# arkworks-rs/groth16

Hardware: AMD Instinct MI355X
Metric: R1CS constraints/sec (create_proof, BLS12-381) (higher is better)
Workload: dtype u32-limb Montgomery integers (Fr 255-bit, Fq 381-bit); 1 GPU; SYN(k=22) synthetic R1CS, 4194302 constraints, FFT domain 2^22, bls12_381, full create_proof (7 NTTs + 4 G1 MSMs + 1 G2 MSM), valid proving key generated on the GPU from seeded toxic waste; curve=bls12_381, log2_domain=22, constraints=4194302, key=valid, witness=resident in HBM at entry (--full: value_incl_h2d holds the PCIe-inclusive rates), parallelism=single-gpu

## Files before the change

### groth16_amd/csrc/api.hip

```cpp
#include "api_types.hpp"
#include "key_load.hpp"
#include "prover.hpp"
#include "proof_glue.hpp"
#include "unit_api.hpp"

namespace {
template <class C>
struct Impl : KeyLoader<C>, Prover<C>, ProofGlue<C>, UnitApi<C> {
    typedef typename C::Fr Fr;
    typedef typename C::Fq Fq;
    typedef typename C::Fq2 Fq2;
};
}

#define G16_DISPATCH(curve, EXPR)                                             \
    do {                                                                      \
        try {                                                                 \
            if ((curve) == G16_BLS12_381) { typedef Impl<Bls12_381> I; return EXPR; } \
            if ((curve) == G16_BN254) { typedef Impl<Bn254> I; return EXPR; }  \
            return G16_ERR_BAD_ARG;                                           \
        } catch (const std::bad_alloc&) {                                     \
            return G16_ERR_OOM;                                               \
        } catch (...) {                                                       \
            return G16_ERR_INTERNAL;                                          \
// ... 59 lines not shown
              hipEventCreate(&c->ev_edge[0]) == hipSuccess && hipEventCreate(&c->ev_edge[1]) == hipSuccess &&
              hipEventCreate(&c->ev_edge[2]) == hipSuccess && hipEventCreate(&c->ev_edge[3]) == hipSuccess &&
              hipEventCreate(&c->ev_edge[4]) == hipSuccess && hipEventCreate(&c->ev_edge[5]) == hipSuccess &&
              hipEventCreate(&c->ev_edge[6]) == hipSuccess && hipEventCreate(&c->ev_edge[7]) == hipSuccess &&
              hipEventCreateWithFlags(&c->ev_heavy[0], hipEventDisableTiming) == hipSuccess &&
              hipEventCreateWithFlags(&c->ev_heavy[1], hipEventDisableTiming) == hipSuccess &&
              hipEventCreateWithFlags(&c->ev_heavy[2], hipEventDisableTiming) == hipSuccess &&
              hipEventCreateWithFlags(&c->ev_heavy[3], hipEventDisableTiming) == hipSuccess &&
              hipStreamCreateWithPriority(&c->red[0], hipStreamNonBlocking, prio_hi) == hipSuccess &&
              hipStreamCreateWithPriority(&c->red[1], hipStreamNonBlocking, prio_hi) == hipSuccess &&
              hipStreamCreateWithPriority(&c->red[2], hipStreamNonBlocking, prio_hi) == hipSuccess &&
              hipStreamCreateWithPriority(&c->red[3], hipStreamNonBlocking, prio_hi) == hipSuccess &&
              hipStreamCreateWithPriority(&c->red[4], hipStreamNonBlocking, prio_hi) == hipSuccess &&
              hipEventCreateWithFlags(&c->ev_wm, hipEventDisableTiming) == hipSuccess &&
              hipEventCreateWithFlags(&c->ev_z, hipEventDisableTiming) == hipSuccess &&
              hipEventCreateWithFlags(&c->ev_h, hipEventDisableTiming) == hipSuccess;
    for (int i = 0; ok && i < 5; ++i)
        ok = hipEventCreate(&c->ev_done[i]) == hipSuccess;
    for (int i = 0; ok && i < 8; ++i)
        ok = hipEventCreateWithFlags(&c->ev_up[i], hipEventDisableTiming) == hipSuccess;
    if (!ok) {
        g16::set_last_error("stream/event creation", hipGetLastError(), __FILE__, __LINE__);
        delete c;
        return G16_ERR_HIP;
    }
    *out = c;
    return G16_OK;
}

int g16_ctx_create_multi(int curve, const int* device_ids, int n_dev, g16_ctx** out) {
    if (!out || !device_ids || n_dev < 1 || n_dev > 64 || (curve != G16_BLS12_381 && curve != G16_BN254)) return G16_ERR_BAD_ARG;
    if (n_dev == 1) return g16_ctx_create(curve, device_ids[0], out);
    g16_ctx* c = new (std::nothrow) g16_ctx();
    if (!c) return G16_ERR_OOM;
    c->curve = curve;
    c->device = device_ids[0];
    c->stream = c->stream2 = c->stream3 = nullptr;
    memset(&c->tm, 0, sizeof(c->tm));
    for (int i = 0; i < n_dev; ++i) {
        g16_ctx* sub = nullptr;
        const int rc = g16_ctx_create(curve, device_ids[i], &sub);
        if (rc) {
            for (g16_ctx* s : c->subs) g16_ctx_destroy(s);
            delete c;
            return rc;
        }
        c->subs.push_back(sub);
    }
    const bool require_peer = getenv("G16_MULTI_REQUIRE_PEER") && atoi(getenv("G16_MULTI_REQUIRE_PEER")) != 0;
    const bool fake_refusal = getenv("G16_MULTI_FAKE_NO_PEER") && atoi(getenv("G16_MULTI_FAKE_NO_PEER")) != 0;
    c->peer.assign((size_t)n_dev * (size_t)n_dev, 1);
    auto fail = [&](int rc) {
        for (g16_ctx* sub : c->subs) g16_ctx_destroy(sub);
        delete c;
        return rc;
    };
    for (int a = 0; a < n_dev; ++a)
        for (int b = 0; b < n_dev; ++b) {
            if (a == b) continue;
            int can = device_ids[a] == device_ids[b] ? 1 : 0;
            if (!can && hipDeviceCanAccessPeer(&can, device_ids[a], device_ids[b]) != hipSuccess) { (void)hipGetLastError(); can = 0; }
            if (fake_refusal) can = 0;
            if (can && device_ids[a] != device_ids[b]) {
                if (hipSetDevice(device_ids[a]) != hipSuccess) return fail(G16_ERR_HIP);
                const hipError_t e = hipDeviceEnablePeerAccess(device_ids[b], 0);
                if (e != hipSuccess && e != hipErrorPeerAccessAlreadyEnabled) {
                    g16::set_last_error("hipDeviceEnablePeerAccess (the pair reports peer capability)", e, __FILE__, __LINE__);
                    return fail(G16_ERR_HIP);
                }
                (void)hipGetLastError();
            }
            c->peer[(size_t)a * n_dev + b] = (char)can;
            if (!can && require_peer) {
                char buf[160];
                snprintf(buf, sizeof(buf), "devices %d and %d of the context have no peer access (G16_MULTI_REQUIRE_PEER=1)", device_ids[a], device_ids[b]);
                g_last_error = buf;
                return fail(G16_ERR_NO_PEER_ACCESS);
            }
        }
    *out = c;
    return G16_OK;
}

int g16_ctx_peer_access(const g16_ctx* ctx, int i, int j) {
    if (!ctx) return -1;
    const int n = ctx->subs.empty() ? 1 : (int)ctx->subs.size();
    if (i < 0 || j < 0 || i >= n || j >= n) return -1;
    if (i == j || ctx->subs.empty()) return 1;
    return ctx->peer[(size_t)i * n + j] ? 1 : 0;
}

int g16_ctx_num_devices(const g16_ctx* ctx) { return ctx ? (ctx->subs.empty() ? 1 : (int)ctx->subs.size()) : 0; }

void g16_ctx_destroy(g16_ctx* ctx) {
    if (!ctx) return;
    if (!ctx->subs.empty()) {
        for (g16_ctx* sub : ctx->subs) g16_ctx_destroy(sub);
        delete ctx;
        return;
    }
    ctx->finprep.drop();
    (void)hipSetDevice(ctx->device);
    (void)hipStreamSynchronize(ctx->stream);
    (void)hipStreamSynchronize(ctx->stream2);
    (void)hipStreamSynchronize(ctx->stream3);
    (void)hipStreamSynchronize(ctx->stream_wm);
    (void)hipStreamSynchronize(ctx->stream_h2d);
    for (int i = 0; i < 5; ++i) (void)hipStreamSynchronize(ctx->red[i]);
    ctx->arena.release();
    ctx->t_wm.destroy(); ctx->t_prep_h.destroy(); ctx->t_prep_z.destroy(); ctx->t_ntt[0].destroy(); ctx->t_ntt[1].destroy();
    for (int i = 0; i < 5; ++i) {
        ctx->t_bucket[i].destroy();
        (void)hipEventDestroy(ctx->ev_done[i]);
    }
    (void)hipEventDestroy(ctx->ev_z); (void)hipEventDestroy(ctx->ev_h); (void)hipEventDestroy(ctx->ev_wm); (void)hipEventDestroy(ctx->ev_dwm);
    for (int i = 0; i < 4; ++i) (void)hipEventDestroy(ctx->ev_heavy[i]);
    for (int i = 0; i < 8; ++i) (void)hipEventDestroy(ctx->ev_edge[i]);
    for (int i = 0; i < 8; ++i) (void)hipEventDestroy(ctx->ev_up[i]);
    (void)hipStreamDestroy(ctx->stream_h2d);
    (void)hipStreamDestroy(ctx->stream_wm);
    if (ctx->pinned) (void)hipHostFree(ctx->pinned);
    (void)hipStreamDestroy(ctx->stream);
    (void)hipStreamDestroy(ctx->stream2);
    (void)hipStreamDestroy(ctx->stream3);
    for (int i = 0; i < 5; ++i) (void)hipStreamDestroy(ctx->red[i]);
    delete ctx;
}

void* g16_ctx_stream(g16_ctx* ctx) { return ctx ? (void*)(ctx->subs.empty() ? ctx->stream : ctx->subs[0]->stream) : nullptr; }
void* g16_ctx_wm_stream(g16_ctx* ctx) { return ctx ? (void*)(ctx->subs.empty() ? ctx->stream_wm : ctx->subs[0]->stream_wm) : nullptr; }

int g16_pk_load(g16_ctx* ctx, const g16_pk_view* view, g16_pk** out) {
    if (!ctx || !view || !out) return G16_ERR_BAD_ARG;
    if (!ctx->subs.empty()) {
        const int n = (int)ctx->subs.size();
        if (view->a.start || view->b_g1.start || view->b_g2.start || view->h.start || view->l.start) return G16_ERR_BAD_ARG;
        if (view->b_g1.count != view->a.count || view->b_g2.count != view->a.count || view->l.count > view->a.count) return G16_ERR_BAD_LENGTH;
        if (view->flags & G16_PK_DEVICE_PTRS)
            for (g16_ctx* sub : ctx->subs) if (sub->device != ctx->subs[0]->device) return G16_ERR_BAD_ARG;
        g16_pk* h = new (std::nothrow) g16_pk{ctx->curve, ctx, nullptr};
        if (!h) return G16_ERR_OOM;
        h->subs.assign((size_t)n, nullptr);
        const uint64_t m = view->a.count, w = view->l.count, hl = view->h.count, skip = m - w;
        const size_t g1b = (ctx->curve == G16_BLS12_381 ? 12 : 8), g2b = 2 * g1b;
        const bool dist_h = !(view->flags & G16_PK_DEVICE_PTRS) && view->h.points && dist_wm_admissible(n, hl + 1);
        if (dist_h) h->dist_n = hl + 1;
        bool bucket = false, bucket_forced = false;
        {
            const char* me = g_multi_force_base ? "base" : getenv("G16_MULTI_SHARD_MODE");
            if (me && strcmp(me, "bucket") == 0) bucket = bucket_forced = true;
            else if (!me || strcmp(me, "auto") == 0) {
                const double key_bytes = (double)(g1b * 8) * (double)(m * 2 + w + hl) + (double)(g2b * 8) * (double)m;
                const double rows = m >= ((uint64_t)1 << 20) ? 13.0 : 32.0;
                const double need = rows * key_bytes * 1.08 + 3.0 * key_bytes + 8.0 * 1073741824.0;
                bucket = rows * key_bytes <= 80.0 * 1073741824.0 && !(view->flags & G16_PK_DEVICE_PTRS);
                const char* pc = getenv("G16_MSM_PRECOMP");
                if ((pc && atoi(pc) == 0) || m <= 1 || hl == 0) bucket = false;
                for (g16_ctx* sub : ctx->subs) {
                    size_t fr = 0, tot = 0;
                    if (!bucket) break;
                    if (hipSetDevice(sub->device) != hipSuccess || hipMemGetInfo(&fr, &tot) != hipSuccess) { (void)hipGetLastError(); bucket = false; }
                    size_t copies = 0;
                    for (g16_ctx* o : ctx->subs) copies += o->device == sub->device ? 1 : 0;
                    if (need * (double)copies > (double)fr) bucket = false;
                }
            }
            if (bucket && (view->flags & G16_PK_DEVICE_PTRS)) { delete h; return G16_ERR_BAD_ARG; }
        }
        h->bucket_mode = bucket;
        std::vector<uint64_t> hgather;
        if (bucket && dist_h) {
            const uint64_t M = (hl + 1) / (uint64_t)n, blk = M / (uint64_t)n;
            hgather.reserve((size_t)(hl * g1b));
            for (uint64_t q = 0; q < (uint64_t)n; ++q)
                for (uint64_t k1 = 0; k1 < (uint64_t)n; ++k1)
                    for (uint64_t j = 0; j < blk; ++j) {
                        const uint64_t idx = q * blk + j + M * k1;
                        if (idx < hl) hgather.insert(hgather.end(), view->h.points + idx * g1b, view->h.points + (idx + 1) * g1b);
                    }
        }
        int rc = for_each_device(n, [&](int i) -> int {
            g16_pk_view v = *view;
            if (bucket) {
                if (dist_h) { v.h.points = hgather.data(); v.h.count = hgather.size() / g1b; v.h.start = 0; }
                return g16_pk_load_bucket_shard(ctx->subs[(size_t)i], &v, i, n, &h->subs[(size_t)i]);
            }
            const uint64_t a_lo = m * (uint64_t)i / n, a_hi = m * (uint64_t)(i + 1) / n;
            const uint64_t l_lo = std::min(w, a_lo > skip ? a_lo - skip : 0), l_hi = std::min(w, a_hi > skip ? a_hi - skip : 0);
            const uint64_t h_lo = hl * (uint64_t)i / n, h_hi = hl * (uint64_t)(i + 1) / n;
            std::vector<uint64_t> hblock;
            if (dist_h) {
                const uint64_t M = (hl + 1) / (uint64_t)n, blk = M / (uint64_t)n;
                hblock.reserve((size_t)(M * g1b));
                for (uint64_t k1 = 0; k1 < (uint64_t)n; ++k1)
                    for (uint64_t j = 0; j < blk; ++j) {
                        const uint64_t idx = (uint64_t)i * blk + j + M * k1;
                        if (idx < hl) hblock.insert(hblock.end(), view->h.points + idx * g1b, view->h.points + (idx + 1) * g1b);
                    }
            }
            auto cut = [](const g16_query& q, uint64_t lo, uint64_t hi, size_t limbs) {
                g16_query r;
                r.points = q.points ? q.points + lo * limbs : nullptr;
                r.count = hi - lo;
                r.start = lo;
                return r;
            };
            v.a = cut(view->a, a_lo, a_hi, g1b);
            v.b_g1 = cut(view->b_g1, a_lo, a_hi, g1b);
            v.b_g2 = cut(view->b_g2, a_lo, a_hi, g2b);
            v.l = cut(view->l, l_lo, l_hi, g1b);
            v.h = cut(view->h, h_lo, h_hi, g1b);
            if (dist_h) { v.h.points = hblock.data(); v.h.count = hblock.size() / g1b; v.h.start = 0; }
            return g16_pk_load(ctx->subs[(size_t)i], &v, &h->subs[(size_t)i]);
        }, serial_loads(ctx));
        if ((rc == G16_ERR_OOM || rc == G16_ERR_BAD_ARG) && bucket && !bucket_forced) {
            for (g16_pk*& sub : h->subs) { g16_pk_free(sub); sub = nullptr; }
            delete h;
            g_multi_force_base = true;
            const int rc2 = g16_pk_load(ctx, view, out);
            g_multi_force_base = false;
            return rc2;
        }
        if (rc) { g16_pk_free(h); return rc; }
        *out = h;
        return G16_OK;
    }
    G16_HIP_TRY(hipSetDevice(ctx->device));
    G16_DISPATCH(ctx->curve, I::pk_load(ctx, view, out));
}

int g16_pk_load_bucket_shard(g16_ctx* ctx, const g16_pk_view* view, int rank, int world, g16_pk** out) {
    if (!ctx || !view || !out || world < 1 || world > 64 || rank < 0 || rank >= world) return G16_ERR_BAD_ARG;
    if (!ctx->subs.empty()) return G16_ERR_BAD_ARG;
    if (world == 1) return g16_pk_load(ctx, view, out);
    G16_HIP_TRY(hipSetDevice(ctx->device));
    G16_DISPATCH(ctx->curve, I::pk_load(ctx, view, out, world, rank));
}

int g16_pk_rebind_bucket_shard(g16_pk* pk, int rank, int world) {
    if (!pk || world < 1 || world > 64 || rank < 0 || rank >= world || !pk->subs.empty() || !pk->dp) return G16_ERR_BAD_ARG;
    auto rebind = [&](auto* dp) -> int {
        if (dp->c_z == 0 || dp->a_start || dp->b_g1_start || dp->b_g2_start || dp->h_start || dp->l_start) return G16_ERR_BAD_ARG;
        dp->shard_n = world;
        dp->shard_r = rank;
        return G16_OK;
    };
    if (pk->ctx->finprep.key_id == pk->id) pk->ctx->finprep.drop();
    pk->ctx->drop_prepared_sort(pk->id);
    if (pk->curve == G16_BLS12_381) return rebind(static_cast<DevicePk<Bls12_381>*>(pk->dp));
    return rebind(static_cast<DevicePk<Bn254>*>(pk->dp));
}

int g16_pk_get_info(const g16_pk* pk, g16_pk_info* out) {
    if (!pk || !out) return G16_ERR_BAD_ARG;
    memset(out, 0, sizeof(*out));
    const g16_pk* one = pk->subs.empty() ? pk : pk->subs[0];
    if (!one || !one->dp) return G16_ERR_BAD_ARG;
    auto fill = [&](const auto* dp) {
        out->window_bits_z = dp->c_z;
        out->window_bits_h = dp->c_h;
        out->table_fallback = dp->table_fallback;
        out->bucket_shard_rank = dp->shard_r;
        out->bucket_shard_world = dp->shard_n;
        out->device_bytes = dp->table_bytes;
    };
    if (one->curve == G16_BLS12_381) fill(static_cast<const DevicePk<Bls12_381>*>(one->dp));
    else fill(static_cast<const DevicePk<Bn254>*>(one->dp));
    out->n_devices = pk->subs.empty() ? 1 : (int)pk->subs.size();
    return G16_OK;
}

void g16_pk_free(g16_pk* pk) {
    if (!pk) return;
    if (!pk->ctx->subs.empty()) {
        for (g16_pk* sub : pk->subs) g16_pk_free(sub);
        delete pk;
        return;
    }
    if (pk->ctx->finprep.key_id == pk->id) pk->ctx->finprep.drop();
    (void)hipSetDevice(pk->ctx->device);
    pk->ctx->drop_prepared_sort(pk->id);
    if (pk->curve == G16_BLS12_381) Impl<Bls12_381>::pk_free(static_cast<DevicePk<Bls12_381>*>(pk->dp));
    else Impl<Bn254>::pk_free(static_cast<DevicePk<Bn254>*>(pk->dp));
    delete pk;
}

int g16_circuit_load(g16_ctx* ctx, const g16_csr_view abc[3], uint64_t num_inputs, uint64_t num_constraints, uint64_t num_variables,
                     g16_circuit** out) {
    if (!ctx || !abc || !out) return G16_ERR_BAD_ARG;
    if (!ctx->subs.empty()) {
        const int n = (int)ctx->subs.size();
        g16_circuit* h = new (std::nothrow) g16_circuit{ctx->curve, ctx, nullptr, 0};
        if (!h) return G16_ERR_OOM;
        h->subs.assign((size_t)n, nullptr);
        const int rc = for_each_device(n, [&](int i) -> int {
            return g16_circuit_load(ctx->subs[(size_t)i], abc, num_inputs, num_constraints, num_variables, &h->subs[(size_t)i]);
        }, serial_loads(ctx));
        if (rc) { g16_circuit_free(h); return rc; }
        h->domain_size = h->subs[0]->domain_size;
        h->num_variables = num_variables;
        if (dist_wm_admissible(n, h->domain_size)) {
            h->dist.assign((size_t)n, DwmSlot());
            const uint64_t M = h->domain_size / (uint64_t)n;
            const int rc2 = for_each_device(n, [&](int i) -> int {
                DwmSlot& sl = h->dist[(size_t)i];
                G16_TRY(g16_dwm_create(ctx->subs[(size_t)i], h->subs[(size_t)i], i, n, &sl.dwm));
                for (int k = 0; k < 3; ++k) {
                    if (hipMalloc((void**)&sl.work[k], M * 32) != hipSuccess || hipMalloc((void**)&sl.recv[k], M * 32) != hipSuccess) return G16_ERR_OOM;
// ... 480 lines not shown
```

### groth16_amd/csrc/batch_affine.hpp

```cpp
#pragma once
#include "curve.hpp"
#include "fp30.hpp"

namespace g16 {

template <class P>
struct ModInv30 {
    static constexpr int NL = P::NL30;
    static constexpr int32_t M30 = (int32_t)((1u << 30) - 1u);
    struct S30 { int32_t v[NL]; };
    struct T2x2 { int32_t u, v, q, r; };

    G16_HD static int32_t divsteps30(int32_t zeta, uint32_t f0, uint32_t g0, T2x2& t) {
        uint32_t u = 1, v = 0, q = 0, r = 1, f = f0, g = g0;
        for (int i = 0; i < 30; ++i) {
            uint32_t m1 = (uint32_t)(zeta >> 31);
            const uint32_t m2 = 0u - (g & 1u);
            const uint32_t x = (f ^ m1) - m1, y = (u ^ m1) - m1, z = (v ^ m1) - m1;
            g += x & m2; q += y & m2; r += z & m2;
            m1 &= m2;
            zeta = (zeta ^ (int32_t)m1) - 1;
            f += g & m1; u += q & m1; v += r & m1;
            g >>= 1; u <<= 1; v <<= 1;
        }
        t.u = (int32_t)u; t.v = (int32_t)v; t.q = (int32_t)q; t.r = (int32_t)r;
        return zeta;
    }
    G16_HD static void update_fg(S30& f, S30& g, const T2x2& t) {
        const int64_t u = t.u, v = t.v, q = t.q, r = t.r;
        int64_t cf = u * f.v[0] + v * g.v[0], cg = q * f.v[0] + r * g.v[0];
        cf >>= 30; cg >>= 30;
        G16_UNROLL for (int i = 1; i < NL; ++i) {
            cf += u * f.v[i] + v * g.v[i];
            cg += q * f.v[i] + r * g.v[i];
            f.v[i - 1] = (int32_t)cf & M30; cf >>= 30;
            g.v[i - 1] = (int32_t)cg & M30; cg >>= 30;
        }
        f.v[NL - 1] = (int32_t)cf;
        g.v[NL - 1] = (int32_t)cg;
    }
    G16_HD static void update_de(S30& d, S30& e, const T2x2& t) {
        const int64_t u = t.u, v = t.v, q = t.q, r = t.r;
        const int32_t sd = d.v[NL - 1] >> 31, se = e.v[NL - 1] >> 31;
        int32_t md = (t.u & sd) + (t.v & se), me = (t.q & sd) + (t.r & se);
        int64_t cd = u * d.v[0] + v * e.v[0], ce = q * d.v[0] + r * e.v[0];
        md -= (int32_t)((P::PPINV30 * (uint32_t)cd + (uint32_t)md) & (uint32_t)M30);
        me -= (int32_t)((P::PPINV30 * (uint32_t)ce + (uint32_t)me) & (uint32_t)M30);
        cd += (int64_t)(int32_t)P::p30(0) * md;
        ce += (int64_t)(int32_t)P::p30(0) * me;
        cd >>= 30; ce >>= 30;
        G16_UNROLL for (int i = 1; i < NL; ++i) {
            cd += u * d.v[i] + v * e.v[i] + (int64_t)(int32_t)P::p30(i) * md;
            ce += q * d.v[i] + r * e.v[i] + (int64_t)(int32_t)P::p30(i) * me;
            d.v[i - 1] = (int32_t)cd & M30; cd >>= 30;
            e.v[i - 1] = (int32_t)ce & M30; ce >>= 30;
        }
        d.v[NL - 1] = (int32_t)cd;
        e.v[NL - 1] = (int32_t)ce;
    }
    G16_HD static void carry(S30& r) {
        G16_UNROLL for (int i = 0; i + 1 < NL; ++i) { r.v[i + 1] += r.v[i] >> 30; r.v[i] &= M30; }
    }
    G16_HD static void normalize(S30& r, int32_t sign) {
        const int32_t add1 = r.v[NL - 1] >> 31, neg = sign >> 31;
        G16_UNROLL for (int i = 0; i < NL; ++i) {
            int32_t x = r.v[i] + ((int32_t)P::p30(i) & add1);
            r.v[i] = (x ^ neg) - neg;
        }
        carry(r);
        const int32_t add2 = r.v[NL - 1] >> 31;
        G16_UNROLL for (int i = 0; i < NL; ++i) r.v[i] += (int32_t)P::p30(i) & add2;
        carry(r);
    }
    G16_HD static Fp30<P> inverse_plain(const Fp30<P>& x) {
        S30 d, e, f, g;
        G16_UNROLL for (int i = 0; i < NL; ++i) { d.v[i] = 0; e.v[i] = 0; f.v[i] = (int32_t)P::p30(i); g.v[i] = (int32_t)x.l[i]; }
        e.v[0] = 1;
        int32_t zeta = -1;
        for (int it = 0; it < 4 * NL; ++it) {
            int32_t nz = 0;
            G16_UNROLL for (int i = 0; i < NL; ++i) nz |= g.v[i];
            if (nz == 0) break;
            T2x2 t;
            zeta = divsteps30(zeta, (uint32_t)f.v[0], (uint32_t)g.v[0], t);
            update_de(d, e, t);
            update_fg(f, g, t);
        }
        normalize(d, f.v[NL - 1]);
        Fp30<P> r;
        G16_UNROLL for (int i = 0; i < NL; ++i) r.l[i] = (uint32_t)d.v[i];
        return r;
    }
    G16_HD static Fp30<P> inverse(const Fp30<P>& x) {
        Fp30<P> c;
        G16_UNROLL for (int i = 0; i < NL; ++i) c.l[i] = P::r3_30(i);
        return inverse_plain(x).mul(c);
    }
};

template <class P>
G16_HD Fp30<P> batch_inverse(const Fp30<P>& a) { return ModInv30<P>::inverse(a); }
template <class P>
G16_HD Fp30<P> pair_inverse(bool hi, const Fp30<P>& m, const Fp30<P>& o) {
    const Fp30<P> n = m.sqr().add(o.sqr());
    const Fp30<P> t = m.mul(ModInv30<P>::inverse(n));
    return hi ? Fp30<P>::zero().template sub<2>(t) : t;
}
template <class P>
G16_HD Fp2p30<P> batch_inverse(const Fp2p30<P>& a) { return {pair_inverse<P>(Fp2p30<P>::lane_hi(), a.c, Fp2p30<P>::swap(a.c))}; }

template <class F>
struct AffineBatch {
    enum { ADD = 0, DBL = 1, TAKE_P = 2, TAKE_Q = 3, ZERO = 4 };
    G16_HD static int classify(bool pz, bool qz, const F& px, const F& py, const F& qx, const F& qy, F& d) {
        d = F::one();
        if (pz || qz) return pz ? (qz ? (int)ZERO : (int)TAKE_Q) : (int)TAKE_P;
        if (qx.equals_canonical(px)) {
            if (py.add(qy).is_zero_exact()) return ZERO;
            d = py.dbl();
            return DBL;
        }
        d = qx.template sub<2>(px);
        return ADD;
    }
    G16_HD static void finish(int kind, const F& px, const F& py, const F& qx, const F& qy, const F& inv_d, F& rx, F& ry, bool& rz) {
        rz = false;
        if (kind >= TAKE_P) {
            if (kind == TAKE_P) { rx = px; ry = py; }
            else if (kind == TAKE_Q) { rx = qx; ry = qy; }
            else { rx = F::zero(); ry = F::zero(); rz = true; }
            return;
        }
        F num;
        if (kind == DBL) {
            const F x2 = px.sqr();
            num = x2.dbl().add(x2);
        } else {
            num = qy.template sub<2>(py);
        }
        const F lam = num.mul(inv_d);
        rx = lam.sqr().template sub<2>(px).template sub<2>(qx).canonical_lt8p();
        ry = lam.mul(px.template sub<2>(rx)).template sub<2>(py).canonical_lt8p();
    }
};

struct alignas(16) Word4 { uint32_t w[4]; };
static constexpr uint32_t SORT_HOLE = 0xffffffffu;

template <class F>
struct AffineLevelArgs {
    const Affine<typename F::Std>* in;
    Affine<typename F::Std>* out;
    const uint32_t* sorted;
    const uint32_t* total;
    Word4* prefix;
    int64_t shift;
    uint64_t base_count;
    uint32_t merged;
    uint32_t level;
    uint32_t K;
};

template <class F, bool LEVEL0>
struct AffineLevel {
    typedef Affine<typename F::Std> A;
    static constexpr int LPT = F::LANES_PER_TASK;
    static constexpr uint32_t T = 64 / LPT;
    static constexpr int QUADS = (F::PREFIX_LIMBS + 3) / 4;

    G16_HD static bool load_operand(const AffineLevelArgs<F>& a, uint64_t slot, F& x, F& y) {
        if constexpr (LEVEL0) {
            const uint32_t v = a.sorted[slot];
            if (v == SORT_HOLE) return false;
            const uint32_t pt = a.merged ? (v & 0x3ffffffu) : (v & 0x7fffffffu);
            const uint64_t row = a.merged ? (uint64_t)((v >> 26) & 31u) * a.base_count : 0;
            const int64_t idx = (int64_t)pt + a.shift;
            if (idx < 0 || (uint64_t)idx >= a.base_count) return false;
            if (!F::load_point(a.in, (int64_t)row + idx, x, y)) return false;
            if (v >> 31) y = y.neg_canonical();
            return true;
        } else {
            return F::load_point(a.in, (int64_t)slot, x, y);
        }
    }
    G16_HD static void store_prefix(const AffineLevelArgs<F>& a, uint32_t wave, uint32_t j, uint32_t lane, const F& v) {
        uint32_t w[4 * QUADS];
        G16_UNROLL for (int i = 0; i < 4 * QUADS; ++i) w[i] = 0;
        v.get_limbs(w);
        Word4* dst = a.prefix + ((uint64_t)wave * a.K + j) * (QUADS * 64) + lane;
        G16_UNROLL for (int c = 0; c < QUADS; ++c) {
            Word4 q;
            G16_UNROLL for (int i = 0; i < 4; ++i) q.w[i] = w[4 * c + i];
            dst[c * 64] = q;
        }
    }
    G16_HD static F load_prefix(const AffineLevelArgs<F>& a, uint32_t wave, uint32_t j, uint32_t lane) {
        uint32_t w[4 * QUADS];
        const Word4* src = a.prefix + ((uint64_t)wave * a.K + j) * (QUADS * 64) + lane;
        G16_UNROLL for (int c = 0; c < QUADS; ++c) {
            const Word4 q = src[c * 64];
            G16_UNROLL for (int i = 0; i < 4; ++i) w[4 * c + i] = q.w[i];
        }
        return F::from_limbs(w);
    }
    G16_HD static void run(const AffineLevelArgs<F>& a, uint32_t wave, uint32_t lane) {
        const uint64_t n_out = (uint64_t)(*a.total) >> (a.level + 1);
        const uint64_t first = (uint64_t)wave * a.K * T;
        if (first >= n_out) return;
        const uint64_t left = (n_out - first + T - 1) / T;
        const uint32_t steps = left < a.K ? (uint32_t)left : a.K;
        const uint32_t task = lane / LPT;
        F pre = F::one();
        for (uint32_t j = 0; j < steps; ++j) {
            const uint64_t q = first + (uint64_t)j * T + task;
            F px = F::zero(), py = F::zero(), qx = F::zero(), qy = F::zero(), d;
            bool pz = true, qz = true;
            if (q < n_out) {
                pz = !load_operand(a, 2 * q, px, py);
                qz = !load_operand(a, 2 * q + 1, qx, qy);
            }
            (void)AffineBatch<F>::classify(pz, qz, px, py, qx, qy, d);
            pre = pre.mul(d);
            store_prefix(a, wave, j, lane, pre);
        }
        F inv = batch_inverse(pre);
        for (uint32_t j = steps; j-- > 0;) {
            const uint64_t q = first + (uint64_t)j * T + task;
            F px = F::zero(), py = F::zero(), qx = F::zero(), qy = F::zero(), d;
            bool pz = true, qz = true;
            if (q < n_out) {
                pz = !load_operand(a, 2 * q, px, py);
                qz = !load_operand(a, 2 * q + 1, qx, qy);
            }
            const F prev = j ? load_prefix(a, wave, j - 1, lane) : F::one();
            const int kind = AffineBatch<F>::classify(pz, qz, px, py, qx, qy, d);
            const F inv_d = inv.mul(prev);
            inv = inv.mul(d);
            F rx, ry;
            bool rz;
            AffineBatch<F>::finish(kind, px, py, qx, qy, inv_d, rx, ry, rz);
            if (q < n_out) F::store_point(a.out, (int64_t)q, rx, ry, rz);
        }
    }
};

}
```

### groth16_amd/csrc/devtest.hip

```cpp
#include "internal.hpp"
#include "fp30.hpp"
#include <vector>

using namespace g16;

namespace g16 {
int ctx_devices(const g16_ctx* ctx, int* curve, std::vector<int>& devs, std::vector<hipStream_t>& streams);
}

namespace {

constexpr bool lab_slots(int form, int* nin, int* nout) {
    int i = 0, o = 1;
    switch (form) {
        case 0: i = 2; break;
        case 1: i = 1; break;
        case 2: i = 4; break;
        case 3: i = 8; break;
        case 4: case 6: case 8: i = 3; break;
        case 5: case 7: case 9: i = 5; break;
        case 10: i = 4; break;
        case 11: i = 3; break;
        case 20: case 21: case 22: case 23: case 24: case 25: i = 2; break;
        case 26: i = 1; break;
        case 27: i = 3; break;
        case 28: i = 2; o = 2; break;
        case 30: case 31: case 32: case 33: case 34: case 35: case 36: case 37: case 38: case 39: case 40: case 41: case 42: case 43: i = 1; break;
        case 50: i = 4; o = 2; break;
        case 51: i = 2; o = 2; break;
        case 60: i = 4; o = 2; break;
        case 61: i = 2; o = 2; break;
        case 62: i = 6; o = 2; break;
        case 63: case 64: case 65: i = 8; o = 2; break;
        case 70: i = 11; o = 5; break;
        case 71: case 72: i = 21; o = 9; break;
        default: return false;
    }
    *nin = i;
    *nout = o;
    return true;
}
constexpr int lab_nin(int form) { int i = 0, o = 0; lab_slots(form, &i, &o); return i; }
constexpr int lab_nout(int form) { int i = 0, o = 0; lab_slots(form, &i, &o); return o; }
constexpr bool lab_is_pair(int form) { return (form >= 60 && form < 70) || form == 72; }
template <class P>
constexpr bool lab_has(int form) {
    constexpr bool base = FipsAsm<P>::has_sub;
    if ((form >= 4 && form <= 11) || form >= 50) return base;
    if (form == 27) return !base;
    return true;
}

template <class P> G16_HD Fp30<P> ld(const uint32_t* s, int k) {
    Fp30<P> r;
    G16_UNROLL for (int i = 0; i < Fp30<P>::NL; ++i) r.l[i] = s[k * Fp30<P>::NL + i];
    return r;
}
template <class P> G16_HD void st(uint32_t* o, int k, const Fp30<P>& v) {
    G16_UNROLL for (int i = 0; i < Fp30<P>::NL; ++i) o[k * Fp30<P>::NL + i] = v.l[i];
}
template <class P> G16_HD void st_flag(uint32_t* o, int k, bool b) {
    G16_UNROLL for (int i = 0; i < Fp30<P>::NL; ++i) o[k * Fp30<P>::NL + i] = (i == 0 && b) ? 1u : 0u;
}
template <class P> G16_HD Fp<P> ld_words(const uint32_t* s, int k) {
    Fp<P> r;
    G16_UNROLL for (int i = 0; i < P::N; ++i) r.v[i] = s[k * Fp30<P>::NL + i];
    return r;
}
template <class P> G16_HD void st_words(uint32_t* o, int k, const Fp<P>& v) {
    G16_UNROLL for (int i = 0; i < Fp30<P>::NL; ++i) o[k * Fp30<P>::NL + i] = i < P::N ? v.v[i] : 0u;
}

template <class P, class F>
struct AccLab {
    typedef Fp30<P> B;
    static constexpr int C = sizeof(F) == sizeof(B) && F::LANES_PER_TASK == 1 ? 1 : 2;
    G16_HD static F ldf(const uint32_t* in, int slot, int hi) {
        if constexpr (F::LANES_PER_TASK == 2) return F{ld<P>(in, slot + hi)};
        else if constexpr (C == 2) return F{ld<P>(in, slot), ld<P>(in, slot + 1)};
        else return ld<P>(in, slot);
    }
    G16_HD static void stf(uint32_t* out, int slot, int hi, const F& v) {
        if constexpr (F::LANES_PER_TASK == 2) st_words<P>(out, slot + hi, v.c.to_packed());
        else if constexpr (C == 2) { st_words<P>(out, slot, v.c0.to_packed()); st_words<P>(out, slot + 1, v.c1.to_packed()); }
        else st_words<P>(out, slot, v.to_packed());
    }
    G16_HD static void run(const uint32_t* in, uint32_t* out, int hi) {
        const uint32_t* flags = in + 4 * C * B::NL;
        Acc30<F> a;
        a.x = ldf(in, 0, hi); a.y = ldf(in, C, hi); a.zz = ldf(in, 2 * C, hi); a.zzz = ldf(in, 3 * C, hi);
        a.inf = flags[0] != 0;
        const int n = flags[1] > 3u ? 3 : (int)flags[1];
        for (int j = 0; j < n; ++j) {
            if (flags[2 + j] != 0) continue;
            a.add_affine(ldf(in, 4 * C + 1 + 2 * j * C, hi), ldf(in, 4 * C + 1 + (2 * j + 1) * C, hi));
        }
        if (a.inf) a.x = a.y = a.zz = a.zzz = F::zero();
        stf(out, 0, hi, a.x); stf(out, C, hi, a.y); stf(out, 2 * C, hi, a.zz); stf(out, 3 * C, hi, a.zzz);
        if (F::LANES_PER_TASK == 1 || hi == 0) st_flag<P>(out, 4 * C, a.inf);
    }
};

template <class P, int FORM>
struct LabOp {
    typedef Fp30<P> B;
    G16_HD static void run(const uint32_t* in, uint32_t* out) {
        auto L = [&](int k) { return ld<P>(in, k); };
        if constexpr (FORM == 0) st<P>(out, 0, L(0).mul(L(1)));
        else if constexpr (FORM == 1) st<P>(out, 0, L(0).sqr());
        else if constexpr (FORM == 2) st<P>(out, 0, B::mul_add_fused(L(0), L(1), L(2), L(3)));
        else if constexpr (FORM == 3) st<P>(out, 0, B::template mul4_cols<uint64_t>(L(0), L(1), L(2), L(3), L(4), L(5), L(6), L(7)));
        else if constexpr (FORM == 4) st<P>(out, 0, L(0).template mul_sub_k<2>(L(1), L(2)));
        else if constexpr (FORM == 5) st<P>(out, 0, B::template mul2_sub_k<2>(L(0), L(1), L(2), L(3), L(4)));
        else if constexpr (FORM == 6) st<P>(out, 0, L(0).template mul_sub_k<4>(L(1), L(2)));
        else if constexpr (FORM == 7) st<P>(out, 0, B::template mul2_sub_k<4>(L(0), L(1), L(2), L(3), L(4)));
        else if constexpr (FORM == 8) st<P>(out, 0, L(0).template mul_sub_k<8>(L(1), L(2)));
        else if constexpr (FORM == 9) st<P>(out, 0, B::template mul2_sub_k<8>(L(0), L(1), L(2), L(3), L(4)));
        else if constexpr (FORM == 10) st<P>(out, 0, L(0).mul_sub_x3(L(1), L(2), L(3)));
        else if constexpr (FORM == 11) st<P>(out, 0, L(0).sqr_sub_x3(L(1), L(2)));
        else if constexpr (FORM == 20) st<P>(out, 0, L(0).template sub<2>(L(1)));
        else if constexpr (FORM == 21) st<P>(out, 0, L(0).template sub<4>(L(1)));
        else if constexpr (FORM == 22) st<P>(out, 0, L(0).template sub<6>(L(1)));
        else if constexpr (FORM == 23) st<P>(out, 0, L(0).template sub<8>(L(1)));
        else if constexpr (FORM == 24) st<P>(out, 0, L(0).template sub<16>(L(1)));
        else if constexpr (FORM == 25) st<P>(out, 0, L(0).add_dbl(L(1)));
        else if constexpr (FORM == 26) { B a = L(0); a.normalize(); st<P>(out, 0, a); }
        else if constexpr (FORM == 27) {
            const int k = (int)in[2 * B::NL];
            st<P>(out, 0, L(0).sub_pow2(L(1), k < 0 ? 0 : k > 11 ? 11 : k));
        }
        else if constexpr (FORM == 28) {
            const Fp<P> y = ld_words<P>(in, 0);
            const bool flip = in[B::NL] != 0;
            st<P>(out, 0, B::unpack_cond_neg(y, flip));
            st<P>(out, 1, B::cond_neg2(B::unpack(y.v), flip));
        }
        else if constexpr (FORM == 30) st<P>(out, 0, L(0).template cond_sub<2>());
        else if constexpr (FORM == 31) st<P>(out, 0, L(0).template cond_sub<4>());
        else if constexpr (FORM == 32) st<P>(out, 0, L(0).template cond_sub<8>());
        else if constexpr (FORM == 33) st<P>(out, 0, L(0).template cond_sub<16>());
        else if constexpr (FORM == 34) st<P>(out, 0, L(0).weak_reduce32());
        else if constexpr (FORM == 35) st<P>(out, 0, L(0).canonical_lt2p());
        else if constexpr (FORM == 36) st<P>(out, 0, L(0).canonical_lt8p());
        else if constexpr (FORM == 37) st<P>(out, 0, L(0).canonical_quick());
        else if constexpr (FORM == 38) st<P>(out, 0, L(0).neg_canonical());
        else if constexpr (FORM == 39) st_flag<P>(out, 0, L(0).maybe_zero());
        else if constexpr (FORM == 40) st_flag<P>(out, 0, L(0).is_zero_exact());
        else if constexpr (FORM == 41) st_words<P>(out, 0, L(0).to_std());
        else if constexpr (FORM == 42) st_words<P>(out, 0, B::std_to_r30(ld_words<P>(in, 0)));
        else if constexpr (FORM == 43) st_words<P>(out, 0, L(0).to_packed());
        else if constexpr (FORM == 50) {
            const Fp2x30<P> a{L(0), L(1)}, b{L(2), L(3)};
            const Fp2x30<P> r = a.mul(b);
            st<P>(out, 0, r.c0); st<P>(out, 1, r.c1);
        }
        else if constexpr (FORM == 51) {
            const Fp2x30<P> a{L(0), L(1)};
            const Fp2x30<P> r = a.sqr();
            st<P>(out, 0, r.c0); st<P>(out, 1, r.c1);
        }
        else if constexpr (FORM == 70) AccLab<P, Fp30<P>>::run(in, out, 0);
        else if constexpr (FORM == 71) AccLab<P, Fp2x30<P>>::run(in, out, 0);
    }
};

template <class P, int FORM>
struct LabPair {
    typedef Fp30<P> B;
    typedef Fp2p30<P> F;
#if defined(__HIP_DEVICE_COMPILE__)
    static __device__ __forceinline__ void run(const uint32_t* in, uint32_t* out) {
        const int hi = F::lane_hi() ? 1 : 0;
        if constexpr (FORM == 72) { AccLab<P, F>::run(in, out, hi); return; }
        auto L = [&](int k) { return F{ld<P>(in, 2 * k + hi)}; };
        F r = F::zero();
        if constexpr (FORM == 60) r = F::mul_v(F::lhs(L(0)), F::rhs(L(1)));
        else if constexpr (FORM == 61) r = F::sqr_v(F::lhs(L(0)));
        else if constexpr (FORM == 62) r = F::sqr_sub_x3_v(F::lhs(L(0)), L(1), L(2));
        else if constexpr (FORM == 63) r = F::mul_add_fused(L(0), L(1), L(2), L(3));
        else if constexpr (FORM == 64) r = F::mul_sub_fused(L(0), L(1), L(2), L(3));
        else if constexpr (FORM == 65) r = F::mul_add_fused_v(F::lhs(L(0)), F::rhs(L(1)), F::lhs(L(2)), F::rhs(L(3)));
        st<P>(out, hi, r.c);
    }
#endif
    static void run_host(const uint32_t* in, uint32_t* out) {
        for (int h = 0; h < 2; ++h) {
            const bool hi = h != 0;
            auto C = [&](int k, int c) { return ld<P>(in, 2 * k + c); };
            auto y2 = [&](int k) { return hi ? C(k, 0) : C(k, 1).neg16(); };
            B r = B::zero();
            if constexpr (FORM == 60) r = F::pair_mul_c(hi, C(0, 0), C(0, 1), C(1, h), C(1, 1 - h));
            else if constexpr (FORM == 61) r = F::pair_sqr_c(hi, C(0, 0), C(0, 1));
            else if constexpr (FORM == 62) r = F::pair_sqr_sub_x3(hi, C(0, 0), C(0, 1), C(1, h), C(2, h));
            else if constexpr (FORM == 63) r = F::pair_mul_add_c(hi, C(0, 0), C(0, 1), C(1, h), C(1, 1 - h), C(2, 0), C(2, 1), C(3, h), C(3, 1 - h));
            else if constexpr (FORM == 64) r = F::pair_mul_sub_c(hi, C(0, 0), C(0, 1), C(1, h), C(1, 1 - h), C(2, 0), C(2, 1), C(3, h), C(3, 1 - h));
            else if constexpr (FORM == 65) r = B::template mul4_cols<uint64_t>(C(0, 0), C(1, h), C(0, 1), y2(1), C(2, 0), C(3, h), C(2, 1), y2(3));
            st<P>(out, h, r);
        }
    }
};

constexpr int LAB_WG = 64;

template <class P, int FORM>
__global__ void __launch_bounds__(LAB_WG) devlab_op(const uint32_t* __restrict__ in, uint32_t* __restrict__ out, uint32_t n) {
    constexpr int NL = Fp30<P>::NL, NIN = lab_nin(FORM), NOUT = lab_nout(FORM);
    const uint32_t t = blockIdx.x * LAB_WG + threadIdx.x;
    if constexpr (lab_is_pair(FORM)) {
        if (t >= 2 * n) return;
        const size_t i = t >> 1;
#if defined(__HIP_DEVICE_COMPILE__)
        LabPair<P, FORM>::run(in + i * NIN * NL, out + i * NOUT * NL);
#endif
    } else {
        if (t >= n) return;
        LabOp<P, FORM>::run(in + (size_t)t * NIN * NL, out + (size_t)t * NOUT * NL);
    }
}

template <class P, int FORM>
int lab_device(hipStream_t st, const uint32_t* operands, uint64_t n, uint32_t* out) {
    constexpr int NL = Fp30<P>::NL, NIN = lab_nin(FORM), NOUT = lab_nout(FORM);
    const size_t in_bytes = (size_t)n * NIN * NL * 4, out_bytes = (size_t)n * NOUT * NL * 4;
    uint32_t *d_in = nullptr, *d_out = nullptr;
    G16_HIP_TRY(hipMalloc((void**)&d_in, in_bytes));
    if (hipMalloc((void**)&d_out, out_bytes) != hipSuccess) { (void)hipFree(d_in); return G16_ERR_OOM; }
    auto body = [&]() -> int {
        G16_HIP_TRY(hipMemcpyAsync(d_in, operands, in_bytes, hipMemcpyHostToDevice, st));
        G16_HIP_TRY(hipMemsetAsync(d_out, 0, out_bytes, st));
        const uint64_t lanes = lab_is_pair(FORM) ? 2 * n : n;
        devlab_op<P, FORM><<<dim3((unsigned)((lanes + LAB_WG - 1) / LAB_WG)), dim3(LAB_WG), 0, st>>>(d_in, d_out, (uint32_t)n);
        G16_LAUNCH_CHECK();
        G16_HIP_TRY(hipMemcpyAsync(out, d_out, out_bytes, hipMemcpyDeviceToHost, st));
        G16_HIP_TRY(hipStreamSynchronize(st));
        return G16_OK;
    };
    const int rc = body();
    (void)hipFree(d_in);
    (void)hipFree(d_out);
    return rc;
}

template <class P, int FORM>
int lab_host(const uint32_t* operands, uint64_t n, uint32_t* out) {
    constexpr int NL = Fp30<P>::NL, NIN = lab_nin(FORM), NOUT = lab_nout(FORM);
    for (uint64_t i = 0; i < n; ++i) {
        if constexpr (lab_is_pair(FORM)) LabPair<P, FORM>::run_host(operands + i * NIN * NL, out + i * NOUT * NL);
        else LabOp<P, FORM>::run(operands + i * NIN * NL, out + i * NOUT * NL);
    }
    return G16_OK;
}

#define LAB_FORMS(X)                                                                                                              \
    X(0) X(1) X(2) X(3) X(4) X(5) X(6) X(7) X(8) X(9) X(10) X(11) X(20) X(21) X(22) X(23) X(24) X(25) X(26) X(27) X(28) X(30) X(31) \
    X(32) X(33) X(34) X(35) X(36) X(37) X(38) X(39) X(40) X(41) X(42) X(43) X(50) X(51) X(60) X(61) X(62) X(63) X(64) X(65) X(70) X(71) X(72)

template <class P>
int lab_dispatch(bool device, hipStream_t st, int form, const uint32_t* operands, uint64_t n, uint32_t* out) {
    switch (form) {
#define X(F)                                                                                   \
    case F:                                                                                    \
        if constexpr (lab_has<P>(F)) {                                                         \
            if (device) return lab_device<P, F>(st, operands, n, out);                         \
            if constexpr (F == 72) return G16_ERR_BAD_ARG;                                     \
            else return lab_host<P, F>(operands, n, out);                                      \
        } else return G16_ERR_BAD_ARG;
        LAB_FORMS(X)
#undef X
        default: return G16_ERR_BAD_ARG;
    }
}

int lab_run(int curve, bool device, hipStream_t st, int field, int form, const uint32_t* operands, uint64_t n, uint32_t* out) {
    int nin = 0, nout = 0;
    if (!operands || !out || n == 0 || n > ((uint64_t)1 << 22) || (field != 0 && field != 1) || !lab_slots(form, &nin, &nout)) return G16_ERR_BAD_ARG;
    if (curve == G16_BLS12_381)
        return field ? lab_dispatch<Bls12_381FqP>(device, st, form, operands, n, out) : lab_dispatch<Bls12_381FrP>(device, st, form, operands, n, out);
    if (curve == G16_BN254)
        return field ? lab_dispatch<Bn254FqP>(device, st, form, operands, n, out) : lab_dispatch<Bn254FrP>(device, st, form, operands, n, out);
    return G16_ERR_BAD_ARG;
}

}

extern "C" int g16_dev_fp30_op(g16_ctx* ctx, int field, int form, const uint32_t* operands, uint64_t n, uint32_t* out) {
    int curve = 0;
    std::vector<int> devs;
    std::vector<hipStream_t> streams;
    G16_TRY(ctx_devices(ctx, &curve, devs, streams));
    G16_HIP_TRY(hipSetDevice(devs[0]));
    return lab_run(curve, true, streams[0], field, form, operands, n, out);
}

extern "C" int g16_host_fp30_op(int curve, int field, int form, const uint32_t* operands, uint64_t n, uint32_t* out) {
    return lab_run(curve, false, nullptr, field, form, operands, n, out);
}
```

### groth16_amd/csrc/fp30.hpp

```cpp
#pragma once
#include "field.hpp"
#include "fips_asm_gen.hpp"

#if defined(__HIP_DEVICE_COMPILE__) && !defined(G16_NO_FIPS_ASM)
#define G16_ASM_PRODUCTS 1
#endif

namespace g16 {

template <class P>
struct Fp30 {
    typedef P Params_t;
    static constexpr int NL = P::NL30;
    static constexpr int NW = P::N;
    static constexpr uint32_t MASK = (1u << 30) - 1u;
    uint32_t l[NL];

    G16_HD static Fp30 zero() {
        Fp30 r;
        G16_UNROLL for (int i = 0; i < NL; ++i) r.l[i] = 0;
        return r;
    }
    G16_HD static Fp30 one() {
        Fp30 r;
        G16_UNROLL for (int i = 0; i < NL; ++i) r.l[i] = P::one30(i);
        return r;
    }
    G16_HD static Fp30 unpack(const uint32_t* w) {
        Fp30 r;
        G16_UNROLL for (int i = 0; i < NL; ++i) {
            const int bit = 30 * i, wd = bit >> 5, sh = bit & 31;
            uint32_t v = w[wd] >> sh;
            if (sh > 2 && wd + 1 < NW) v |= w[wd + 1] << (32 - sh);
            r.l[i] = (i == NL - 1) ? v : (v & MASK);
        }
        return r;
    }
    G16_HD void pack(uint32_t* w) const {
        G16_UNROLL for (int k = 0; k < NW; ++k) w[k] = 0;
        G16_UNROLL for (int i = 0; i < NL; ++i) {
            const int bit = 30 * i, wd = bit >> 5, sh = bit & 31;
            w[wd] |= l[i] << sh;
            if (sh > 2 && wd + 1 < NW) w[wd + 1] |= l[i] >> (32 - sh);
        }
    }
    G16_HD void normalize() {
        G16_UNROLL for (int i = 0; i + 1 < NL; ++i) {
            l[i + 1] += l[i] >> 30;
            l[i] &= MASK;
        }
    }
    G16_HD Fp30 add(const Fp30& b) const {
        Fp30 r;
        G16_UNROLL for (int i = 0; i < NL; ++i) r.l[i] = l[i] + b.l[i];
        r.normalize();
        return r;
    }
    G16_HD Fp30 dbl() const { return add(*this); }
    template <int K>
    G16_HD Fp30 sub(const Fp30& b) const {
        static_assert(K == 2 || K == 4 || K == 6 || K == 8 || K == 16, "redundant K p tables exist for K = 2, 4, 6, 8, 16 only");
        Fp30 r;
        G16_UNROLL for (int i = 0; i < NL; ++i) {
            const uint32_t kp = K == 2 ? P::kp2(i) : K == 4 ? P::kp4(i) : K == 6 ? P::kp6(i) : K == 8 ? P::kp8(i) : P::kp16(i);
            r.l[i] = l[i] + kp - b.l[i];
        }
        r.normalize();
        return r;
    }
    G16_HD Fp30 add_dbl(const Fp30& b) const {
        Fp30 r;
        G16_UNROLL for (int i = 0; i < NL; ++i) r.l[i] = l[i] + (b.l[i] << 1);
        r.normalize();
        return r;
    }
    G16_HD Fp30 sub_pow2(const Fp30& b, int k) const {
        Fp30 r;
        G16_UNROLL for (int i = 0; i < NL; ++i) r.l[i] = l[i] + P::kp_pow2(k, i) - b.l[i];
        r.normalize();
        return r;
    }
    G16_HD Fp30 neg2() const { return zero().template sub<2>(*this); }
    typedef Fp<P> PackedC;
    G16_HD static constexpr uint32_t two_p32(int i) { return (P::mod(i) << 1) | (i ? P::mod(i - 1) >> 31 : 0u); }
    G16_HD static Fp30 unpack_cond_neg(const PackedC& y, bool flip) {
        uint32_t w[NW];
#if defined(__HIP_DEVICE_COMPILE__)
        unsigned borrow = 0;
        G16_UNROLL for (int i = 0; i < NW; ++i) {
            const uint32_t d = __builtin_subc(two_p32(i), y.v[i], borrow, &borrow);
            w[i] = flip ? d : y.v[i];
        }
#else
        uint32_t borrow = 0;
        G16_UNROLL for (int i = 0; i < NW; ++i) {
            const uint64_t t = (uint64_t)two_p32(i) - y.v[i] - borrow;
            borrow = (uint32_t)(t >> 63);
            w[i] = flip ? (uint32_t)t : y.v[i];
        }
#endif
        return unpack(w);
    }
    G16_HD static Fp30 cond_neg2(const Fp30& a, bool flip) { return flip ? a.neg2() : a; }
    G16_HD Fp30 neg16() const { return zero().template sub<16>(*this); }
    typedef Fp<P> Std;
    G16_HD static Fp30 from_packed(const Std& x) { return unpack(x.v); }

    G16_HD Fp30 mul(const Fp30& b) const { return mul_impl(b); }
    template <int NS>
    struct FipsPlan {
        unsigned char seg[2 * NL][NS + 1];
        unsigned char nseg[2 * NL];
        int extra;
        bool ok;
    };
    template <int NS>
    static constexpr FipsPlan<NS> fips_plan() {
        typedef unsigned __int128 W;
        FipsPlan<NS> pl{};
        const W LIM = (W)1 << 64, M = MASK, W32 = 0xffffffffu;
        W carry = 0;
        pl.ok = true;
        pl.extra = 0;
        for (int c = 0; c < 2 * NL - 1; ++c) {
            const int lo = c < NL ? 0 : c - NL + 1, hi = c < NL ? c : NL - 1;
            W psum = 0;
            for (int i = lo; i <= hi; ++i)
                if (i != c) psum += M * (W)P::p30(c - i);
            W B[NS + 1] = {};
            B[0] = carry + (c < NL ? M * (W)P::p30(0) : (W)0) + (W)(NS + 2) * W32;
            int cur = 0;
            for (int k = 0; k <= NS; ++k) {
                const W part = k < NS ? (W)(hi - lo + 1) * M * M : psum;
                if (B[cur] + part >= LIM) {
                    ++cur;
                    if (cur > NS || part >= LIM) { pl.ok = false; return pl; }
                }
                B[cur] += part;
                pl.seg[c][k] = (unsigned char)cur;
            }
            pl.nseg[c] = (unsigned char)(cur + 1);
            pl.extra += cur;
            carry = B[0] >> 30;
            for (int s = 1; s <= cur; ++s) carry += 4 * (B[s] >> 32);
        }
        return pl;
    }
    template <int NS>
    static constexpr bool fips_asm_plan_agrees() {
        if constexpr (!FipsAsm<P>::available) return true;
        else {
            static_assert(NS == 1 || NS == 2 || NS == 4, "assembly exists for one, two and four sweeps");
            const FipsPlan<NS> pl = fips_plan<NS>();
            if (!pl.ok || FipsAsm<P>::NL != NL) return false;
            for (int c = 0; c < 2 * NL - 1; ++c)
                for (int k = 0; k <= NS; ++k) {
                    const int want = NS == 1 ? FipsAsm<P>::plan1(c * 2 + k) : NS == 2 ? FipsAsm<P>::plan2(c * 3 + k) : FipsAsm<P>::plan4(c * 5 + k);
                    if (pl.seg[c][k] != want) return false;
                }
            return true;
        }
// ... 97 lines not shown
            Fp30 r;
            FipsAsm<P>::mul2(r.l, x1.l, y1.l, x2.l, y2.l);
            return r;
        }
#endif
        const Fp30* xs[2] = {&x1, &x2};
        const Fp30* ys[2] = {&y1, &y2};
        return fips<U, 2, false>(xs, ys);
    }
    template <class U>
    G16_HD static Fp30 mul4_cols(const Fp30& x1, const Fp30& y1, const Fp30& x2, const Fp30& y2, const Fp30& x3, const Fp30& y3,
                                 const Fp30& x4, const Fp30& y4) {
#ifdef G16_ASM_PRODUCTS
        if constexpr (sizeof(U) == 8 && FipsAsm<P>::available) {
            static_assert(fips_asm_plan_agrees<4>(), "gen_fips_asm.py and Fp30::fips_plan disagree on the column plan");
            Fp30 r;
            FipsAsm<P>::mul4(r.l, x1.l, y1.l, x2.l, y2.l, x3.l, y3.l, x4.l, y4.l);
            return r;
        }
#endif
        const Fp30* xs[4] = {&x1, &x2, &x3, &x4};
        const Fp30* ys[4] = {&y1, &y2, &y3, &y4};
        return fips<U, 4, false>(xs, ys);
    }
    template <class U>
    G16_HD static Fp30 mul_sub_cols(const Fp30& a, const Fp30& b, const Fp30& c, const Fp30& d) {
        return mul2_cols<U>(a, b, c, d.neg2());
    }
    template <int K>
    G16_HD Fp30 mul_sub_k(const Fp30& b, const Fp30& s) const {
        static_assert(K == 2 || K == 4 || K == 8, "fused subtraction: K = 2, 4, 8");
#ifdef G16_ASM_PRODUCTS
        if constexpr (FipsAsm<P>::has_sub) {
            static_assert(fips_asm_plan_agrees<1>(), "gen_fips_asm.py and Fp30::fips_plan disagree on the column plan");
            Fp30 r;
            if constexpr (K == 2) FipsAsm<P>::mul_s2(r.l, l, b.l, s.l);
            else if constexpr (K == 4) FipsAsm<P>::mul_s4(r.l, l, b.l, s.l);
            else FipsAsm<P>::mul_s8(r.l, l, b.l, s.l);
            return r;
        }
#endif
        return mul(b).template sub<K>(s);
    }
    template <int K>
    G16_HD static Fp30 mul2_sub_k(const Fp30& x1, const Fp30& y1, const Fp30& x2, const Fp30& y2, const Fp30& s) {
        static_assert(K == 2 || K == 4 || K == 8, "fused subtraction: K = 2, 4, 8");
#ifdef G16_ASM_PRODUCTS
        if constexpr (FipsAsm<P>::has_sub) {
            static_assert(fips_asm_plan_agrees<2>(), "gen_fips_asm.py and Fp30::fips_plan disagree on the column plan");
            Fp30 r;
            if constexpr (K == 2) FipsAsm<P>::mul2_s2(r.l, x1.l, y1.l, x2.l, y2.l, s.l);
            else if constexpr (K == 4) FipsAsm<P>::mul2_s4(r.l, x1.l, y1.l, x2.l, y2.l, s.l);
            else FipsAsm<P>::mul2_s8(r.l, x1.l, y1.l, x2.l, y2.l, s.l);
            return r;
        }
#endif
        return mul2_cols<uint64_t>(x1, y1, x2, y2).template sub<K>(s);
    }
    G16_HD Fp30 sqr_sub_x3(const Fp30& u, const Fp30& v) const {
#ifdef G16_ASM_PRODUCTS
        if constexpr (FipsAsm<P>::has_sub) {
            Fp30 r;
            FipsAsm<P>::sqr_x3(r.l, l, u.l, v.l);
            return r;
        }
#endif
        return sqr().template sub<6>(u.add_dbl(v));
    }
    G16_HD Fp30 mul_sub_x3(const Fp30& b, const Fp30& u, const Fp30& v) const {
#ifdef G16_ASM_PRODUCTS
        if constexpr (FipsAsm<P>::has_sub) {
            Fp30 r;
            FipsAsm<P>::mul_x3(r.l, l, b.l, u.l, v.l);
            return r;
        }
#endif
        return mul_impl(b).template sub<6>(u.add_dbl(v));
    }
    G16_HD Fp30 mul_impl(const Fp30& b) const { return mul_cols<uint64_t>(b); }
    G16_HD static Fp30 mul_sub(const Fp30& a, const Fp30& b, const Fp30& c, const Fp30& d) { return a.mul(b).template sub<2>(c.mul(d)); }
    typedef Fp30 Lhs;
    typedef Fp30 Rhs;
    G16_HD static const Fp30& lhs(const Fp30& a) { return a; }
    G16_HD static const Fp30& rhs(const Fp30& a) { return a; }
    G16_HD static Fp30 mul_v(const Fp30& a, const Fp30& b) { return a.mul(b); }
    G16_HD static Fp30 sqr_v(const Fp30& a) { return a.sqr(); }
    G16_HD static Fp30 sqr_sub_x3_v(const Fp30& a, const Fp30& u, const Fp30& v) { return a.sqr_sub_x3(u, v); }
    G16_HD static Fp30 mul_add_fused_v(const Fp30& a, const Fp30& b, const Fp30& c, const Fp30& d) { return mul2_cols<uint64_t>(a, b, c, d); }
    G16_HD static Fp30 mul_add_fused(const Fp30& a, const Fp30& b, const Fp30& c, const Fp30& d) { return mul2_cols<uint64_t>(a, b, c, d); }
    G16_HD static Fp30 mul_sub_fused(const Fp30& a, const Fp30& b, const Fp30& c, const Fp30& d) { return mul_sub_cols<uint64_t>(a, b, c, d); }
    G16_HD Fp30 sqr() const { return sqr_cols<uint64_t>(); }

    G16_HD bool maybe_zero() const { return ((l[0] * P::PPINV30) & MASK) < 16u; }
    G16_HD bool is_zero_exact() const {
        const uint32_t k = (l[0] * P::PPINV30) & MASK;
        if (k >= 16u) return false;
        Fp30 kp;
        uint64_t c = 0;
        G16_UNROLL for (int i = 0; i < NL; ++i) {
            const uint64_t v = (uint64_t)k * P::p30(i) + c;
            kp.l[i] = (i == NL - 1) ? (uint32_t)v : ((uint32_t)v & MASK);
            c = v >> 30;
        }
        uint32_t diff = 0;
        G16_UNROLL for (int i = 0; i < NL; ++i) diff |= kp.l[i] ^ l[i];
        return diff == 0;
    }
    template <int K>
    G16_HD Fp30 cond_sub() const {
        static_assert(K == 2 || K == 4 || K == 8 || K == 16, "k p constants exist for k = 2, 4, 8, 16 only");
        Fp30 d;
        int32_t br = 0;
        G16_UNROLL for (int i = 0; i < NL; ++i) {
            const uint32_t c = K == 2 ? P::np2(i) : K == 4 ? P::np4(i) : K == 8 ? P::np8(i) : P::np16(i);
            const int32_t v = (int32_t)l[i] - (int32_t)c + br;
            if (i == NL - 1) { d.l[i] = (uint32_t)v; br = v >> 31; }
            else { d.l[i] = (uint32_t)v & MASK; br = v >> 30; }
        }
        Fp30 r;
        const bool lt = br < 0;
        G16_UNROLL for (int i = 0; i < NL; ++i) r.l[i] = lt ? l[i] : d.l[i];
        return r;
    }
    G16_HD Fp30 weak_reduce32() const { return cond_sub<16>().template cond_sub<8>().template cond_sub<4>().template cond_sub<2>(); }
    G16_HD bool raw_zero() const {
        uint32_t a = 0;
        G16_UNROLL for (int i = 0; i < NL; ++i) a |= l[i];
        return a == 0;
    }
    typedef Fp30 Raw;
    static constexpr int KM = 2, K2M = 4, KX = 8, KY = 4;
#ifndef G16_ACC_MIN_WAVES
#define G16_ACC_MIN_WAVES 2
#endif
    static constexpr int ACC_MIN_WAVES = G16_ACC_MIN_WAVES;
    static constexpr bool ACC_PREFETCH = true;
    static constexpr int LANES_PER_TASK = 1;
    template <class A>
    G16_HD static bool load_point(const A* bases, int64_t idx, Fp30& px, Fp30& py) {
        const A p = bases[idx];
        if (p.is_identity()) return false;
        px = from_packed(p.x);
        py = from_packed(p.y);
        return true;
    }
    template <class A>
    G16_HD static bool load_point_py(const A* bases, int64_t idx, Fp30& px, PackedC& yw) {
        const A p = bases[idx];
        if (p.is_identity()) return false;
        px = from_packed(p.x);
        yw = p.y;
        return true;
    }


    G16_HD Fp30 canonical_lt2p() const {
        Fp30 d;
        int32_t br = 0;
        G16_UNROLL for (int i = 0; i < NL; ++i) {
            const int32_t v = (int32_t)l[i] - (int32_t)P::p30(i) + br;
            if (i == NL - 1) { d.l[i] = (uint32_t)v; br = v >> 31; }
            else { d.l[i] = (uint32_t)v & MASK; br = v >> 30; }
        }
        Fp30 r;
        const bool lt = br < 0;
        G16_UNROLL for (int i = 0; i < NL; ++i) r.l[i] = lt ? l[i] : d.l[i];
        return r;
    }

    G16_HD Fp30 canonical_lt8p() const { return cond_sub<4>().template cond_sub<2>().canonical_lt2p(); }
    G16_HD Fp30 canonical_quick() const {
        constexpr uint32_t D = P::p30(NL - 1) + 1u;
        static_assert(D > (1u << 13), "the top limb of p carries at least 14 bits for every supported field");
        constexpr uint64_t MAGIC = ((uint64_t)1 << 40) / D;
        const uint32_t q = (uint32_t)(((uint64_t)l[NL - 1] * MAGIC) >> 40);
        Fp30 r;
        int64_t carry = 0;
        G16_UNROLL for (int i = 0; i < NL; ++i) {
            const int64_t t = (int64_t)l[i] - (int64_t)((uint64_t)q * P::p30(i)) + carry;
            r.l[i] = (i == NL - 1) ? (uint32_t)t : ((uint32_t)t & MASK);
            carry = t >> 30;
        }
        return r.canonical_lt8p();
    }
    G16_HD Fp30 neg_canonical() const {
        Fp30 d;
        int32_t br = 0;
        G16_UNROLL for (int i = 0; i < NL; ++i) {
            const int32_t v = (int32_t)P::p30(i) - (int32_t)l[i] + br;
            if (i == NL - 1) d.l[i] = (uint32_t)v;
            else { d.l[i] = (uint32_t)v & MASK; br = v >> 30; }
        }
        return d;
    }
    G16_HD bool same_limbs(const Fp30& o) const {
        uint32_t a = 0;
        G16_UNROLL for (int i = 0; i < NL; ++i) a |= l[i] ^ o.l[i];
        return a == 0;
    }
    static constexpr int PREFIX_LIMBS = NL;
    G16_HD void get_limbs(uint32_t* w) const { G16_UNROLL for (int i = 0; i < NL; ++i) w[i] = l[i]; }
    G16_HD static Fp30 from_limbs(const uint32_t* w) { Fp30 r; G16_UNROLL for (int i = 0; i < NL; ++i) r.l[i] = w[i]; return r; }
    G16_HD bool equals_canonical(const Fp30& o) const { return same_limbs(o); }
    template <class A>
    G16_HD static void store_point(A* dst, int64_t idx, const Fp30& x, const Fp30& y, bool identity) {
        A p;
        if (identity) { p = A::identity(); }
        else { x.pack(p.x.v); y.pack(p.y.v); }
        dst[idx] = p;
    }

    G16_HD Std to_packed() const {
        Std r;
        mul_impl(one()).canonical_lt2p().pack(r.v);
        return r;
    }
    G16_HD static Fp<P> std_to_r30(const Fp<P>& x) {
        Fp<P> c;
        G16_UNROLL for (int i = 0; i < P::N; ++i) c.v[i] = P::r30_plain(i);
        return x * c;
    }
    G16_HD Fp<P> to_std() const {
        Fp30 c;
        G16_UNROLL for (int i = 0; i < NL; ++i) c.l[i] = P::rstd30(i);
        const Fp30 t = mul(c).canonical_lt2p();
        Fp<P> r;
        t.pack(r.v);
        return r;
    }
};

template <class P>
struct Fp2x30 {
    typedef Fp30<P> B;
    typedef Fp2<P> Std;
    B c0, c1;
    G16_HD static Fp2x30 zero() { return {B::zero(), B::zero()}; }
    G16_HD static Fp2x30 one() { return {B::one(), B::zero()}; }
    G16_HD static Fp2x30 from_packed(const Std& x) { return {B::unpack(x.c0.v), B::unpack(x.c1.v)}; }
    G16_HD Fp2x30 add(const Fp2x30& o) const { return {c0.add(o.c0), c1.add(o.c1)}; }
    G16_HD Fp2x30 dbl() const { return {c0.dbl(), c1.dbl()}; }
    G16_HD Fp2x30 add_dbl(const Fp2x30& o) const { return {c0.add_dbl(o.c0), c1.add_dbl(o.c1)}; }
    template <int K>
    G16_HD Fp2x30 sub(const Fp2x30& o) const { return {c0.template sub<K>(o.c0), c1.template sub<K>(o.c1)}; }
    G16_HD Fp2x30 neg2() const { return {c0.neg2(), c1.neg2()}; }
    G16_HD static Fp2x30 cond_neg2(const Fp2x30& a, bool flip) { return flip ? a.neg2() : a; }
    G16_HD Fp2x30 mul_impl(const Fp2x30& o) const {
        Fp2x30 r;
        const B nb1 = o.c1.neg16();
        r.c0 = B::template mul2_cols<uint64_t>(c0, o.c0, c1, nb1);
        r.c1 = B::template mul2_cols<uint64_t>(c0, o.c1, c1, o.c0);
        return r;
    }
    G16_HD Fp2x30 sqr_impl() const {
        return {c0.add(c1).mul_impl(c0.template sub<16>(c1)), c0.dbl().mul_impl(c1)};
    }
    G16_HD_NOINLINE static Fp2x30 mul_outlined(const Fp2x30& a, const Fp2x30& b) { return a.mul_impl(b); }
    G16_HD_NOINLINE static Fp2x30 sqr_outlined(const Fp2x30& a) { return a.sqr_impl(); }
    G16_HD Fp2x30 mul(const Fp2x30& o) const { return mul_outlined(*this, o); }
    G16_HD Fp2x30 sqr() const { return sqr_outlined(*this); }
    template <int K>
    G16_HD Fp2x30 mul_sub_k(const Fp2x30& o, const Fp2x30& s) const { return mul(o).template sub<K>(s); }
    G16_HD Fp2x30 sqr_sub_x3(const Fp2x30& u, const Fp2x30& v) const { return sqr().template sub<KM + K2M>(u.add_dbl(v)); }
    G16_HD bool maybe_zero() const { return c0.maybe_zero() && c1.maybe_zero(); }
    G16_HD bool is_zero_exact() const { return c0.is_zero_exact() && c1.is_zero_exact(); }
    G16_HD Std to_std() const { return {c0.to_std(), c1.to_std()}; }
    G16_HD Std to_packed() const { return {c0.to_packed(), c1.to_packed()}; }
    static constexpr int KM = 2, K2M = 4, KX = 8, KY = 4;
    G16_HD static Fp2x30 mul_sub(const Fp2x30& a, const Fp2x30& b, const Fp2x30& c, const Fp2x30& d) { return a.mul(b).template sub<KM>(c.mul(d)); }
    G16_HD static Fp2x30 mul_sub_fused(const Fp2x30& a, const Fp2x30& b, const Fp2x30& c, const Fp2x30& d) { return mul_sub(a, b, c, d); }
    G16_HD static Fp2x30 mul_add_fused(const Fp2x30& a, const Fp2x30& b, const Fp2x30& c, const Fp2x30& d) { return a.mul(b).add(c.mul(d)); }
    typedef Fp2x30 Lhs;
    typedef Fp2x30 Rhs;
    G16_HD static const Fp2x30& lhs(const Fp2x30& a) { return a; }
    G16_HD static const Fp2x30& rhs(const Fp2x30& a) { return a; }
    G16_HD static Fp2x30 mul_v(const Fp2x30& a, const Fp2x30& b) { return a.mul(b); }
    G16_HD static Fp2x30 sqr_v(const Fp2x30& a) { return a.sqr(); }
    G16_HD static Fp2x30 sqr_sub_x3_v(const Fp2x30& a, const Fp2x30& u, const Fp2x30& v) { return a.sqr_sub_x3(u, v); }
    G16_HD static Fp2x30 mul_add_fused_v(const Fp2x30& a, const Fp2x30& b, const Fp2x30& c, const Fp2x30& d) { return mul_add_fused(a, b, c, d); }
    G16_HD bool raw_zero() const { return c0.raw_zero() && c1.raw_zero(); }
    typedef Fp2x30 Raw;
    static constexpr int PREFIX_LIMBS = 2 * B::NL;
    static constexpr int LANES_PER_TASK = 1;
};

template <class P>
struct Fp2p30 {
    typedef Fp30<P> B;
    typedef Fp2<P> Std;
    B c;

    G16_HD static bool lane_hi() {
#if defined(__HIP_DEVICE_COMPILE__)
        return (threadIdx.x & 1u) != 0;
#else
        return false;
#endif
    }
    G16_HD static uint32_t swap32(uint32_t v) {
#if defined(__HIP_DEVICE_COMPILE__)
        return (uint32_t)__builtin_amdgcn_mov_dpp((int)v, 0xB1 , 0xF, 0xF, true);
#else
        return v;
#endif
    }
    G16_HD static B swap(const B& x) {
        B r;
        G16_UNROLL for (int i = 0; i < B::NL; ++i) r.l[i] = swap32(x.l[i]);
        return r;
    }
    G16_HD static B sel(bool c, const B& a, const B& b) {
        B r;
        G16_UNROLL for (int i = 0; i < B::NL; ++i) r.l[i] = c ? a.l[i] : b.l[i];
        return r;
    }
    G16_HD static uint32_t bcast32(uint32_t v, bool odd) {
#if defined(__HIP_DEVICE_COMPILE__)
        return odd ? (uint32_t)__builtin_amdgcn_mov_dpp((int)v, 0xF5 , 0xF, 0xF, true)
                   : (uint32_t)__builtin_amdgcn_mov_dpp((int)v, 0xA0 , 0xF, 0xF, true);
#else
        return v;
#endif
    }
    G16_HD static B comp0(const B& x) { B r; G16_UNROLL for (int i = 0; i < B::NL; ++i) r.l[i] = bcast32(x.l[i], false); return r; }
    G16_HD static B comp1(const B& x) { B r; G16_UNROLL for (int i = 0; i < B::NL; ++i) r.l[i] = bcast32(x.l[i], true); return r; }
    G16_HD static B pair_mul_c(bool hi, const B& a0, const B& a1, const B& mb, const B& ob) {
        const B y2 = sel(hi, ob, ob.neg16());
        return pair_cols<uint64_t>(a0, mb, a1, y2);
    }
    G16_HD static B pair_mul(bool hi, const B& ma, const B& oa, const B& mb, const B& ob) {
        return pair_mul_c(hi, sel(hi, oa, ma), sel(hi, ma, oa), mb, ob);
    }
    template <class U>
    G16_HD static B pair_cols(const B& x1, const B& y1, const B& x2, const B& y2) {
        return B::template mul2_cols<U>(x1, y1, x2, y2);
    }
    G16_HD static void pair_sqr_operands(bool hi, const B& a0, const B& a1, B& x, B& y) {
        x = a0.add(sel(hi, a0, a1));
        y = sel(hi, a1, a0.template sub<16>(a1));
    }
    G16_HD static B pair_sqr_c(bool hi, const B& a0, const B& a1) {
        B x, y;
        pair_sqr_operands(hi, a0, a1, x, y);
        return x.mul_impl(y);
    }
    G16_HD static B pair_sqr(bool hi, const B& m, const B& o) { return pair_sqr_c(hi, sel(hi, o, m), sel(hi, m, o)); }
    G16_HD static B pair_mul_sub_c(bool hi, const B& a0, const B& a1, const B& mb, const B& ob, const B& c0, const B& c1, const B& md,
                                   const B& od) {
        const B y2 = sel(hi, ob, ob.neg16());
        const B z1 = md.neg2();
        const B z2 = sel(hi, od.neg2(), od);
        return B::template mul4_cols<uint64_t>(a0, mb, a1, y2, c0, z1, c1, z2);
    }
    G16_HD static B pair_mul_sub(bool hi, const B& ma, const B& oa, const B& mb, const B& ob, const B& mc, const B& oc, const B& md,
                                 const B& od) {
        return pair_mul_sub_c(hi, sel(hi, oa, ma), sel(hi, ma, oa), mb, ob, sel(hi, oc, mc), sel(hi, mc, oc), md, od);
    }
    G16_HD static B pair_mul_add_c(bool hi, const B& a0, const B& a1, const B& mb, const B& ob, const B& c0, const B& c1, const B& md,
                                   const B& od) {
        const B y2 = sel(hi, ob, ob.neg16());
        const B z2 = sel(hi, od, od.neg2());
        return B::template mul4_cols<uint64_t>(a0, mb, a1, y2, c0, md, c1, z2);
    }
    G16_HD static Fp2p30 mul_add_fused(const Fp2p30& a, const Fp2p30& b, const Fp2p30& c, const Fp2p30& d) {
        return {pair_mul_add_c(lane_hi(), comp0(a.c), comp1(a.c), b.c, swap(b.c), comp0(c.c), comp1(c.c), d.c, swap(d.c))};
    }
    struct Lhs { B a0, a1; };
    struct Rhs { B m, y2; };
    G16_HD static Lhs lhs(const Fp2p30& a) { return {comp0(a.c), comp1(a.c)}; }
    G16_HD static Rhs rhs(const Fp2p30& b) { return {b.c, swap(sel(lane_hi(), b.c.neg16(), b.c))}; }
    G16_HD static Fp2p30 mul_v(const Lhs& a, const Rhs& b) { return {pair_cols<uint64_t>(a.a0, b.m, a.a1, b.y2)}; }
    G16_HD static Fp2p30 sqr_v(const Lhs& a) { return {pair_sqr_c(lane_hi(), a.a0, a.a1)}; }
    G16_HD static Fp2p30 sqr_sub_x3_v(const Lhs& a, const Fp2p30& u, const Fp2p30& v) { return {pair_sqr_sub_x3(lane_hi(), a.a0, a.a1, u.c, v.c)}; }
    G16_HD static Fp2p30 mul_add_fused_v(const Lhs& a, const Rhs& b, const Lhs& c, const Rhs& d) {
        return {B::template mul4_cols<uint64_t>(a.a0, b.m, a.a1, b.y2, c.a0, d.m, c.a1, d.y2)};
    }
    G16_HD static Fp2p30 mul_sub(const Fp2p30& a, const Fp2p30& b, const Fp2p30& c, const Fp2p30& d) { return a.mul(b).template sub<2>(c.mul(d)); }
    G16_HD static Fp2p30 mul_sub_fused(const Fp2p30& a, const Fp2p30& b, const Fp2p30& c, const Fp2p30& d) {
        return {pair_mul_sub_c(lane_hi(), comp0(a.c), comp1(a.c), b.c, swap(b.c), comp0(c.c), comp1(c.c), d.c, swap(d.c))};
    }
    G16_HD static Fp2p30 zero() { return {B::zero()}; }
    G16_HD static Fp2p30 one() { return {lane_hi() ? B::zero() : B::one()}; }
    G16_HD Fp2p30 add(const Fp2p30& o) const { return {c.add(o.c)}; }
    G16_HD Fp2p30 dbl() const { return {c.dbl()}; }
    G16_HD Fp2p30 add_dbl(const Fp2p30& o) const { return {c.add_dbl(o.c)}; }
    template <int K>
    G16_HD Fp2p30 sub(const Fp2p30& o) const { return {c.template sub<K>(o.c)}; }
    G16_HD Fp2p30 neg2() const { return {c.neg2()}; }
    G16_HD static Fp2p30 cond_neg2(const Fp2p30& a, bool flip) { return flip ? a.neg2() : a; }
    G16_HD Fp2p30 mul(const Fp2p30& o) const { return {pair_mul_c(lane_hi(), comp0(c), comp1(c), o.c, swap(o.c))}; }
    template <int K>
    G16_HD static B pair_mul_sub_k(bool hi, const B& a0, const B& a1, const B& mb, const B& ob, const B& sub) {
        const B y2 = sel(hi, ob, ob.neg16());
        return B::template mul2_sub_k<K>(a0, mb, a1, y2, sub);
    }
    template <int K>
    G16_HD Fp2p30 mul_sub_k(const Fp2p30& o, const Fp2p30& s) const { return {pair_mul_sub_k<K>(lane_hi(), comp0(c), comp1(c), o.c, swap(o.c), s.c)}; }
    G16_HD static B pair_sqr_sub_x3(bool hi, const B& a0, const B& a1, const B& u, const B& v) {
        B x, y;
        pair_sqr_operands(hi, a0, a1, x, y);
        return x.mul_sub_x3(y, u, v);
    }
    G16_HD Fp2p30 sqr_sub_x3(const Fp2p30& u, const Fp2p30& v) const { return {pair_sqr_sub_x3(lane_hi(), comp0(c), comp1(c), u.c, v.c)}; }
    G16_HD Fp2p30 sqr() const { return {pair_sqr_c(lane_hi(), comp0(c), comp1(c))}; }
    G16_HD static bool both(bool v) { return v && (swap32(v ? 1u : 0u) != 0u); }
    G16_HD bool maybe_zero() const { return both(c.maybe_zero()); }
    G16_HD bool is_zero_exact() const { return both(c.is_zero_exact()); }
    static constexpr int KM = 2, K2M = 4, KX = 8, KY = 4;
    G16_HD Fp2p30 canonical_lt8p() const { return {c.canonical_lt8p()}; }
    G16_HD Fp2p30 neg_canonical() const { return {c.neg_canonical()}; }
    G16_HD bool equals_canonical(const Fp2p30& o) const { return both(c.same_limbs(o.c)); }
    static constexpr int PREFIX_LIMBS = B::NL;
    G16_HD void get_limbs(uint32_t* w) const { c.get_limbs(w); }
    G16_HD static Fp2p30 from_limbs(const uint32_t* w) { return {B::from_limbs(w)}; }
    template <class A>
    G16_HD static void store_point(A* dst, int64_t idx, const Fp2p30& x, const Fp2p30& y, bool identity) {
        Fp<P>* w = reinterpret_cast<Fp<P>*>(dst + idx);
        const int k = lane_hi() ? 1 : 0;
        Fp<P> xw = Fp<P>::zero(), yw = Fp<P>::zero();
        if (!identity) { x.c.pack(xw.v); y.c.pack(yw.v); }
        w[k] = xw;
        w[2 + k] = yw;
    }
    typedef Fp2x30<P> Raw;
#ifndef G16_PAIR_MIN_WAVES
#define G16_PAIR_MIN_WAVES 2
#endif
    static constexpr int ACC_MIN_WAVES = G16_PAIR_MIN_WAVES;
    static constexpr bool ACC_PREFETCH = false;
    static constexpr int LANES_PER_TASK = 2;
    template <class A>
    G16_HD static bool load_point(const A* bases, int64_t idx, Fp2p30& px, Fp2p30& py) {
        const Fp<P>* w = reinterpret_cast<const Fp<P>*>(bases + idx);
        const int k = lane_hi() ? 1 : 0;
        const Fp<P> xw = w[k], yw = w[2 + k];
        const bool zero_half = xw.is_zero() && yw.is_zero();
        if (both(zero_half)) return false;
        px.c = B::unpack(xw.v);
        py.c = B::unpack(yw.v);
        return true;
    }
    typedef Fp<P> PackedC;
    template <class A>
    G16_HD static bool load_point_py(const A* bases, int64_t idx, Fp2p30& px, PackedC& yout) {
        const Fp<P>* w = reinterpret_cast<const Fp<P>*>(bases + idx);
        const int k = lane_hi() ? 1 : 0;
        const Fp<P> xw = w[k], yw = w[2 + k];
        const bool zero_half = xw.is_zero() && yw.is_zero();
        if (both(zero_half)) return false;
        px.c = B::unpack(xw.v);
        yout = yw;
        return true;
    }
    G16_HD static Fp2p30 unpack_cond_neg(const PackedC& y, bool flip) { return {B::unpack_cond_neg(y, flip)}; }
};

template <class R>
struct alignas(16) AccRaw {
    R x, y, zz, zzz;
};

template <class F>
struct Acc30 {
    typedef typename F::Std StdF;
    F x, y, zz, zzz;
    bool inf;

    G16_HD static Acc30 identity() {
        Acc30 a;
        a.x = a.y = a.zz = a.zzz = F::zero();
        a.inf = true;
        return a;
    }
    G16_HD void set_double(const F& px, const F& py) {
        const F U = py.dbl();
        if (U.is_zero_exact()) { inf = true; return; }
        const F V = U.sqr();
        const F W = U.mul(V);
        const F S = px.mul(V);
        const F X2 = px.sqr();
        const F M = X2.dbl().add(X2);
        const F X3 = M.sqr().template sub<F::K2M>(S.dbl());
        const F Y3 = F::mul_sub(M, S.template sub<F::KX>(X3), py, W);
        x = X3; y = Y3; zz = V; zzz = W;
        inf = false;
    }
    G16_HD void add_affine(const F& px, const F& py) {
        if (inf) {
            x = px; y = py; zz = F::one(); zzz = F::one();
            inf = false;
            return;
        }
        const F U2 = px.mul(zz);
        const F S2 = py.mul(zzz);
        const F Pd = U2.template sub<F::KX>(x);
        const F R = S2.template sub<F::KY>(y);
        if (Pd.maybe_zero()) {
            if (Pd.is_zero_exact()) {
                if (R.is_zero_exact()) set_double(px, py);
                else inf = true;
                return;
            }
        }
        const F PP = Pd.sqr();
        const F PPP = Pd.mul(PP);
        const F Q = x.mul(PP);
        const F X3 = R.sqr().template sub<F::KM>(PPP).template sub<F::K2M>(Q.dbl());
        const F Y3 = F::mul_sub(R, Q.template sub<F::KX>(X3), y, PPP);
        x = X3;
        y = Y3;
        zz = zz.mul(PP);
        zzz = zzz.mul(PPP);
    }
    G16_HD void dbl() {
        if (inf) return;
        const F U = y.dbl();
        if (U.is_zero_exact()) { inf = true; return; }
        const F V = U.sqr();
        const F W = U.mul(V);
        const F S = x.mul(V);
        const F X2 = x.sqr();
        const F M = X2.dbl().add(X2);
        const F X3 = M.sqr().template sub<F::K2M>(S.dbl());
        const F Y3 = F::mul_sub(M, S.template sub<F::KX>(X3), y, W);
        x = X3; y = Y3;
        zz = V.mul(zz);
        zzz = W.mul(zzz);
    }
    G16_HD void add(const Acc30& o) {
        if (o.inf) return;
        if (inf) { *this = o; return; }
        const F U1 = x.mul(o.zz);
        const F U2 = o.x.mul(zz);
        const F S1 = y.mul(o.zzz);
        const F S2 = o.y.mul(zzz);
        const F Pd = U2.template sub<F::KM>(U1);
        const F R = S2.template sub<F::KM>(S1);
        if (Pd.maybe_zero()) {
            if (Pd.is_zero_exact()) {
                if (R.is_zero_exact()) dbl();
                else inf = true;
                return;
            }
        }
        const F PP = Pd.sqr();
        const F PPP = Pd.mul(PP);
        const F Q = U1.mul(PP);
        const F X3 = R.sqr().template sub<F::KM>(PPP).template sub<F::K2M>(Q.dbl());
        const F Y3 = F::mul_sub(R, Q.template sub<F::KX>(X3), S1, PPP);
        x = X3;
        y = Y3;
        zz = zz.mul(o.zz).mul(PP);
        zzz = zzz.mul(o.zzz).mul(PPP);
    }
    G16_HD Acc30 mul_small(uint32_t k) const {
        Acc30 acc = identity();
        for (int i = 31; i >= 0; --i) {
            acc.dbl();
            if ((k >> i) & 1) acc.add(*this);
        }
        return acc;
    }
    G16_HD void store_raw(AccRaw<typename F::Raw>* dst) const {
        typedef typename F::Raw R;
        if constexpr (F::LANES_PER_TASK == 1) {
            static_assert(sizeof(F) == sizeof(R), "one-lane fields share the raw layout");
            F* w = reinterpret_cast<F*>(dst);
            w[0] = x; w[1] = y; w[2] = inf ? F::zero() : zz; w[3] = zzz;
        } else {
            typedef typename F::B B30;
            B30* w = reinterpret_cast<B30*>(dst);
            const int k = F::lane_hi() ? 1 : 0;
            w[0 + k] = x.c; w[2 + k] = y.c; w[4 + k] = inf ? B30::zero() : zz.c; w[6 + k] = zzz.c;
        }
    }
    G16_HD static Acc30 load_raw(const AccRaw<typename F::Raw>& p) {
        Acc30 a;
        if constexpr (F::LANES_PER_TASK == 1) {
            const F* w = reinterpret_cast<const F*>(&p);
            a.x = w[0]; a.y = w[1]; a.zz = w[2]; a.zzz = w[3];
            a.inf = a.zz.raw_zero();
        } else {
            typedef typename F::B B30;
            const B30* w = reinterpret_cast<const B30*>(&p);
            const int k = F::lane_hi() ? 1 : 0;
            a.x.c = w[0 + k]; a.y.c = w[2 + k]; a.zz.c = w[4 + k]; a.zzz.c = w[6 + k];
            a.inf = F::both(a.zz.c.raw_zero());
        }
        return a;
    }
    G16_HD void store_std(XYZZ<StdF>* dst) const {
        if constexpr (F::LANES_PER_TASK == 1) {
            *dst = to_std();
        } else {
            typedef typename F::B B30;
            typedef typename B30::Std W;
            W* w = reinterpret_cast<W*>(dst);
            const int k = F::lane_hi() ? 1 : 0;
            const W z = W::zero();
            w[0 + k] = inf ? z : x.c.to_std();
            w[2 + k] = inf ? z : y.c.to_std();
            w[4 + k] = inf ? z : zz.c.to_std();
            w[6 + k] = inf ? z : zzz.c.to_std();
        }
    }
    G16_HD void store_packed(XYZZ<StdF>* dst) const {
        if constexpr (F::LANES_PER_TASK == 1) {
// ... 164 lines not shown
```

### groth16_amd/csrc/internal.hpp

```cpp
#pragma once
#include <hip/hip_runtime.h>
#include <atomic>
#include <cstdint>
#include <cstdio>
#include <cstring>
#include <string>
#include <vector>
#include "../../include/g16_mi355x.h"
#include "curve.hpp"

namespace g16 {

void set_last_error(const char* what, hipError_t e, const char* file, int line);

#define G16_HIP_TRY(expr)                                                     \
    do {                                                                      \
        hipError_t e__ = (expr);                                              \
        if (e__ != hipSuccess) {                                              \
            ::g16::set_last_error(#expr, e__, __FILE__, __LINE__);            \
            return e__ == hipErrorOutOfMemory ? G16_ERR_OOM : G16_ERR_HIP;    \
        }                                                                     \
    } while (0)

#define G16_TRY(expr)                  \
// ... 30 lines not shown
    int start(hipStream_t s) {
        if (!a) { G16_HIP_TRY(hipEventCreate(&a)); G16_HIP_TRY(hipEventCreate(&b)); }
        used = true;
        G16_HIP_TRY(hipEventRecord(a, s));
        return G16_OK;
    }
    int stop(hipStream_t s) { G16_HIP_TRY(hipEventRecord(b, s)); return G16_OK; }
    double ms() {
        if (!used) return 0.0;
        float t = 0.f;
        if (hipEventElapsedTime(&t, a, b) != hipSuccess) return 0.0;
        return (double)t;
    }
    void destroy() { if (a) { (void)hipEventDestroy(a); (void)hipEventDestroy(b); a = b = nullptr; } }
};

template <class C>
struct Domain {
    typedef typename C::Fr Fr;
    int log_n = 0;
    size_t n = 0;
    Fr* tw_fwd = nullptr;
    Fr* tw_inv = nullptr;
    Fr* s1_br = nullptr;
    Fr* s2 = nullptr;
    Fr* g_pow = nullptr;
    Fr n_inv, zinv;
};
template <class C> int domain_create(int log_n, hipStream_t st, Domain<C>** out);
template <class C> void domain_destroy(Domain<C>* d);
template <class C> int domain_ensure_gpow(Domain<C>* d, hipStream_t st);

template <class C> int ntt_dif(const Domain<C>* d, typename C::Fr* data, bool inverse, hipStream_t st);
template <class C> int ntt_dif_quotient(const Domain<C>* d, typename C::Fr* a, const typename C::Fr* b, const typename C::Fr* c,
                                        const typename C::Fr& zinv, bool inverse, hipStream_t st);
template <class C> int ntt_dit(const Domain<C>* d, typename C::Fr* data, bool inverse, const typename C::Fr* prescale, hipStream_t st);
template <class C> int ntt_dif_dit(const Domain<C>* d, typename C::Fr* data, bool dif_inverse, const typename C::Fr* prescale, hipStream_t st);
template <class C> int ntt_dif_batch(const Domain<C>* d, typename C::Fr* const* data, int nbatch, bool inverse, hipStream_t st);
template <class C> int ntt_dit_batch(const Domain<C>* d, typename C::Fr* const* data, int nbatch, bool inverse, const typename C::Fr* prescale,
                                     hipStream_t st);
template <class C> int ntt_dif_dit_batch(const Domain<C>* d, typename C::Fr* const* data, int nbatch, bool dif_inverse,
                                         const typename C::Fr* prescale, hipStream_t st);
template <class C> int bitrev_scale(const Domain<C>* d, typename C::Fr* out, const typename C::Fr* in, const typename C::Fr* table,
                                    const typename C::Fr* cst, hipStream_t st);
template <class C> int scale_by_table(typename C::Fr* data, const typename C::Fr* table, size_t n, hipStream_t st);
template <class C> int gen_power_table(typename C::Fr* out, size_t n, const typename C::Fr& base, const typename C::Fr& scale, bool r30_form,
                                       hipStream_t st);

template <class C>
struct DeviceCircuit {
    typedef typename C::Fr Fr;
    uint64_t num_inputs = 0, num_constraints = 0, num_variables = 0;
    uint64_t* row_ptr[3] = {nullptr, nullptr, nullptr};
    uint32_t* col[3] = {nullptr, nullptr, nullptr};
    Fr* val[3] = {nullptr, nullptr, nullptr};
    uint64_t nnz[3] = {0, 0, 0};
    Domain<C>* dom = nullptr;
    static constexpr int Z_CHUNKS = 8;
    uint64_t need_col[Z_CHUNKS] = {};
};
struct ZUpload {
    const void* host = nullptr;
    hipStream_t copy_stream = nullptr;
    hipEvent_t landed[8] = {};
    int pieces = 0;
};
template <class C> int mark_unit_coefficients(DeviceCircuit<C>* ck, hipStream_t st);
template <class C> int witness_map_device(const DeviceCircuit<C>* ck, const typename C::Fr* d_z, typename C::Fr* d_h, Arena& arena,
                                          hipStream_t st, EventTimer* ntt_timers = nullptr, ZUpload* up = nullptr);

template <class C>
struct DistWm {
    typedef typename C::Fr Fr;
    int rank = 0, world = 1, log_world = 0;
    size_t M = 0, blk = 0;
    Domain<C>* dom_m = nullptr;
    Fr* tw1 = nullptr;
    Fr* sc_mid = nullptr;
    Fr* tw2 = nullptr;
    Fr* sc_out = nullptr;
    Fr wn_fwd[8], wn_inv[8];
    Fr zinv;
};
template <class C> int dwm_create(const DeviceCircuit<C>* ck, int rank, int world, hipStream_t st, DistWm<C>** out);
template <class C> void dwm_destroy(DistWm<C>* d);
template <class C> int dwm_stage(const DeviceCircuit<C>* ck, const DistWm<C>* dw, int stage, const typename C::Fr* d_z,
                                 typename C::Fr* const work[3], typename C::Fr* const recv[3], typename C::Fr* h_local, hipStream_t st);

struct MsmPlan {
    int c = 0;
    int W = 0;
    int groups = 0;
    bool merged = false;
    uint32_t B = 0;
    uint32_t Lmax = 0;
    int affine_levels = 0;
    uint32_t chunk = 0;
    uint32_t K[10];
    int shard_n = 1, shard_r = 0;
    uint32_t buckets() const { return B * (uint32_t)groups; }
    uint32_t G = 8;
    uint32_t chunk_buckets() const { return B >= G ? G : B; }
    uint32_t chunks() const { return B / chunk_buckets(); }
    int chunk_bits() const { int k = 0; while ((1u << k) < chunks()) ++k; return k; }
    int planes() const { return 2 + chunk_bits(); }
    int outputs() const { return groups * planes(); }
};
static constexpr int MSM_MAX_OUTPUTS = 256;
static constexpr int MSM_MERGED_MIN_C = 9, MSM_MERGED_MAX_C = 20;
static constexpr uint64_t MSM_MERGED_MAX_N = (uint64_t)1 << 26;
int make_msm_plan(uint64_t n, int scalar_bits, const uint32_t* modulus_words, int mod_nwords, int merged_c, MsmPlan* plan, int shard_n = 1,
                  int shard_r = 0);
int msm_window_override();
int merged_window_bits(uint64_t n, int scalar_bits, const uint32_t* modulus_words, int mod_nwords);
int msm_plan_windows(int c, int scalar_bits, const uint32_t* modulus_words, int mod_nwords);

struct ScalarSort {
    MsmPlan plan;
    uint64_t n = 0;
    uint32_t* sorted = nullptr;
    uint32_t* offsets = nullptr;
    uint32_t* task_off = nullptr;
    uint32_t* heavy = nullptr;
    uint32_t max_tasks = 0;
    uint32_t max_segments = 0;
    uint64_t max_sorted = 0;
};
template <class C> int sort_scalars(const typename C::Fr* d_scalars, uint64_t n, int merged_c, Arena& arena, hipStream_t st, ScalarSort* out,
                                    int shard_n = 1, int shard_r = 0);

template <class F>
struct MsmBuffers {
    void* partials = nullptr;
    void* chunk_out = nullptr;
    XYZZ<F>* window_sums = nullptr;
};
template <class F> int msm_bucket_pass(const Affine<F>* d_bases, int64_t shift, uint64_t base_count, const ScalarSort& ss, Arena& arena,
                                       hipStream_t st, MsmBuffers<F>* out, EventTimer* bucket_timer);
template <class F>
struct PassJob {
    const Affine<F>* bases;
    int64_t shift;
    uint64_t base_count;
    const ScalarSort* ss;
    MsmBuffers<F>* out;
};
template <class F> int msm_bucket_pass_batch(const PassJob<F>* jobs, int n, Arena& arena, hipStream_t st, EventTimer* bucket_timer);
template <class F> int msm_reduce(const MsmBuffers<F>& buf, const ScalarSort& ss, hipStream_t st);
template <class F> int msm_reduce_batch(const MsmBuffers<F>* const* bufs, const ScalarSort* const* sorts, int n, hipStream_t st, bool heavy_done);
template <class F> int msm_heavy_reduce(const MsmBuffers<F>& buf, const ScalarSort& ss, hipStream_t st);
template <class F> int msm_heavy_reduce_batch(const MsmBuffers<F>* const* bufs, const ScalarSort* const* sorts, int n, hipStream_t st);
template <class F> int convert_bases(Affine<F>* d_bases, uint64_t n, hipStream_t st);
template <class F> XYZZ<F> fold_windows(const XYZZ<F>* window_sums, const MsmPlan& plan);
template <class F> int build_window_tables(const Affine<F>* d_src, uint64_t n, int c, int W, Affine<F>* d_table, hipStream_t st, void* park = nullptr);
template <class F> size_t window_table_park_bytes(uint64_t n, int W);

template <class C>
int generate_parameters_device(hipStream_t st, Arena& arena, const g16_csr_view abc[3], uint64_t ni, uint64_t nc, uint64_t nv,
                               const g16_toxic_waste* tw, const uint64_t* g1_gen, const uint64_t* g2_gen, const g16_params_view* out);
template <class C>
int qap_evaluations_host(const g16_csr_view abc[3], uint64_t ni, uint64_t nc, uint64_t nv, const uint64_t* t, uint64_t* a_out, uint64_t* b_out,
                         uint64_t* c_out, uint64_t* zt_out);

int serialize_points(int curve, int g2, int compressed, const uint64_t* points, uint64_t n, uint8_t* out);
int deserialize_points(int curve, int g2, int compressed, const uint8_t* in, uint64_t n, int validate, uint64_t* points_out);
uint64_t serialized_point_size(int curve, int g2, int compressed);

int mad_rate_device(hipStream_t st, double* mad_per_s);
template <class C> int synth_bases_device(int g2, uint64_t seed, uint64_t first, uint64_t n, void* out_dev, hipStream_t st);

}
```

### groth16_amd/csrc/key_load.hpp

```cpp
#pragma once
#include "api_types.hpp"

namespace {

template <class C>
struct KeyLoader {
    typedef typename C::Fr Fr;
    typedef typename C::Fq Fq;
    typedef typename C::Fq2 Fq2;
    typedef typename C::G1A G1A;
    typedef typename C::G2A G2A;
    typedef typename C::G1X G1X;
    typedef typename C::G2X G2X;
    static constexpr int L = Fq::N / 2;

    struct LoadScratch {
        void* park = nullptr;
        size_t park_bytes = 0;
        struct Staged { void* p; hipEvent_t built; };
        std::vector<Staged> staged;
        void reap(bool wait) {
            size_t keep = 0;
            for (Staged& st : staged) {
                if (wait ? ((void)hipEventSynchronize(st.built), true) : hipEventQuery(st.built) == hipSuccess) {
                    (void)hipFree(st.p);
                    (void)hipEventDestroy(st.built);
                } else {
                    staged[keep++] = st;
                }
            }
            staged.resize(keep);
        }
        void release() {
            reap(true);
            (void)hipFree(park);
            park = nullptr;
            park_bytes = 0;
        }
        int alloc(void** out, size_t bytes) {
            if (hipMalloc(out, bytes) == hipSuccess) return G16_OK;
            (void)hipGetLastError();
            if (staged.empty()) return G16_ERR_OOM;
            reap(true);
            return hipMalloc(out, bytes) == hipSuccess ? G16_OK : G16_ERR_OOM;
        }
    };

    template <class F>
    static int load_query(g16_ctx* ctx, const g16_query& q, bool dev_ptrs, int c, Affine<F>** out, LoadScratch& ls) {
        typedef Affine<F> P;
        *out = nullptr;
        if (q.count == 0) return G16_OK;
        if (!q.points) return G16_ERR_BAD_ARG;
        if (c == 0) {
            if (hipMalloc((void**)out, q.count * sizeof(P)) != hipSuccess) return G16_ERR_OOM;
            G16_HIP_TRY(hipMemcpyAsync(*out, q.points, q.count * sizeof(P), dev_ptrs ? hipMemcpyDeviceToDevice : hipMemcpyHostToDevice,
                                       ctx->stream));
            return convert_bases<F>(*out, q.count, ctx->stream);
        }
        uint32_t modw[Fr::N];
        for (int i = 0; i < Fr::N; ++i) modw[i] = Fr::Params::mod(i);
        const int W = msm_plan_windows(c, Fr::Params::BITS, modw, Fr::N);
        if (W <= 0) return G16_ERR_INTERNAL;
        const char* cap = getenv("G16_PK_TABLE_BUDGET_MB");
        if (cap && (double)q.count * sizeof(P) * W > atof(cap) * 1048576.0) return G16_ERR_OOM;
        if (ls.alloc((void**)out, q.count * sizeof(P) * (size_t)W) != G16_OK) return G16_ERR_OOM;
        const P* src = reinterpret_cast<const P*>(q.points);
        P* staged = nullptr;
        if (!dev_ptrs) {
            if (ls.alloc((void**)&staged, q.count * sizeof(P)) != G16_OK) return G16_ERR_OOM;
            G16_HIP_TRY(hipMemcpyAsync(staged, q.points, q.count * sizeof(P), hipMemcpyHostToDevice, ctx->stream));
            src = staged;
        }
        const size_t need = window_table_park_bytes<F>(q.count, W);
        if (need > ls.park_bytes) {
            if (ls.park) {
                G16_HIP_TRY(hipStreamSynchronize(ctx->stream));
                (void)hipFree(ls.park);
                ls.park = nullptr;
                ls.park_bytes = 0;
            }
            if (ls.alloc(&ls.park, need) != G16_OK) { if (staged) (void)hipFree(staged); return G16_ERR_OOM; }
            ls.park_bytes = need;
        }
        const int rc = build_window_tables<F>(src, q.count, c, W, *out, ctx->stream, ls.park);
        if (staged) {
            hipEvent_t ev = nullptr;
            if (hipEventCreateWithFlags(&ev, hipEventDisableTiming) != hipSuccess || hipEventRecord(ev, ctx->stream) != hipSuccess) {
                (void)hipStreamSynchronize(ctx->stream);
                (void)hipFree(staged);
                if (ev) (void)hipEventDestroy(ev);
            } else {
                ls.staged.push_back({staged, ev});
            }
        }
        return rc;
    }

    static void pk_free(DevicePk<C>* p) {
        if (!p) return;
        (void)hipFree(p->a); (void)hipFree(p->b_g1); (void)hipFree(p->b_g2); (void)hipFree(p->h); (void)hipFree(p->l);
        delete p;
    }

    static int pk_load(g16_ctx* ctx, const g16_pk_view* v, g16_pk** out, int shard_n = 1, int shard_r = 0) {
        if (!v->alpha_g1 || !v->beta_g1 || !v->delta_g1 || !v->beta_g2 || !v->delta_g2 || !v->a_query0 || !v->b_g1_query0 ||
            !v->b_g2_query0)
            return G16_ERR_BAD_ARG;
        DevicePk<C>* p = new (std::nothrow) DevicePk<C>();
        if (!p) return G16_ERR_OOM;
        p->glue->alpha_g1 = load_pod<G1A>(v->alpha_g1);
        p->glue->beta_g1 = load_pod<G1A>(v->beta_g1);
        p->glue->delta_g1 = load_pod<G1A>(v->delta_g1);
        p->glue->beta_g2 = load_pod<G2A>(v->beta_g2);
        p->glue->delta_g2 = load_pod<G2A>(v->delta_g2);
        p->glue->a_query0 = load_pod<G1A>(v->a_query0);
        p->glue->b_g1_query0 = load_pod<G1A>(v->b_g1_query0);
        p->glue->b_g2_query0 = load_pod<G2A>(v->b_g2_query0);
        const bool dev = (v->flags & G16_PK_DEVICE_PTRS) != 0;
        int rc = G16_OK;
        uint32_t modw[Fr::N];
        for (int i = 0; i < Fr::N; ++i) modw[i] = Fr::Params::mod(i);
        const uint64_t nz = std::max(std::max(v->a.count, v->b_g1.count), std::max(v->b_g2.count, v->l.count));
        if (std::max(nz, (uint64_t)v->h.count) >= ((uint64_t)1 << 27)) {
            delete p;
            g_last_error = "a proving-key shard holds 2^27 or more points of one query: shard it over more ranks";
            return G16_ERR_BAD_LENGTH;
        }
        p->c_z = merged_window_bits(nz, Fr::Params::BITS, modw, Fr::N);
        p->c_h = merged_window_bits(v->h.count, Fr::Params::BITS, modw, Fr::N);
        if (v->h.count == 0) p->c_h = p->c_z;
        if (nz == 0) p->c_z = p->c_h;
        if (p->c_z == 0 || p->c_h == 0) {
            const char* e = getenv("G16_MSM_PRECOMP");
            p->table_fallback = (nz || v->h.count) ? ((e && atoi(e) == 0) ? 1 : 2) : 0;
            p->c_z = p->c_h = 0;
        }
        p->shard_n = shard_n;
        p->shard_r = shard_r;
        if (shard_n > 1) {
            if (v->a.start || v->b_g1.start || v->b_g2.start || v->h.start || v->l.start) {
                delete p;
                g_last_error = "a bucket-space shard is loaded from the WHOLE key (every query.start == 0): the ranks divide the buckets, not the bases";
                return G16_ERR_BAD_ARG;
            }
            if (p->c_z == 0) {
                delete p;
                g_last_error = "a bucket-space shard needs the key's window tables (merged windows): G16_MSM_PRECOMP=0 or an over-long query rules them out";
                return G16_ERR_BAD_ARG;
            }
        }
        LoadScratch ls;
        for (int attempt = 0; attempt < 2; ++attempt) {
            const int cz = p->c_z, ch = p->c_h;
            if ((rc = load_query<Fq2>(ctx, v->b_g2, dev, cz, &p->b_g2, ls)) || (rc = load_query<Fq>(ctx, v->a, dev, cz, &p->a, ls)) ||
                (rc = load_query<Fq>(ctx, v->b_g1, dev, cz, &p->b_g1, ls)) || (rc = load_query<Fq>(ctx, v->l, dev, cz, &p->l, ls)) ||
                (rc = load_query<Fq>(ctx, v->h, dev, ch, &p->h, ls))) {
                (void)hipStreamSynchronize(ctx->stream);
                ls.release();
                (void)hipFree(p->a); (void)hipFree(p->b_g1); (void)hipFree(p->b_g2); (void)hipFree(p->h); (void)hipFree(p->l);
                p->a = p->b_g1 = p->h = p->l = nullptr;
                p->b_g2 = nullptr;
                if (rc == G16_ERR_OOM && cz != 0 && shard_n <= 1) {
                    (void)hipGetLastError();
                    p->c_z = p->c_h = 0;
                    p->table_fallback = 3;
                    continue;
                }
                if (rc == G16_ERR_OOM && shard_n > 1)
                    g_last_error = "the whole key's window tables do not fit on this GPU: a bucket-space shard cannot be held (use base-range shards)";
                pk_free(p);
                return rc;
            }
            break;
        }
        p->a_start = v->a.start; p->a_count = v->a.count;
        p->b_g1_start = v->b_g1.start; p->b_g1_count = v->b_g1.count;
        p->b_g2_start = v->b_g2.start; p->b_g2_count = v->b_g2.count;
        p->h_start = v->h.start; p->h_count = v->h.count;
        p->l_start = v->l.start; p->l_count = v->l.count;
        {
            const uint64_t rows_z = p->c_z ? (uint64_t)msm_plan_windows(p->c_z, Fr::Params::BITS, modw, Fr::N) : 1;
            const uint64_t rows_h = p->c_h ? (uint64_t)msm_plan_windows(p->c_h, Fr::Params::BITS, modw, Fr::N) : 1;
            p->table_bytes = rows_z * ((v->a.count + v->b_g1.count + v->l.count) * sizeof(G1A) + v->b_g2.count * sizeof(G2A)) +
                             rows_h * v->h.count * sizeof(G1A);
        }
        const bool load_ok = hipStreamSynchronize(ctx->stream) == hipSuccess;
        ls.release();
        if (!load_ok) { pk_free(p); return G16_ERR_HIP; }
        g16_pk* h = new (std::nothrow) g16_pk{C::CURVE_ID, ctx, p};
        if (!h) { pk_free(p); return G16_ERR_OOM; }
        *out = h;
        return G16_OK;
    }

    static void circuit_free(DeviceCircuit<C>* dc) {
        if (!dc) return;
        for (int m = 0; m < 3; ++m) { (void)hipFree(dc->row_ptr[m]); (void)hipFree(dc->col[m]); (void)hipFree(dc->val[m]); }
        domain_destroy<C>(dc->dom);
        delete dc;
    }

    static int circuit_load(g16_ctx* ctx, const g16_csr_view abc[3], uint64_t num_inputs, uint64_t num_constraints, uint64_t num_variables,
                            g16_circuit** out) {
        if (num_inputs == 0 || num_variables < num_inputs) return G16_ERR_BAD_LENGTH;
        const uint64_t need = num_constraints + num_inputs;
        int log_n = 0;
        while (((uint64_t)1 << log_n) < need) {
            ++log_n;
            if (log_n > 40) return G16_ERR_DEGREE_TOO_LARGE;
        }
        if (log_n > C::TWO_ADICITY) return G16_ERR_DEGREE_TOO_LARGE;
        if (log_n > 30) return G16_ERR_DEGREE_TOO_LARGE;
        DeviceCircuit<C>* dc = new (std::nothrow) DeviceCircuit<C>();
        if (!dc) return G16_ERR_OOM;
        dc->num_inputs = num_inputs;
        dc->num_constraints = num_constraints;
        dc->num_variables = num_variables;
        auto fail = [&](int code) { circuit_free(dc); return code; };
        for (int m = 0; m < 3; ++m) {
            if (!abc[m].row_ptr) return fail(G16_ERR_BAD_ARG);
            if (abc[m].row_ptr[0] != 0) return fail(G16_ERR_BAD_LENGTH);
            for (uint64_t i = 0; i < num_constraints; ++i)
                if (abc[m].row_ptr[i] > abc[m].row_ptr[i + 1]) return fail(G16_ERR_BAD_LENGTH);
            const uint64_t nnz = abc[m].row_ptr[num_constraints];
            dc->nnz[m] = nnz;
            if (nnz && (!abc[m].col || !abc[m].val)) return fail(G16_ERR_BAD_ARG);
            for (uint64_t k = 0; k < nnz; ++k)
                if (abc[m].col[k] >= num_variables) return fail(G16_ERR_BAD_LENGTH);
            if (hipMalloc((void**)&dc->row_ptr[m], (num_constraints + 1) * sizeof(uint64_t)) != hipSuccess) return fail(G16_ERR_OOM);
            if (hipMalloc((void**)&dc->col[m], (nnz ? nnz : 1) * sizeof(uint32_t)) != hipSuccess) return fail(G16_ERR_OOM);
            if (hipMalloc((void**)&dc->val[m], (nnz ? nnz : 1) * sizeof(Fr)) != hipSuccess) return fail(G16_ERR_OOM);
            if (hipMemcpyAsync(dc->row_ptr[m], abc[m].row_ptr, (num_constraints + 1) * sizeof(uint64_t), hipMemcpyHostToDevice, ctx->stream) !=
                hipSuccess)
                return fail(G16_ERR_HIP);
            if (nnz) {
                if (hipMemcpyAsync(dc->col[m], abc[m].col, nnz * sizeof(uint32_t), hipMemcpyHostToDevice, ctx->stream) != hipSuccess)
                    return fail(G16_ERR_HIP);
                if (hipMemcpyAsync(dc->val[m], abc[m].val, nnz * sizeof(Fr), hipMemcpyHostToDevice, ctx->stream) != hipSuccess)
                    return fail(G16_ERR_HIP);
            }
        }
        {
            constexpr int ZC = DeviceCircuit<C>::Z_CHUNKS;
            const uint64_t n_dom = (uint64_t)1 << log_n;
            uint64_t run = 0;
            for (int k = 0; k < ZC; ++k) {
                const uint64_t r_lo = n_dom * (uint64_t)k / ZC, r_hi = n_dom * (uint64_t)(k + 1) / ZC;
                for (int m = 0; m < 3; ++m) {
                    const uint64_t a = std::min(r_lo, num_constraints), b = std::min(r_hi, num_constraints);
                    for (uint64_t e = abc[m].row_ptr[a]; e < abc[m].row_ptr[b]; ++e) run = std::max<uint64_t>(run, abc[m].col[e]);
                }
                if (r_hi > num_constraints && num_inputs) run = std::max(run, std::min(r_hi - num_constraints, num_inputs) - 1);
                dc->need_col[k] = run;
            }
        }
        int rc = mark_unit_coefficients<C>(dc, ctx->stream);
        if (rc) return fail(rc);
        rc = domain_create<C>(log_n, ctx->stream, &dc->dom);
        if (rc) return fail(rc);
        if (hipStreamSynchronize(ctx->stream) != hipSuccess) return fail(G16_ERR_HIP);
        g16_circuit* h = new (std::nothrow) g16_circuit{C::CURVE_ID, ctx, dc, (uint64_t)1 << log_n};
        if (!h) return fail(G16_ERR_OOM);
        *out = h;
        return G16_OK;
    }

};

}
```

### groth16_amd/csrc/msm.hip

```cpp
#include "internal.hpp"
#include "msm_common.hpp"
#include "fp30.hpp"
#include "batch_affine.hpp"
#include "window_tables.hpp"
#include <algorithm>
#include <cstdlib>

namespace g16 {

static constexpr int SORT_THREADS = 1024;
static constexpr int ACC_THREADS = 64;
static constexpr int RED_THREADS = 64;
static constexpr int WIN_THREADS = 256;
#ifndef G16_REDUCE_G
#define G16_REDUCE_G 8
#endif
static constexpr uint32_t REDUCE_G = G16_REDUCE_G;

struct PlanDev {
    int c, W;
    uint32_t B;
    uint32_t K[10];
    uint32_t shard_n, shard_r, shard_magic;
};

__device__ __forceinline__ bool shard_local_key(const PlanDev& plan, uint32_t* key) {
    if (plan.shard_n <= 1) return true;
    const uint32_t q = __umulhi(*key, plan.shard_magic);
    if (*key - q * plan.shard_n != plan.shard_r) return false;
    *key = q;
    return true;
}

template <class Fr>
__global__ __launch_bounds__(256) void digits_kernel(const Fr* __restrict__ scalars, uint64_t n, PlanDev plan,
                                                     uint16_t* __restrict__ planes) {
    __shared__ uint32_t sw[MSM_SWORDS][256];
    const uint64_t i = (uint64_t)blockIdx.x * 256 + threadIdx.x;
    if (i >= n) return;
    uint32_t s[Fr::N];
    scalars[i].to_canonical(s);
    uint64_t carry = 0;
    G16_UNROLL for (int k = 0; k < 10; ++k) {
        carry += (uint64_t)(k < Fr::N ? s[k] : 0u) + plan.K[k];
        sw[k][threadIdx.x] = (uint32_t)carry;
        carry >>= 32;
    }
    sw[10][threadIdx.x] = 0;
    for (int w = 0; w < plan.W; ++w) {
        const int bit = w * plan.c, word = bit >> 5, sh = bit & 31;
        const uint64_t two = (uint64_t)sw[word][threadIdx.x] | ((uint64_t)sw[word + 1][threadIdx.x] << 32);
        planes[(uint64_t)w * n + i] = (uint16_t)((uint32_t)(two >> sh) & ((1u << plan.c) - 1u));
    }
}

static __global__ __launch_bounds__(SORT_THREADS) void bucket_count_kernel(const uint16_t* __restrict__ planes, uint64_t n, uint32_t chunk,
                                                                    int c, uint32_t B, uint32_t* __restrict__ counts) {
    extern __shared__ __attribute__((aligned(16))) unsigned char smem[];
    uint32_t* hist = reinterpret_cast<uint32_t*>(smem);
    const int w = blockIdx.y;
    for (uint32_t b = threadIdx.x; b < B; b += SORT_THREADS) hist[b] = 0;
    __syncthreads();
    const uint64_t lo = (uint64_t)blockIdx.x * chunk, hi = min(n, lo + chunk);
    const uint16_t* plane = planes + (uint64_t)w * n;
    for (uint64_t p = lo + threadIdx.x; p < hi; p += SORT_THREADS) {
        uint32_t bucket, neg;
        if (digit_to_bucket(plane[p], c, &bucket, &neg)) atomicAdd(&hist[bucket], 1u);
    }
    __syncthreads();
    uint32_t* out = counts + (uint64_t)w * B;
    for (uint32_t b = threadIdx.x; b < B; b += SORT_THREADS) {
        const uint32_t v = hist[b];
        if (v) atomicAdd(&out[b], v);
    }
}

static constexpr int CLASS_THREADS = 256;
static constexpr int MAX_CLASSES = 64;
static constexpr uint32_t SORT_CLASS_LOG = 13;
static constexpr int SORT_M_THREADS = 256;

template <class Fr>
__device__ __forceinline__ void biased_scalar(const Fr& sc, const PlanDev& plan, uint32_t (*sw)[CLASS_THREADS]) {
    uint32_t s[Fr::N];
    sc.to_canonical(s);
    uint64_t carry = 0;
    G16_UNROLL for (int k = 0; k < 10; ++k) {
        carry += (uint64_t)(k < Fr::N ? s[k] : 0u) + plan.K[k];
        sw[k][threadIdx.x] = (uint32_t)carry;
        carry >>= 32;
    }
    sw[10][threadIdx.x] = 0;
}
__device__ __forceinline__ uint32_t window_of(const uint32_t (*sw)[CLASS_THREADS], int w, int c) {
    const int bit = w * c, word = bit >> 5, sh = bit & 31;
    const uint64_t two = (uint64_t)sw[word][threadIdx.x] | ((uint64_t)sw[word + 1][threadIdx.x] << 32);
    return (uint32_t)(two >> sh) & ((1u << c) - 1u);
}

template <class Fr>
__global__ __launch_bounds__(CLASS_THREADS) void class_count_kernel(const Fr* __restrict__ scalars, uint64_t n, PlanDev plan, uint32_t blog,
                                                                    uint32_t Q, uint32_t* __restrict__ block_counts) {
    __shared__ uint32_t sw[MSM_SWORDS][CLASS_THREADS];
    __shared__ uint32_t cnt[MAX_CLASSES];
    if (threadIdx.x < MAX_CLASSES) cnt[threadIdx.x] = 0;
    __syncthreads();
    const uint64_t i = (uint64_t)blockIdx.x * CLASS_THREADS + threadIdx.x;
    if (i < n) {
        biased_scalar(scalars[i], plan, sw);
        for (int w = 0; w < plan.W; ++w) {
            uint32_t key, neg;
            if (digit_to_bucket(window_of(sw, w, plan.c), plan.c, &key, &neg) && shard_local_key(plan, &key)) atomicAdd(&cnt[key >> blog], 1u);
        }
    }
    __syncthreads();
    if (threadIdx.x < Q) block_counts[(uint64_t)threadIdx.x * gridDim.x + blockIdx.x] = cnt[threadIdx.x];
}

template <class Fr>
__global__ __launch_bounds__(CLASS_THREADS) void class_partition_kernel(const Fr* __restrict__ scalars, uint64_t n, PlanDev plan, uint32_t blog,
                                                                        uint32_t Q, const uint32_t* __restrict__ block_off,
                                                                        uint16_t* __restrict__ ent_key, uint32_t* __restrict__ ent_tag) {
    __shared__ uint32_t sw[MSM_SWORDS][CLASS_THREADS];
    __shared__ uint32_t cur[MAX_CLASSES];
    if (threadIdx.x < Q) cur[threadIdx.x] = block_off[(uint64_t)threadIdx.x * gridDim.x + blockIdx.x];
    __syncthreads();
    const uint64_t i = (uint64_t)blockIdx.x * CLASS_THREADS + threadIdx.x;
    if (i >= n) return;
    biased_scalar(scalars[i], plan, sw);
    for (int w = 0; w < plan.W; ++w) {
        uint32_t key, neg;
        if (digit_to_bucket(window_of(sw, w, plan.c), plan.c, &key, &neg) && shard_local_key(plan, &key)) {
            const uint32_t pos = atomicAdd(&cur[key >> blog], 1u);
            ent_key[pos] = (uint16_t)((key & ((1u << blog) - 1u)) | (neg << 15));
            ent_tag[pos] = (uint32_t)i | ((uint32_t)w << 26);
        }
    }
}

static __global__ __launch_bounds__(SORT_M_THREADS) void bucket_count_merged_kernel(const uint16_t* __restrict__ ent_key,
                                                                           const uint32_t* __restrict__ class_off, uint32_t nb, uint32_t B,
                                                                           uint32_t* __restrict__ wg_counts) {
    extern __shared__ __attribute__((aligned(16))) unsigned char smem[];
    uint32_t* hist = reinterpret_cast<uint32_t*>(smem);
    const uint32_t q = blockIdx.y;
    const uint32_t lo = class_off[(uint64_t)q * nb], hi = class_off[(uint64_t)(q + 1) * nb];
    for (uint32_t b = threadIdx.x; b < B; b += SORT_M_THREADS) hist[b] = 0;
    __syncthreads();
    for (uint64_t p = (uint64_t)lo + blockIdx.x * SORT_M_THREADS + threadIdx.x; p < hi; p += (uint64_t)gridDim.x * SORT_M_THREADS)
        atomicAdd(&hist[ent_key[p] & 0x7fffu], 1u);
    __syncthreads();
    uint32_t* out = wg_counts + ((uint64_t)q * gridDim.x + blockIdx.x) * B;
    for (uint32_t b = threadIdx.x; b < B; b += SORT_M_THREADS) out[b] = hist[b];
}

static __global__ __launch_bounds__(256) void bucket_wg_scan_kernel(uint32_t* __restrict__ wg_counts, uint32_t G, uint32_t B, uint32_t M,
                                                                    uint32_t* __restrict__ counts) {
    const uint32_t i = blockIdx.x * 256 + threadIdx.x;
    if (i >= M) return;
// ... 65 lines not shown
                                                                          uint32_t* __restrict__ prefix) {
    __shared__ uint32_t sa[SCAN_THREADS];
    uint32_t carry = 0;
    for (uint32_t base = 0; base < nblocks; base += SCAN_THREADS) {
        const uint32_t i = base + threadIdx.x;
        const uint32_t a = i < nblocks ? block_sums[i] : 0u;
        uint32_t tot;
        const uint32_t ea = block_exclusive(a, sa, &tot);
        if (i < nblocks) block_sums[i] = carry + ea;
        carry += tot;
    }
    if (threadIdx.x == 0) prefix[M] = carry;
}

static __global__ __launch_bounds__(SCAN_THREADS) void scan_write_kernel(const uint32_t* __restrict__ vals, uint32_t M, uint32_t pad,
                                                                  const uint32_t* __restrict__ block_base, uint32_t* __restrict__ prefix) {
    __shared__ uint32_t sa[SCAN_THREADS];
    const uint32_t base = blockIdx.x * SCAN_TILE + threadIdx.x * SCAN_PER_THREAD;
    uint32_t cv[SCAN_PER_THREAD], sum = 0, tot;
    G16_UNROLL for (int j = 0; j < SCAN_PER_THREAD; ++j) { cv[j] = (base + j < M) ? ((vals[base + j] + pad) & ~pad) : 0u; sum += cv[j]; }
    uint32_t a = block_base[blockIdx.x] + block_exclusive(sum, sa, &tot);
    G16_UNROLL for (int j = 0; j < SCAN_PER_THREAD; ++j) {
        if (base + j < M) { prefix[base + j] = a; a += cv[j]; }
    }
}

static __global__ void bucket_slots_kernel(const uint32_t* __restrict__ offsets, uint32_t M, uint32_t off_shift, uint32_t lseg,
                                    uint32_t* __restrict__ nparts, uint32_t* __restrict__ heavy ) {
    const uint32_t b = blockIdx.x * blockDim.x + threadIdx.x;
    if (b >= M) return;
    const uint32_t lo = offsets[b] >> off_shift, hi = offsets[b + 1] >> off_shift;
    const uint32_t np = hi > lo ? ((hi - 1) / lseg - lo / lseg + 1u) : 0u;
    nparts[b] = np;
    if (np > HEAVY_PARTS) heavy[1 + atomicAdd(&heavy[0], 1u)] = b;
}

static __global__ __launch_bounds__(SORT_THREADS) void bucket_scatter_kernel(const uint16_t* __restrict__ planes, uint64_t n, uint32_t chunk,
                                                                      int c, uint32_t B, const uint32_t* __restrict__ offsets,
                                                                      uint32_t* __restrict__ cursor, uint32_t* __restrict__ sorted) {
    extern __shared__ __attribute__((aligned(16))) unsigned char smem[];
    uint32_t* hist = reinterpret_cast<uint32_t*>(smem);
    const int w = blockIdx.y;
    for (uint32_t b = threadIdx.x; b < B; b += SORT_THREADS) hist[b] = 0;
    __syncthreads();
    const uint64_t lo = (uint64_t)blockIdx.x * chunk, hi = min(n, lo + chunk);
    const uint16_t* plane = planes + (uint64_t)w * n;
    for (uint64_t p = lo + threadIdx.x; p < hi; p += SORT_THREADS) {
        uint32_t bucket, neg;
        if (digit_to_bucket(plane[p], c, &bucket, &neg)) atomicAdd(&hist[bucket], 1u);
    }
    __syncthreads();
    const uint64_t wb = (uint64_t)w * B;
    for (uint32_t b = threadIdx.x; b < B; b += SORT_THREADS) {
        const uint32_t v = hist[b];
        if (v) hist[b] = offsets[wb + b] + atomicAdd(&cursor[wb + b], v);
    }
    __syncthreads();
    for (uint64_t p = lo + threadIdx.x; p < hi; p += SORT_THREADS) {
        uint32_t bucket, neg;
        if (digit_to_bucket(plane[p], c, &bucket, &neg)) {
            const uint32_t pos = atomicAdd(&hist[bucket], 1u);
            sorted[pos] = (uint32_t)p | (neg << 31);
        }
    }
}

template <class F30>
struct LdsAccStore {
    static constexpr int NL = F30::PREFIX_LIMBS;
    static constexpr int QUADS = NL / 4, TAIL = NL % 4;
    static constexpr int WORDS_PER_VALUE = NL * ACC_THREADS;
    uint32_t* quad;
    uint32_t* tail;
    __device__ __forceinline__ F30 ld(int v) const {
        asm volatile("" ::: "memory");
        uint32_t w[NL];
        const uint32_t* q = quad + v * WORDS_PER_VALUE;
        G16_UNROLL for (int g = 0; g < QUADS; ++g) {
            const uint4 t = *reinterpret_cast<const uint4*>(q + g * 4 * ACC_THREADS);
            w[4 * g] = t.x; w[4 * g + 1] = t.y; w[4 * g + 2] = t.z; w[4 * g + 3] = t.w;
        }
        const uint32_t* r = tail + v * WORDS_PER_VALUE;
        G16_UNROLL for (int i = 0; i < TAIL; ++i) w[4 * QUADS + i] = r[i * ACC_THREADS];
        return F30::from_limbs(w);
    }
    __device__ __forceinline__ void st(int v, const F30& a) const {
        uint32_t w[NL];
        a.get_limbs(w);
        uint32_t* q = quad + v * WORDS_PER_VALUE;
        G16_UNROLL for (int g = 0; g < QUADS; ++g)
            *reinterpret_cast<uint4*>(q + g * 4 * ACC_THREADS) = make_uint4(w[4 * g], w[4 * g + 1], w[4 * g + 2], w[4 * g + 3]);
        uint32_t* r = tail + v * WORDS_PER_VALUE;
        G16_UNROLL for (int i = 0; i < TAIL; ++i) r[i * ACC_THREADS] = w[4 * QUADS + i];
        asm volatile("" ::: "memory");
    }
};

template <class F30>
struct RawAccStore {
    AccRaw<typename F30::Raw>* p;
    __device__ __forceinline__ F30 ld(int k) const {
        asm volatile("" ::: "memory");
        if constexpr (F30::LANES_PER_TASK == 1) {
            static_assert(sizeof(F30) == sizeof(typename F30::Raw), "one-lane fields share the raw layout");
            return reinterpret_cast<const F30*>(p)[k];
        } else {
            typedef typename F30::B B30;
            return F30{reinterpret_cast<const B30*>(p)[2 * k + (F30::lane_hi() ? 1 : 0)]};
        }
    }
    __device__ __forceinline__ void st(int k, const F30& a) const {
        if constexpr (F30::LANES_PER_TASK == 1) {
            reinterpret_cast<F30*>(p)[k] = a;
        } else {
            typedef typename F30::B B30;
            reinterpret_cast<B30*>(p)[2 * k + (F30::lane_hi() ? 1 : 0)] = a.c;
        }
        asm volatile("" ::: "memory");
    }
    __device__ __forceinline__ bool inf() const {
        const F30 zz = ld(2);
        if constexpr (F30::LANES_PER_TASK == 1) return zz.raw_zero();
        else return F30::both(zz.c.raw_zero());
    }
    __device__ __forceinline__ void set_inf() const { st(2, F30::zero()); }
};
template <class F30>
struct RegAccStore {
    F30 v[4];
    __device__ __forceinline__ F30 ld(int k) const { return v[k]; }
    __device__ __forceinline__ void st(int k, const F30& a) { v[k] = a; }
};
template <class F30, class St>
__device__ __forceinline__ Acc30<F30> gather_acc(const St& st, bool inf) {
    Acc30<F30> a;
    a.inf = inf;
    if (inf) { a.x = a.y = a.zz = a.zzz = F30::zero(); return a; }
    a.x = st.ld(0); a.y = st.ld(1); a.zz = st.ld(2); a.zzz = st.ld(3);
    return a;
}

static constexpr int PASS_BATCH = 4;
template <class F30>
struct PassBatch {
    const Affine<typename F30::Std>* bases[PASS_BATCH];
    int64_t shift[PASS_BATCH];
    uint64_t base_count[PASS_BATCH];
    const uint32_t* sorted[PASS_BATCH];
    const uint32_t* offsets[PASS_BATCH];
    const uint32_t* slot_off[PASS_BATCH];
    AccRaw<typename F30::Raw>* partials[PASS_BATCH];
};

template <class F30, bool DIRECT>
__global__ __launch_bounds__(ACC_THREADS, F30::ACC_MIN_WAVES) void bucket_accumulate30_kernel(
    PassBatch<F30> batch, uint32_t M, uint32_t off_shift, uint32_t lseg, uint32_t merged) {
    const Affine<typename F30::Std>* __restrict__ bases = batch.bases[blockIdx.y];
    const int64_t shift = batch.shift[blockIdx.y];
    const uint64_t base_count = batch.base_count[blockIdx.y];
    const uint32_t* __restrict__ sorted = batch.sorted[blockIdx.y];
    const uint32_t* __restrict__ offsets = batch.offsets[blockIdx.y];
    const uint32_t* __restrict__ slot_off = batch.slot_off[blockIdx.y];
    AccRaw<typename F30::Raw>* __restrict__ partials = batch.partials[blockIdx.y];
    const uint32_t t = (blockIdx.x * ACC_THREADS + threadIdx.x) / F30::LANES_PER_TASK;
    const uint32_t S = offsets[M] >> off_shift;
    const uint64_t start64 = (uint64_t)t * lseg;
    if (start64 >= S) return;
    const uint32_t start = (uint32_t)start64;
    const uint32_t end = (uint32_t)min((uint64_t)S, start64 + lseg);
    uint32_t lo = 0, hi = M;
    while (hi - lo > 1) {
        const uint32_t mid = (lo + hi) >> 1;
        if ((offsets[mid] >> off_shift) <= start) lo = mid; else hi = mid;
    }
    uint32_t b = lo, b_first = offsets[b] >> off_shift, b_end = offsets[b + 1] >> off_shift;
    __shared__ __attribute__((aligned(16))) uint32_t acc_lds[4 * F30::PREFIX_LIMBS * ACC_THREADS];
    AccParked<F30, LdsAccStore<F30>> acc;
    acc.s.quad = acc_lds + 4 * threadIdx.x;
    acc.s.tail = acc_lds + 4 * LdsAccStore<F30>::QUADS * ACC_THREADS + threadIdx.x;
    acc.inf = true;
    auto flush = [&](AccRaw<typename F30::Raw>* dst) { acc.gather().store_raw(dst); acc.inf = true; };
    uint32_t v_next = 0;
    typedef typename F30::PackedC YNext;
    F30 px_next = F30::zero();
    YNext py_next = YNext::zero();
    bool ok_next = false;
    auto decode = [&](uint32_t v, int64_t* at) -> bool {
        const uint32_t pt = merged ? (v & 0x3ffffffu) : (v & 0x7fffffffu);
        const uint64_t row = merged ? (uint64_t)((v >> 26) & 31u) * base_count : 0;
        const int64_t idx = (int64_t)pt + shift;
        *at = (int64_t)row + idx;
        return idx >= 0 && (uint64_t)idx < base_count;
    };
    auto fetch = [&](uint32_t v) {
        v_next = DIRECT ? 0u : v;
        int64_t at = (int64_t)v;
        ok_next = DIRECT ? true : decode(v, &at);
        if (ok_next) ok_next = F30::load_point_py(bases, at, px_next, py_next);
    };
    fetch(DIRECT ? start : sorted[start]);
    uint32_t v_fetch = DIRECT ? start + 1 : (start + 1 < end ? sorted[start + 1] : 0u);
    for (uint32_t e = start; e < end; ++e) {
        if (e == b_end) {
            flush(&partials[slot_off[b] + (t - b_first / lseg)]);
            do { ++b; b_end = offsets[b + 1] >> off_shift; } while (b_end <= e);
            b_first = offsets[b] >> off_shift;
        }
        const uint32_t v = v_next;
        const F30 px = px_next;
        YNext py = py_next;
        const bool ok = ok_next;
        auto advance = [&]() {
            if (e + 1 < end) fetch(v_fetch);
            if constexpr (DIRECT) v_fetch = e + 2;
            else v_fetch = e + 2 < end ? sorted[e + 2] : 0u;
        };
        if constexpr (F30::ACC_PREFETCH) advance();
        if (ok) acc.add_affine_packed(px, py, (v >> 31) != 0);
        if constexpr (!F30::ACC_PREFETCH) advance();
    }
    flush(&partials[slot_off[b] + (t - b_first / lseg)]);
}

static constexpr int AFF_THREADS = 128;
template <class F30, bool LEVEL0>
__global__ __launch_bounds__(AFF_THREADS, 2) void affine_level_kernel(AffineLevelArgs<F30> args) {
    const uint32_t wave = (blockIdx.x * AFF_THREADS + threadIdx.x) >> 6;
    AffineLevel<F30, LEVEL0>::run(args, wave, threadIdx.x & 63u);
}

template <class P> G16_HD Fp<P> to_r30(const Fp<P>& x) { return Fp30<P>::std_to_r30(x); }
template <class P> G16_HD Fp2<P> to_r30(const Fp2<P>& x) { return {Fp30<P>::std_to_r30(x.c0), Fp30<P>::std_to_r30(x.c1)}; }

template <class F>
__global__ void convert_bases30_kernel(Affine<F>* __restrict__ pts, uint64_t n) {
    const uint64_t i = (uint64_t)blockIdx.x * blockDim.x + threadIdx.x;
    if (i >= n) return;
    Affine<F> a = pts[i];
    a.x = to_r30(a.x);
    a.y = to_r30(a.y);
    pts[i] = a;
}

template <class F> struct Lazy30;
template <class P> struct Lazy30<Fp<P>> { typedef Fp30<P> type; };
template <class P> struct Lazy30<Fp2<P>> { typedef Fp2p30<P> type; };

static constexpr int HEAVY_THREADS = 128;
#ifndef G16_FIRST_STAGE_WAVES
#define G16_FIRST_STAGE_WAVES 2
#endif
static constexpr int HEAVY_BLOCKS = 512;

static constexpr int REDUCE_BATCH = 4;
template <class Raw, class X>
struct ReduceBatch {
    Raw* partials[REDUCE_BATCH];
    const uint32_t* slot_off[REDUCE_BATCH];
    const uint32_t* heavy[REDUCE_BATCH];
    Raw* chunk_out[REDUCE_BATCH];
    X* window_sums[REDUCE_BATCH];
};

template <class F30>
__global__ __launch_bounds__(HEAVY_THREADS, F30::LANES_PER_TASK == 1 ? G16_FIRST_STAGE_WAVES : 2) void heavy_reduce_kernel(ReduceBatch<AccRaw<typename F30::Raw>, XYZZ<typename F30::Std>> batch) {
    extern __shared__ __attribute__((aligned(16))) unsigned char smem[];
    AccRaw<typename F30::Raw>* sh = reinterpret_cast<AccRaw<typename F30::Raw>*>(smem);
    constexpr uint32_t LPT = F30::LANES_PER_TASK, TASKS = HEAVY_THREADS / LPT;
    AccRaw<typename F30::Raw>* __restrict__ partials = batch.partials[blockIdx.y];
    const uint32_t* __restrict__ slot_off = batch.slot_off[blockIdx.y];
    const uint32_t* __restrict__ heavy = batch.heavy[blockIdx.y];
    const uint32_t nheavy = heavy[0], task = threadIdx.x / LPT;
    for (uint32_t i = blockIdx.x; i < nheavy; i += gridDim.x) {
        const uint32_t b = heavy[1 + i];
        const uint32_t t0 = slot_off[b], t1 = slot_off[b + 1];
        __syncthreads();
        const RawAccStore<F30> mine{&sh[task]};
        bool inf = true;
        for (uint32_t q = t0 + task; q < t1; q += TASKS) {
            const RawAccStore<F30> src{&partials[q]};
            acc_add_streamed<F30>(mine, inf, src, src.inf());
        }
        if (inf) mine.set_inf();
        __syncthreads();
        for (uint32_t d = TASKS / 2; d > 0; d >>= 1) {
            if (task < d) {
                const RawAccStore<F30> other{&sh[task + d]};
                bool mi = mine.inf();
                const bool was = mi;
                acc_add_streamed<F30>(mine, mi, other, other.inf());
                if (mi && !was) mine.set_inf();
            }
            __syncthreads();
        }
        if (task == 0) Acc30<F30>::load_raw(sh[0]).store_raw(&partials[t0]);
    }
}

template <class F30>
__global__ __launch_bounds__(RED_THREADS, F30::LANES_PER_TASK == 1 ? G16_FIRST_STAGE_WAVES : 2) void bucket_combine_kernel(ReduceBatch<AccRaw<typename F30::Raw>, XYZZ<typename F30::Std>> batch, uint32_t M) {
    AccRaw<typename F30::Raw>* __restrict__ partials = batch.partials[blockIdx.y];
    const uint32_t* __restrict__ slot_off = batch.slot_off[blockIdx.y];
    const uint32_t b = (blockIdx.x * RED_THREADS + threadIdx.x) / F30::LANES_PER_TASK;
    if (b >= M) return;
    const uint32_t t0 = slot_off[b], np = slot_off[b + 1] - t0;
    if (np < 2 || np > HEAVY_PARTS) return;
    const RawAccStore<F30> mine{&partials[t0]};
    bool inf = mine.inf();
    const bool was = inf;
    for (uint32_t q = 1; q < np; ++q) {
        const RawAccStore<F30> src{&partials[t0 + q]};
        acc_add_streamed<F30>(mine, inf, src, src.inf());
    }
    if (inf && !was) mine.set_inf();
}

template <class F30>
__global__ __launch_bounds__(RED_THREADS, 2) void bucket_reduce_kernel(ReduceBatch<AccRaw<typename F30::Raw>, XYZZ<typename F30::Std>> batch, uint32_t B, int W,
                                                                    uint32_t G) {
    const AccRaw<typename F30::Raw>* __restrict__ partials = batch.partials[blockIdx.y];
    const uint32_t* __restrict__ slot_off = batch.slot_off[blockIdx.y];
    const uint32_t cpw = B / G;
    AccRaw<typename F30::Raw>* __restrict__ chunk_out = batch.chunk_out[blockIdx.y];
    AccRaw<typename F30::Raw>* __restrict__ chunk_sum = chunk_out + (size_t)cpw * W;
    const uint32_t t = (blockIdx.x * RED_THREADS + threadIdx.x) / F30::LANES_PER_TASK;
    if (t >= cpw * (uint32_t)W) return;
    const uint32_t w = t / cpw, ch = t % cpw, b_lo = ch * G;
    constexpr bool PAIR = F30::LANES_PER_TASK == 2;
    constexpr int SLOTS = PAIR ? 8 : 4;
    __shared__ __attribute__((aligned(16))) uint32_t red_lds[SLOTS * F30::PREFIX_LIMBS * RED_THREADS];
    static_assert(RED_THREADS == ACC_THREADS, "LdsAccStore is laid out for ACC_THREADS lanes");
    LdsAccStore<F30> tot_s;
    tot_s.quad = red_lds + 4 * threadIdx.x;
    tot_s.tail = red_lds + 4 * LdsAccStore<F30>::QUADS * RED_THREADS + threadIdx.x;
    typename std::conditional<PAIR, LdsAccStore<F30>, RegAccStore<F30>>::type run_s;
    if constexpr (PAIR) {
        run_s.quad = tot_s.quad + 4 * LdsAccStore<F30>::WORDS_PER_VALUE;
        run_s.tail = tot_s.tail + 4 * LdsAccStore<F30>::WORDS_PER_VALUE;
    }
    bool run_inf = true, tot_inf = true;
    for (uint32_t bb = G; bb-- > 0;) {
        const uint32_t gb = w * B + b_lo + bb;
        const uint32_t t0 = slot_off[gb];
        if (slot_off[gb + 1] != t0) {
            const RawAccStore<F30> src{const_cast<AccRaw<typename F30::Raw>*>(&partials[t0])};
            acc_add_streamed<F30>(run_s, run_inf, src, src.inf());
        }
        acc_add_streamed<F30>(tot_s, tot_inf, run_s, run_inf);
    }
    gather_acc<F30>(run_s, run_inf).store_raw(&chunk_sum[t]);
    gather_acc<F30>(tot_s, tot_inf).store_raw(&chunk_out[t]);
}

template <class F30>
__global__ __launch_bounds__(WIN_THREADS, 2) void window_reduce_kernel(ReduceBatch<AccRaw<typename F30::Raw>, XYZZ<typename F30::Std>> batch, uint32_t cpw) {
    extern __shared__ __attribute__((aligned(16))) unsigned char smem[];
    AccRaw<typename F30::Raw>* sh = reinterpret_cast<AccRaw<typename F30::Raw>*>(smem);
    constexpr uint32_t LPT = F30::LANES_PER_TASK, TASKS = WIN_THREADS / LPT;
    const uint32_t w = blockIdx.x, p = blockIdx.y, task = threadIdx.x / LPT;
    const AccRaw<typename F30::Raw>* __restrict__ chunk_out = batch.chunk_out[blockIdx.z];
    const AccRaw<typename F30::Raw>* __restrict__ chunk_sum = chunk_out + (size_t)cpw * gridDim.x;
    XYZZ<typename F30::Std>* __restrict__ window_sums = batch.window_sums[blockIdx.z];
    const AccRaw<typename F30::Raw>* src = (p == 0 ? chunk_out : chunk_sum) + (uint64_t)w * cpw;
    const uint32_t mask = p >= 2 ? 1u << (p - 2) : 0u;
    const RawAccStore<F30> mine{&sh[task]};
    bool inf = true;
    for (uint32_t j = task; j < cpw; j += TASKS)
        if (!mask || (j & mask)) {
            const RawAccStore<F30> s_j{const_cast<AccRaw<typename F30::Raw>*>(&src[j])};
            acc_add_streamed<F30>(mine, inf, s_j, s_j.inf());
        }
// ... 212 lines not shown
    G16_HIP_TRY(hipMemsetAsync(counts, 0, ((size_t)2 * M + 1) * sizeof(uint32_t), st));
    PlanDev pd;
    pd.c = plan.c; pd.W = plan.W; pd.B = plan.B;
    for (int k = 0; k < 10; ++k) pd.K[k] = plan.K[k];
    pd.shard_n = (uint32_t)plan.shard_n;
    pd.shard_r = (uint32_t)plan.shard_r;
    pd.shard_magic = plan.shard_n > 1 ? (uint32_t)((((uint64_t)1 << 32) + (uint64_t)plan.shard_n - 1) / (uint64_t)plan.shard_n) : 0u;
    const size_t lds = (size_t)Bs * sizeof(uint32_t);
    static PerDeviceOnce attr_once;
    std::atomic<bool>& attr_set = attr_once.flag();
    if (!attr_set) {
        G16_HIP_TRY(hipFuncSetAttribute(reinterpret_cast<const void*>(&bucket_count_kernel), hipFuncAttributeMaxDynamicSharedMemorySize,
                                        128 * 1024));
        G16_HIP_TRY(hipFuncSetAttribute(reinterpret_cast<const void*>(&bucket_scatter_kernel), hipFuncAttributeMaxDynamicSharedMemorySize,
                                        128 * 1024));
        G16_HIP_TRY(hipFuncSetAttribute(reinterpret_cast<const void*>(&bucket_count_merged_kernel),
                                        hipFuncAttributeMaxDynamicSharedMemorySize, 128 * 1024));
        G16_HIP_TRY(hipFuncSetAttribute(reinterpret_cast<const void*>(&bucket_scatter_merged_kernel),
                                        hipFuncAttributeMaxDynamicSharedMemorySize, 128 * 1024));
        attr_set = true;
    }
    const unsigned nchunks = (unsigned)((n + plan.chunk - 1) / plan.chunk);
    const uint32_t blog = plan.merged ? slog : (uint32_t)ilog2(plan.B);
    const uint32_t max_scan = std::max(M, plan.merged ? Q * nb : 0u);
    G16_TRY(arena.alloc_n((size_t)(max_scan + SCAN_TILE - 1) / SCAN_TILE, &block_sums));
    auto prefix_scan = [&](const uint32_t* vals, uint32_t* prefix, uint32_t count, uint32_t padmask = 0) -> int {
        const uint32_t nblocks = (count + SCAN_TILE - 1) / SCAN_TILE;
        hipLaunchKernelGGL(scan_block_sums_kernel, dim3(nblocks), dim3(SCAN_THREADS), 0, st, vals, count, padmask, block_sums);
        G16_LAUNCH_CHECK();
        hipLaunchKernelGGL(scan_block_offsets_kernel, dim3(1), dim3(SCAN_THREADS), 0, st, block_sums, nblocks, count, prefix);
        G16_LAUNCH_CHECK();
        hipLaunchKernelGGL(scan_write_kernel, dim3(nblocks), dim3(SCAN_THREADS), 0, st, vals, count, padmask, block_sums, prefix);
        G16_LAUNCH_CHECK();
        return G16_OK;
    };
    unsigned gx = std::max(1u, std::min(std::min(4096u / Q, 256u), (unsigned)((nw + SORT_M_THREADS - 1) / SORT_M_THREADS)));
    if (const char* e = getenv("G16_SORT_GX")) {
        const int v = atoi(e);
        if (v >= 1 && v <= 4096) gx = (unsigned)v;
    }
    uint32_t* wg_counts = nullptr;
    if (plan.merged) G16_TRY(arena.alloc_n((size_t)Q * gx * Bs, &wg_counts));
    if (n) {
        if (plan.merged) {
            hipLaunchKernelGGL((class_count_kernel<Fr>), dim3(nb), dim3(CLASS_THREADS), 0, st, d_scalars, n, pd, blog, Q, class_cnt);
            G16_LAUNCH_CHECK();
            G16_TRY(prefix_scan(class_cnt, class_off, Q * nb));
            hipLaunchKernelGGL((class_partition_kernel<Fr>), dim3(nb), dim3(CLASS_THREADS), 0, st, d_scalars, n, pd, blog, Q, class_off, planes,
                               ent_tag);
            G16_LAUNCH_CHECK();
            hipLaunchKernelGGL(bucket_count_merged_kernel, dim3(gx, Q), dim3(SORT_M_THREADS), lds, st, planes, class_off, nb, Bs, wg_counts);
            G16_LAUNCH_CHECK();
            hipLaunchKernelGGL(bucket_wg_scan_kernel, dim3((M + 255) / 256), dim3(256), 0, st, wg_counts, gx, Bs, M, counts);
        } else {
            hipLaunchKernelGGL((digits_kernel<Fr>), dim3((unsigned)((n + 255) / 256)), dim3(256), 0, st, d_scalars, n, pd, planes);
            G16_LAUNCH_CHECK();
            hipLaunchKernelGGL(bucket_count_kernel, dim3(nchunks, plan.W), dim3(SORT_THREADS), lds, st, planes, n, plan.chunk, plan.c, plan.B,
                               counts);
        }
        G16_LAUNCH_CHECK();
    }
    G16_TRY(prefix_scan(counts, out->offsets, M, pad));
    hipLaunchKernelGGL(bucket_slots_kernel, dim3((M + 255) / 256), dim3(256), 0, st, out->offsets, M, (uint32_t)R, plan.Lmax, nparts,
                       out->heavy);
    G16_LAUNCH_CHECK();
    G16_TRY(prefix_scan(nparts, out->task_off, M));
    if (n) {
        if (plan.merged)
            hipLaunchKernelGGL(bucket_scatter_merged_kernel, dim3(gx, Q), dim3(SORT_M_THREADS), lds, st, planes, ent_tag, class_off, nb, Bs,
                               out->offsets, wg_counts, out->sorted);
        else
            hipLaunchKernelGGL(bucket_scatter_kernel, dim3(nchunks, plan.W), dim3(SORT_THREADS), lds, st, planes, n, plan.chunk, plan.c, plan.B,
                               out->offsets, cursor, out->sorted);
        G16_LAUNCH_CHECK();
    }
    return G16_OK;
}

template <class F>
static int alloc_msm_buffers(const ScalarSort& ss, Arena& arena, MsmBuffers<F>* out) {
    typedef AccRaw<typename Lazy30<F>::type::Raw> Raw;
    const MsmPlan& plan = ss.plan;
    const uint32_t cpw = plan.B / plan.chunk_buckets();
    Raw *partials = nullptr, *chunk_out = nullptr;
    G16_TRY(arena.alloc_n((size_t)ss.max_tasks ? ss.max_tasks : 1, &partials));
    G16_TRY(arena.alloc_n((size_t)cpw * plan.groups * 2, &chunk_out));
    G16_TRY(arena.alloc_n((size_t)plan.outputs(), &out->window_sums));
    out->partials = partials;
    out->chunk_out = chunk_out;
    return G16_OK;
}

template <class F>
int msm_bucket_pass(const Affine<F>* d_bases, int64_t shift, uint64_t base_count, const ScalarSort& ss, Arena& arena, hipStream_t st,
                    MsmBuffers<F>* out, EventTimer* bucket_timer) {
    typedef typename Lazy30<F>::type F30;
    typedef AccRaw<typename Lazy30<F>::type::Raw> Raw;
    const MsmPlan& plan = ss.plan;
    const uint32_t M = plan.buckets();
    const int R = plan.affine_levels;
    if (!R || !ss.max_sorted) {
        const PassJob<F> job{d_bases, shift, base_count, &ss, out};
        return msm_bucket_pass_batch<F>(&job, 1, arena, st, bucket_timer);
    }
    G16_TRY(alloc_msm_buffers<F>(ss, arena, out));
    Raw* partials = static_cast<Raw*>(out->partials);
    Affine<F>* lists[2] = {nullptr, nullptr};
    Word4* prefix = nullptr;
    constexpr uint32_t T = 64 / F30::LANES_PER_TASK;
    constexpr int QUADS = AffineLevel<F30, true>::QUADS;
    auto level_K = [&](int r) -> uint32_t {
        const uint64_t pairs = ss.max_sorted >> (r + 1);
        uint32_t K = 64;
        while (K > 8 && pairs / ((uint64_t)K * T) < 2048) K >>= 1;
        return K;
    };
    auto level_waves = [&](int r) -> uint64_t { return ((ss.max_sorted >> (r + 1)) + (uint64_t)level_K(r) * T - 1) / ((uint64_t)level_K(r) * T); };
    {
        G16_TRY(arena.alloc_n((size_t)(ss.max_sorted >> 1) + 1, &lists[0]));
        if (R > 1) G16_TRY(arena.alloc_n((size_t)(ss.max_sorted >> 2) + 1, &lists[1]));
        size_t recs = 0;
        for (int r = 0; r < R; ++r) recs = std::max(recs, (size_t)(level_waves(r) * level_K(r)) * QUADS * 64);
        G16_TRY(arena.alloc_n(recs ? recs : 1, &prefix));
    }
    if (bucket_timer) G16_TRY(bucket_timer->start(st));
    {
        AffineLevelArgs<F30> a;
        a.sorted = ss.sorted;
        a.total = ss.offsets + M;
        a.prefix = prefix;
        a.shift = shift;
        a.base_count = base_count;
        a.merged = plan.merged ? 1u : 0u;
        for (int r = 0; r < R; ++r) {
            a.in = r == 0 ? d_bases : lists[(r - 1) & 1];
            a.out = lists[r & 1];
            a.level = (uint32_t)r;
            a.K = level_K(r);
            const uint64_t waves = level_waves(r);
            const unsigned blocks = (unsigned)((waves * 64 + AFF_THREADS - 1) / AFF_THREADS);
            if (r == 0) hipLaunchKernelGGL((affine_level_kernel<F30, true>), dim3(blocks), dim3(AFF_THREADS), 0, st, a);
            else hipLaunchKernelGGL((affine_level_kernel<F30, false>), dim3(blocks), dim3(AFF_THREADS), 0, st, a);
            G16_LAUNCH_CHECK();
        }
    }
    if (ss.max_segments) {
        const uint64_t lanes = (uint64_t)ss.max_segments * F30::LANES_PER_TASK;
        const dim3 grid((unsigned)((lanes + ACC_THREADS - 1) / ACC_THREADS));
        PassBatch<F30> b;
        for (int i = 0; i < PASS_BATCH; ++i) {
            b.bases[i] = lists[(R - 1) & 1]; b.shift[i] = 0; b.base_count[i] = 0; b.sorted[i] = nullptr;
            b.offsets[i] = ss.offsets; b.slot_off[i] = ss.task_off; b.partials[i] = partials;
        }
        hipLaunchKernelGGL((bucket_accumulate30_kernel<F30, true>), grid, dim3(ACC_THREADS), 0, st, b, M, (uint32_t)R, plan.Lmax, 0u);
        G16_LAUNCH_CHECK();
    }
    if (bucket_timer) G16_TRY(bucket_timer->stop(st));
    return G16_OK;
}

template <class F30>
static unsigned pass_lds_pad() {
    static const int want = [] { const char* e = getenv("G16_PASS_WG_PER_CU"); return e ? atoi(e) : 0; }();
    if (want <= 0) return 0;
    const unsigned own = 4u * F30::PREFIX_LIMBS * ACC_THREADS * 4u;
    const unsigned per = (160u * 1024u / (unsigned)want) & ~255u;
    return per > own ? per - own : 0;
}

template <class F>
int msm_bucket_pass_batch(const PassJob<F>* jobs, int n, Arena& arena, hipStream_t st, EventTimer* bucket_timer) {
    typedef typename Lazy30<F>::type F30;
    typedef AccRaw<typename Lazy30<F>::type::Raw> Raw;
    if (n < 1 || n > PASS_BATCH) return G16_ERR_INTERNAL;
    const MsmPlan& plan = jobs[0].ss->plan;
    for (int i = 0; i < n; ++i) {
        const MsmPlan& q = jobs[i].ss->plan;
        if (q.B != plan.B || q.groups != plan.groups || q.Lmax != plan.Lmax || q.merged != plan.merged) return G16_ERR_INTERNAL;
        if (q.affine_levels && jobs[i].ss->max_sorted) return G16_ERR_INTERNAL;
    }
    PassBatch<F30> b;
    uint32_t max_segments = 0;
    for (int i = 0; i < n; ++i) G16_TRY(alloc_msm_buffers<F>(*jobs[i].ss, arena, jobs[i].out));
    for (int i = 0; i < PASS_BATCH; ++i) {
        const PassJob<F>& j = jobs[i < n ? i : 0];
        b.bases[i] = j.bases; b.shift[i] = j.shift; b.base_count[i] = j.base_count; b.sorted[i] = j.ss->sorted;
        b.offsets[i] = j.ss->offsets; b.slot_off[i] = j.ss->task_off; b.partials[i] = static_cast<Raw*>(j.out->partials);
        if (i < n) max_segments = std::max(max_segments, j.ss->max_segments);
    }
    if (bucket_timer) G16_TRY(bucket_timer->start(st));
    if (max_segments) {
        const uint64_t lanes = (uint64_t)max_segments * F30::LANES_PER_TASK;
        const dim3 grid((unsigned)((lanes + ACC_THREADS - 1) / ACC_THREADS), (unsigned)n);
        hipLaunchKernelGGL((bucket_accumulate30_kernel<F30, false>), grid, dim3(ACC_THREADS), pass_lds_pad<F30>(), st, b, plan.buckets(), 0u,
                           plan.Lmax, plan.merged ? 1u : 0u);
        G16_LAUNCH_CHECK();
    }
    if (bucket_timer) G16_TRY(bucket_timer->stop(st));
    return G16_OK;
}

template <class F>
static int reduce_setup(size_t* lds_heavy, size_t* lds_win) {
    typedef typename Lazy30<F>::type F30;
    typedef AccRaw<typename F30::Raw> Raw;
    static PerDeviceOnce attr_once;
    std::atomic<bool>& attr_set = attr_once.flag();
    *lds_heavy = sizeof(Raw) * HEAVY_THREADS / F30::LANES_PER_TASK;
    *lds_win = sizeof(Raw) * WIN_THREADS / F30::LANES_PER_TASK;
    if (!attr_set) {
        G16_HIP_TRY(hipFuncSetAttribute(reinterpret_cast<const void*>(&heavy_reduce_kernel<F30>), hipFuncAttributeMaxDynamicSharedMemorySize,
                                        (int)*lds_heavy));
        G16_HIP_TRY(hipFuncSetAttribute(reinterpret_cast<const void*>(&window_reduce_kernel<F30>), hipFuncAttributeMaxDynamicSharedMemorySize,
                                        (int)*lds_win));
        attr_set = true;
    }
    return G16_OK;
}

template <class F>
static ReduceBatch<AccRaw<typename Lazy30<F>::type::Raw>, XYZZ<F>> make_reduce_batch(const MsmBuffers<F>* const* bufs, const ScalarSort* const* sorts, int n) {
    typedef AccRaw<typename Lazy30<F>::type::Raw> Raw;
    ReduceBatch<Raw, XYZZ<F>> batch;
    for (int i = 0; i < REDUCE_BATCH; ++i) {
        const int k = i < n ? i : 0;
        batch.partials[i] = static_cast<Raw*>(bufs[k]->partials);
        batch.slot_off[i] = sorts[k]->task_off;
        batch.heavy[i] = sorts[k]->heavy;
        batch.chunk_out[i] = static_cast<Raw*>(bufs[k]->chunk_out);
        batch.window_sums[i] = bufs[k]->window_sums;
    }
    return batch;
}

template <class F>
int msm_heavy_reduce_batch(const MsmBuffers<F>* const* bufs, const ScalarSort* const* sorts, int n, hipStream_t st) {
    typedef typename Lazy30<F>::type F30;
    if (n < 1 || n > REDUCE_BATCH) return G16_ERR_INTERNAL;
    const MsmPlan& plan = sorts[0]->plan;
    for (int i = 1; i < n; ++i)
        if (sorts[i]->plan.B != plan.B || sorts[i]->plan.groups != plan.groups) return G16_ERR_INTERNAL;
    size_t lds_heavy, lds_win;
    G16_TRY(reduce_setup<F>(&lds_heavy, &lds_win));
    const auto batch = make_reduce_batch<F>(bufs, sorts, n);
    hipLaunchKernelGGL((heavy_reduce_kernel<F30>), dim3(HEAVY_BLOCKS, n), dim3(HEAVY_THREADS), lds_heavy, st, batch);
    G16_LAUNCH_CHECK();
    const uint32_t M = plan.buckets();
    hipLaunchKernelGGL((bucket_combine_kernel<F30>), dim3((M * F30::LANES_PER_TASK + RED_THREADS - 1) / RED_THREADS, n), dim3(RED_THREADS), 0, st, batch, M);
    G16_LAUNCH_CHECK();
    return G16_OK;
}

template <class F>
int msm_heavy_reduce(const MsmBuffers<F>& buf, const ScalarSort& ss, hipStream_t st) {
    const MsmBuffers<F>* b = &buf;
    const ScalarSort* s = &ss;
    return msm_heavy_reduce_batch<F>(&b, &s, 1, st);
}

template <class F>
int msm_reduce_batch(const MsmBuffers<F>* const* bufs, const ScalarSort* const* sorts, int n, hipStream_t st, bool heavy_done) {
    typedef typename Lazy30<F>::type F30;
    if (n < 1 || n > REDUCE_BATCH) return G16_ERR_INTERNAL;
    const MsmPlan& plan = sorts[0]->plan;
    for (int i = 1; i < n; ++i)
        if (sorts[i]->plan.B != plan.B || sorts[i]->plan.groups != plan.groups) return G16_ERR_INTERNAL;
    const uint32_t G = plan.chunk_buckets();
    const uint32_t cpw = plan.B / G;
    size_t lds_heavy, lds_win;
    G16_TRY(reduce_setup<F>(&lds_heavy, &lds_win));
    const auto batch = make_reduce_batch<F>(bufs, sorts, n);
    if (!heavy_done) G16_TRY((msm_heavy_reduce_batch<F>(bufs, sorts, n, st)));
    hipLaunchKernelGGL((bucket_reduce_kernel<F30>), dim3((cpw * plan.groups * F30::LANES_PER_TASK + RED_THREADS - 1) / RED_THREADS, n), dim3(RED_THREADS), 0,
                       st, batch, plan.B, plan.groups, G);
    G16_LAUNCH_CHECK();
    hipLaunchKernelGGL((window_reduce_kernel<F30>), dim3(plan.groups, plan.planes(), n), dim3(WIN_THREADS), lds_win, st, batch, cpw);
    G16_LAUNCH_CHECK();
    return G16_OK;
}

template <class F>
int msm_reduce(const MsmBuffers<F>& buf, const ScalarSort& ss, hipStream_t st) {
    const MsmBuffers<F>* b = &buf;
    const ScalarSort* s = &ss;
    return msm_reduce_batch<F>(&b, &s, 1, st, false);
}

template <class F>
int convert_bases(Affine<F>* d_bases, uint64_t n, hipStream_t st) {
    if (n == 0) return G16_OK;
    hipLaunchKernelGGL((convert_bases30_kernel<F>), dim3((unsigned)((n + 255) / 256)), dim3(256), 0, st, d_bases, n);
    G16_LAUNCH_CHECK();
    return G16_OK;
}

template <class F>
XYZZ<F> fold_windows(const XYZZ<F>* ws, const MsmPlan& plan) {
    const int NP = plan.planes(), bits = plan.chunk_bits();
    auto group_T = [&](int g) -> XYZZ<F> {
        const XYZZ<F>* P = ws + (size_t)g * NP;
        XYZZ<F> hi = XYZZ<F>::identity();
        for (int k = bits - 1; k >= 0; --k) { hi = hi.dbl(); hi.add(P[2 + k]); }
        for (uint32_t b = plan.chunk_buckets(); b > 1; b >>= 1) hi = hi.dbl();
        hi.add(P[0]);
        return hi;
    };
    XYZZ<F> total = XYZZ<F>::identity();
    if (plan.merged) {
        const int Q = plan.groups;
        if (Q > 1) {
            XYZZ<F> run = XYZZ<F>::identity();
            for (int q = Q - 1; q >= 1; --q) { run.add(ws[(size_t)q * NP + 1]); total.add(run); }
            for (uint32_t b = plan.B; b > 1; b >>= 1) total = total.dbl();
        }
        for (int q = 0; q < Q; ++q) total.add(group_T(q));
        if (plan.shard_n > 1) {
            XYZZ<F> plain = XYZZ<F>::identity();
            for (int q = 0; q < Q; ++q) plain.add(ws[(size_t)q * NP + 1]);
            const uint32_t kn = (uint32_t)plan.shard_n, km = (uint32_t)(plan.shard_n - 1 - plan.shard_r);
            total = total.mul_bits(&kn, 7);
            if (km) total.add(plain.mul_bits(&km, 7).neg());
        }
        return total;
    }
    for (int w = plan.W - 1; w >= 0; --w) {
        for (int k = 0; k < plan.c; ++k) total = total.dbl();
        total.add(group_T(w));
    }
    return total;
}

static constexpr int TABLE_MAX_W = 32;
static constexpr int TABLE_THREADS = 128;
static constexpr uint64_t TABLE_CHUNK = (uint64_t)1 << 18;
template <class F30>
__global__ __launch_bounds__(TABLE_THREADS, 2) void build_window_tables_kernel(const Affine<typename F30::Std>* __restrict__ src, uint64_t first,
                                                                              uint64_t count, uint64_t n, int c, int W,
                                                                              Affine<typename F30::Std>* __restrict__ table, uint32_t* __restrict__ park) {
    typedef TableDeviceIO<F30> IO;
    typedef typename IO::W32 W32;
    const uint64_t lane = (uint64_t)blockIdx.x * TABLE_THREADS + threadIdx.x;
    const uint64_t t = lane / F30::LANES_PER_TASK;
    if (t >= count) return;
    const uint64_t i = first + t;
    IO io{reinterpret_cast<const W32*>(src + i), reinterpret_cast<W32*>(table + i), n * 2 * IO::TL::PARTS, park + lane, count * F30::LANES_PER_TASK};
    window_table_task<F30>(io, c, W);
}

template <class F>
size_t window_table_park_bytes(uint64_t n, int W) {
    typedef typename Lazy30<F>::type F30;
    const uint64_t chunk = std::min(n ? n : 1, TABLE_CHUNK);
    return (size_t)4 * (W > 1 ? W - 1 : 1) * TableLane<F30>::B::NL * chunk * F30::LANES_PER_TASK * sizeof(uint32_t);
}

template <class F>
int build_window_tables(const Affine<F>* d_src, uint64_t n, int c, int W, Affine<F>* d_table, hipStream_t st, void* park_buf) {
    typedef typename Lazy30<F>::type F30;
    static_assert(sizeof(Affine<F>) == 2 * TableLane<F30>::PARTS * sizeof(typename TableLane<F30>::B::Std), "affine point = x parts | y parts");
    if (n == 0) return G16_OK;
    if (W > TABLE_MAX_W) return G16_ERR_INTERNAL;
    const uint64_t chunk = std::min(n, TABLE_CHUNK);
    uint32_t* park = static_cast<uint32_t*>(park_buf);
    if (!park && hipMalloc((void**)&park, window_table_park_bytes<F>(n, W)) != hipSuccess) { (void)hipGetLastError(); return G16_ERR_OOM; }
    int rc = G16_OK;
    for (uint64_t first = 0; first < n && rc == G16_OK; first += chunk) {
        const uint64_t count = std::min(chunk, n - first);
        const uint64_t lanes = count * F30::LANES_PER_TASK;
        hipLaunchKernelGGL((build_window_tables_kernel<F30>), dim3((unsigned)((lanes + TABLE_THREADS - 1) / TABLE_THREADS)), dim3(TABLE_THREADS), 0, st,
                           d_src, first, count, n, c, W, d_table, park);
        if (hipGetLastError() != hipSuccess) rc = G16_ERR_HIP;
    }
    if (!park_buf) {
        if (hipStreamSynchronize(st) != hipSuccess && rc == G16_OK) rc = G16_ERR_HIP;
        (void)hipFree(park);
    }
    return rc;
}

#define G16_INSTANTIATE_MSM(C)                                                                                               \
    template int convert_bases<typename C::Fq>(Affine<typename C::Fq>*, uint64_t, hipStream_t);                             \
    template int convert_bases<typename C::Fq2>(Affine<typename C::Fq2>*, uint64_t, hipStream_t);                           \
    template int sort_scalars<C>(const typename C::Fr*, uint64_t, int, Arena&, hipStream_t, ScalarSort*, int, int);                   \
    template int build_window_tables<typename C::Fq>(const Affine<typename C::Fq>*, uint64_t, int, int, Affine<typename C::Fq>*, hipStream_t, void*);    \
    template int build_window_tables<typename C::Fq2>(const Affine<typename C::Fq2>*, uint64_t, int, int, Affine<typename C::Fq2>*, hipStream_t, void*); \
    template size_t window_table_park_bytes<typename C::Fq>(uint64_t, int);                                                 \
    template size_t window_table_park_bytes<typename C::Fq2>(uint64_t, int);                                                \
    template int msm_bucket_pass<typename C::Fq>(const Affine<typename C::Fq>*, int64_t, uint64_t, const ScalarSort&, Arena&, \
                                                 hipStream_t, MsmBuffers<typename C::Fq>*, EventTimer*);                      \
    template int msm_bucket_pass<typename C::Fq2>(const Affine<typename C::Fq2>*, int64_t, uint64_t, const ScalarSort&,     \
                                                  Arena&, hipStream_t, MsmBuffers<typename C::Fq2>*, EventTimer*);            \
    template int msm_bucket_pass_batch<typename C::Fq>(const PassJob<typename C::Fq>*, int, Arena&, hipStream_t, EventTimer*);   \
    template int msm_bucket_pass_batch<typename C::Fq2>(const PassJob<typename C::Fq2>*, int, Arena&, hipStream_t, EventTimer*); \
    template int msm_reduce<typename C::Fq>(const MsmBuffers<typename C::Fq>&, const ScalarSort&, hipStream_t);             \
    template int msm_reduce_batch<typename C::Fq>(const MsmBuffers<typename C::Fq>* const*, const ScalarSort* const*, int, hipStream_t, bool); \
    template int msm_heavy_reduce<typename C::Fq>(const MsmBuffers<typename C::Fq>&, const ScalarSort&, hipStream_t);     \
    template int msm_heavy_reduce_batch<typename C::Fq>(const MsmBuffers<typename C::Fq>* const*, const ScalarSort* const*, int, hipStream_t); \
    template int msm_reduce<typename C::Fq2>(const MsmBuffers<typename C::Fq2>&, const ScalarSort&, hipStream_t);           \
    template XYZZ<typename C::Fq> fold_windows<typename C::Fq>(const XYZZ<typename C::Fq>*, const MsmPlan&);               \
    template XYZZ<typename C::Fq2> fold_windows<typename C::Fq2>(const XYZZ<typename C::Fq2>*, const MsmPlan&);

#if G16_MSM_PART == 0
G16_INSTANTIATE_MSM(Bls12_381)
#else
G16_INSTANTIATE_MSM(Bn254)
#endif

}
```

### groth16_amd/csrc/unit_api.hpp

```cpp
#pragma once
#include "api_types.hpp"
#include "prover.hpp"

namespace {

template <class C>
struct UnitApi {
    typedef typename C::Fr Fr;
    typedef typename C::Fq Fq;
    typedef typename C::Fq2 Fq2;
    typedef typename C::G1A G1A;
    typedef typename C::G2A G2A;
    typedef typename C::G1X G1X;
    typedef typename C::G2X G2X;
    static constexpr int L = Fq::N / 2;
    static int witness_map_api(g16_ctx* ctx, const g16_circuit* ckh, const uint64_t* z, uint64_t n_assign, int on_device, uint64_t* h_out) {
        const DeviceCircuit<C>* ck = static_cast<const DeviceCircuit<C>*>(ckh->dc);
        if (n_assign != ck->num_variables) return G16_ERR_BAD_LENGTH;
        DrainOnError drain(ctx);
        ctx->reset_arena();
        const Fr* d_z = nullptr;
        G16_TRY(Prover<C>::stage_assignment(ctx, z, n_assign, on_device, &d_z));
        Fr* d_h = nullptr;
        G16_TRY(ctx->arena.alloc_n(ck->dom->n, &d_h));
        G16_TRY((witness_map_device<C>(ck, d_z, d_h, ctx->arena, ctx->stream)));
        G16_HIP_TRY(hipMemcpyAsync(h_out, d_h, ck->dom->n * sizeof(Fr), hipMemcpyDeviceToHost, ctx->stream));
        G16_HIP_TRY(hipStreamSynchronize(ctx->stream));
        drain.dismiss();
        return G16_OK;
    }

    static int dwm_stage_api(g16_ctx* ctx, const g16_circuit* ckh, const void* dwp, int stage, const uint64_t* z, uint64_t n_assign, int on_device,
                             uint64_t* const work[3], uint64_t* const recv[3], uint64_t* h_local, bool async) {
        const DeviceCircuit<C>* ck = static_cast<const DeviceCircuit<C>*>(ckh->dc);
        const DistWm<C>* dw = static_cast<const DistWm<C>*>(dwp);
        DrainOnError drain(ctx);
        const Fr* d_z = nullptr;
        if (stage == 0) {
            if (!z || n_assign != ck->num_variables) return G16_ERR_BAD_LENGTH;
            if (async) {
                if (!on_device) return G16_ERR_BAD_ARG;
                d_z = reinterpret_cast<const Fr*>(z);
            } else {
                ctx->reset_arena();
                G16_TRY(Prover<C>::stage_assignment(ctx, z, n_assign, on_device, &d_z));
            }
        }
        Fr* w[3] = {reinterpret_cast<Fr*>(work[0]), reinterpret_cast<Fr*>(work[1]), reinterpret_cast<Fr*>(work[2])};
        Fr* rv[3] = {reinterpret_cast<Fr*>(recv[0]), reinterpret_cast<Fr*>(recv[1]), reinterpret_cast<Fr*>(recv[2])};
        G16_TRY((dwm_stage<C>(ck, dw, stage, d_z, w, rv, reinterpret_cast<Fr*>(h_local), async ? ctx->stream_wm : ctx->stream)));
        if (!async) G16_HIP_TRY(hipStreamSynchronize(ctx->stream));
        drain.dismiss();
        return G16_OK;
    }

    template <class F>
    static int msm_api(g16_ctx* ctx, const uint64_t* bases, const uint64_t* scalars, uint64_t n, uint64_t* out_affine, int shard_n = 1,
                       int shard_r = 0) {
        typedef Affine<F> A;
        typedef XYZZ<F> X;
        hipStream_t st = ctx->stream;
        DrainOnError drain(ctx);
        ctx->reset_arena();
        A* d_b = nullptr;
        Fr* d_s = nullptr;
        G16_TRY(ctx->arena.alloc_n(n ? n : 1, &d_b));
        G16_TRY(ctx->arena.alloc_n(n ? n : 1, &d_s));
        if (n) {
            G16_HIP_TRY(hipMemcpyAsync(d_b, bases, n * sizeof(A), hipMemcpyHostToDevice, st));
            G16_HIP_TRY(hipMemcpyAsync(d_s, scalars, n * sizeof(Fr), hipMemcpyHostToDevice, st));
        }
        int merged_c = 0;
        const char* e = getenv("G16_MSM_API_PRECOMP");
        uint32_t modw[Fr::N];
        for (int i = 0; i < Fr::N; ++i) modw[i] = Fr::Params::mod(i);
        if (((e && atoi(e) != 0) || shard_n > 1) && n) merged_c = merged_window_bits(n, Fr::Params::BITS, modw, Fr::N);
        if (shard_n > 1 && n && !merged_c) return G16_ERR_BAD_ARG;
        if (shard_n > 1 && !n) { memset(out_affine, 0, sizeof(A)); drain.dismiss(); return G16_OK; }
        if (merged_c) {
            const int W = msm_plan_windows(merged_c, Fr::Params::BITS, modw, Fr::N);
            A* d_t = nullptr;
            G16_TRY(ctx->arena.alloc_n((size_t)n * W, &d_t));
            G16_TRY((build_window_tables<F>(d_b, n, merged_c, W, d_t, st)));
            d_b = d_t;
        } else {
            G16_TRY((convert_bases<F>(d_b, n, st)));
        }
        ScalarSort ss;
        G16_TRY((sort_scalars<C>(d_s, n, merged_c, ctx->arena, st, &ss, shard_n, shard_r)));
        MsmBuffers<F> buf;
        G16_TRY((msm_bucket_pass<F>(d_b, 0, n, ss, ctx->arena, st, &buf, &ctx->t_bucket[0])));
        G16_TRY((msm_reduce<F>(buf, ss, st)));
        std::vector<X> hws(ss.plan.outputs());
        G16_HIP_TRY(hipMemcpyAsync(hws.data(), buf.window_sums, sizeof(X) * ss.plan.outputs(), hipMemcpyDeviceToHost, st));
        G16_HIP_TRY(hipStreamSynchronize(st));
        drain.dismiss();
        const A res = fold_windows<F>(hws.data(), ss.plan).to_affine();
        memcpy(out_affine, &res, sizeof(A));
        ctx->tm.bucket_pass_ms = ctx->t_bucket[0].ms();
        ctx->tm.bucket_ms[0] = ctx->tm.bucket_pass_ms;
        ctx->tm.window_bits = ss.plan.c;
        ctx->tm.windows = ss.plan.W;
        return G16_OK;
    }

    static int ntt_api(g16_ctx* ctx, uint64_t* data, int log_n, int inverse, int coset) {
        if (log_n < 0 || log_n > 30) return G16_ERR_DEGREE_TOO_LARGE;
        hipStream_t st = ctx->stream;
        Domain<C>* dom = nullptr;
        G16_TRY((domain_create<C>(log_n, st, &dom)));
        const size_t n = dom->n;
        ctx->reset_arena();
        Fr *d_a = nullptr, *d_o = nullptr;
        int rc = G16_OK;
        auto body = [&]() -> int {
            G16_TRY(ctx->arena.alloc_n(n, &d_a));
            G16_TRY(ctx->arena.alloc_n(n, &d_o));
            G16_HIP_TRY(hipMemcpyAsync(d_a, data, n * sizeof(Fr), hipMemcpyHostToDevice, st));
            if (!inverse) {
                if (coset) {
                    G16_TRY((domain_ensure_gpow<C>(dom, st)));
                    G16_TRY((scale_by_table<C>(d_a, dom->g_pow, n, st)));
                }
                G16_TRY((ntt_dif<C>(dom, d_a, false, st)));
                G16_TRY((bitrev_scale<C>(dom, d_o, d_a, nullptr, nullptr, st)));
            } else {
                G16_TRY((ntt_dif<C>(dom, d_a, true, st)));
                if (coset) G16_TRY((bitrev_scale<C>(dom, d_o, d_a, dom->s2, nullptr, st)));
                else G16_TRY((bitrev_scale<C>(dom, d_o, d_a, nullptr, &dom->n_inv, st)));
            }
            G16_HIP_TRY(hipMemcpyAsync(data, d_o, n * sizeof(Fr), hipMemcpyDeviceToHost, st));
            G16_HIP_TRY(hipStreamSynchronize(st));
            return G16_OK;
        };
        rc = body();
        domain_destroy<C>(dom);
        return rc;
    }

    template <class F>
    static int field_op(int op, const uint64_t* a, const uint64_t* b, uint64_t* out) {
        F x = load_pod<F>(a), y = b ? load_pod<F>(b) : F::zero(), r;
        switch (op) {
            case 0: r = x + y; break;
            case 1: r = x - y; break;
            case 2: r = x * y; break;
            case 3: r = x.inverse(); break;
            case 4: x.to_canonical(r.v); break;
            case 5: r = F::from_canonical(x.v); break;
            default: return G16_ERR_BAD_ARG;
        }
        memcpy(out, &r, sizeof(F));
        return G16_OK;
    }
    template <class F>
    static int group_op(int op, const uint64_t* p_, const uint64_t* q_, uint64_t* out) {
        typedef Affine<F> A;
        typedef XYZZ<F> X;
        const A p = load_pod<A>(p_);
        X acc = X::from_affine(p);
        if (op == 0) {
            acc.add_affine(load_pod<A>(q_));
        } else if (op == 1) {
            uint32_t k[8];
            memcpy(k, q_, 32);
            acc = acc.mul_bits(k, 256);
        } else if (op == 2) {
            X q = X::from_affine(load_pod<A>(q_));
            X p2 = acc.dbl(), q2 = q.dbl();
            p2.add(q2);
            X np = acc.neg();
            p2.add(np);
            X nq = q.neg();
            p2.add(nq);
            acc = p2;
        } else {
            return G16_ERR_BAD_ARG;
        }
        const A r = acc.to_affine();
        memcpy(out, &r, sizeof(A));
        return G16_OK;
    }
    template <class F>
    static int msm_model(const uint64_t* bases_, const uint64_t* scalars_, uint64_t n, int c_override, uint64_t* out, int shard_n = 1,
                         int shard_r = 0) {
        typedef Affine<F> A;
        typedef XYZZ<F> X;
        uint32_t modw[Fr::N];
        for (int i = 0; i < Fr::N; ++i) modw[i] = Fr::Params::mod(i);
        MsmPlan plan;
        if (c_override > 0) {
            char buf[16];
            snprintf(buf, sizeof(buf), "%d", c_override);
            setenv("G16_MSM_WINDOW", buf, 1);
        }
        if (shard_n > 1 && c_override >= 0) return G16_ERR_BAD_ARG;
        int rc = make_msm_plan(n, Fr::Params::BITS, modw, Fr::N, c_override < 0 ? -c_override : 0, &plan, shard_n, shard_r);
        if (c_override > 0) unsetenv("G16_MSM_WINDOW");
        if (rc) return rc;
        const A* bases = reinterpret_cast<const A*>(bases_);
        std::vector<X> buckets((size_t)plan.buckets(), X::identity());
        for (uint64_t i = 0; i < n; ++i) {
            Fr s;
            memcpy(&s, scalars_ + 4 * i, sizeof(Fr));
            uint32_t can[Fr::N], sp[MSM_SWORDS];
            s.to_canonical(can);
            uint64_t carry = 0;
            for (int k = 0; k < 10; ++k) {
                carry += (uint64_t)(k < Fr::N ? can[k] : 0u) + plan.K[k];
                sp[k] = (uint32_t)carry;
                carry >>= 32;
            }
            sp[10] = 0;
            A p;
            memcpy(&p, bases + i, sizeof(A));
            for (int w = 0; w < plan.W; ++w) {
                if (plan.merged && w) {
                    X d = X::from_affine(p);
                    for (int k = 0; k < plan.c; ++k) d = d.dbl();
                    p = d.to_affine();
                }
                uint32_t bucket, neg;
                if (!digit_to_bucket(window_raw(sp, w, plan.c), plan.c, &bucket, &neg)) continue;
                if (plan.shard_n > 1) {
                    if (bucket % (uint32_t)plan.shard_n != (uint32_t)plan.shard_r) continue;
                    bucket /= (uint32_t)plan.shard_n;
                }
                A q = p;
                if (neg) q.y = q.y.neg();
                buckets[plan.merged ? (size_t)bucket : (size_t)w * plan.B + bucket].add_affine(q);
            }
        }
        const uint32_t G = plan.chunk_buckets(), cpw = plan.chunks();
        const int NP = plan.planes();
        std::vector<X> wsum(plan.outputs(), X::identity());
        for (int w = 0; w < plan.groups; ++w) {
            for (uint32_t ch = 0; ch < cpw; ++ch) {
// ... 20 lines not shown
```

### groth16_amd/csrc/window_tables.hpp

```cpp
#pragma once
#include "fp30.hpp"
#include "batch_affine.hpp"

namespace g16 {

template <class F>
G16_HD void jac30_double(F& X, F& Y, F& Z) {
    const F A = X.sqr();
    const F B2 = Y.sqr().dbl();
    const F D = X.mul(B2.dbl());
    const F E = A.dbl().add(A);
    const F Z3 = Y.mul(Z).dbl();
    const F X3 = E.sqr().template sub<4>(D.dbl());
    const F C8 = B2.sqr().dbl();
    Y = E.mul(D.template sub<8>(X3)).template sub<4>(C8);
    X = X3;
    Z = Z3;
}

template <class F, class IO>
G16_HD void window_table_task(IO& io, int c, int W) {
    F X, Y;
    if (!io.load(X, Y)) {
        for (int j = 0; j < W; ++j) io.store_identity(j);
        return;
    }
    io.store(0, X, Y);
    F Z = F::one(), run = F::one();
    int live = W;
    for (int j = 1; j < W; ++j) {
        for (int d = 0; d < c; ++d) jac30_double(X, Y, Z);
        if (io.is_zero(Z)) { live = j; break; }
        io.put(4 * (j - 1) + 0, X);
        io.put(4 * (j - 1) + 1, Y);
        io.put(4 * (j - 1) + 2, Z);
        io.put(4 * (j - 1) + 3, run);
        run = run.mul(Z);
    }
    F inv = batch_inverse(run);
    for (int j = W - 1; j >= live; --j) io.store_identity(j);
    for (int j = live - 1; j >= 1; --j) {
        const F Zj = io.get(4 * (j - 1) + 2);
        const F zi = inv.mul(io.get(4 * (j - 1) + 3));
        inv = inv.mul(Zj);
        const F zi2 = zi.sqr();
        const F ax = io.get(4 * (j - 1) + 0).mul(zi2);
        const F ay = io.get(4 * (j - 1) + 1).mul(zi2.mul(zi));
        io.store(j, io.canonical(ax), io.canonical(ay));
    }
}

template <class F30> struct TableLane;
template <class P>
struct TableLane<Fp30<P>> {
    typedef Fp30<P> B;
    G16_HD static const B& comp(const Fp30<P>& v) { return v; }
    G16_HD static Fp30<P> wrap(const B& b) { return b; }
    G16_HD static bool all(bool v) { return v; }
    G16_HD static int part() { return 0; }
    static constexpr int PARTS = 1;
};
template <class P>
struct TableLane<Fp2p30<P>> {
    typedef Fp30<P> B;
    G16_HD static const B& comp(const Fp2p30<P>& v) { return v.c; }
    G16_HD static Fp2p30<P> wrap(const B& b) { return Fp2p30<P>{b}; }
    G16_HD static bool all(bool v) { return Fp2p30<P>::both(v); }
    G16_HD static int part() { return Fp2p30<P>::lane_hi() ? 1 : 0; }
    static constexpr int PARTS = 2;
};

template <class F30>
struct TableDeviceIO {
    typedef TableLane<F30> TL;
    typedef typename TL::B B;
    typedef typename B::Std W32;
    static constexpr int NL = B::NL;
    const W32* src_pt;
    W32* table_pt;
    uint64_t row_stride;
    uint32_t* park;
    uint64_t stride;
    G16_HD bool load(F30& x, F30& y) const {
        const int k = TL::part();
        const W32 xs = src_pt[k], ys = src_pt[TL::PARTS + k];
        if (TL::all(xs.is_zero() && ys.is_zero())) return false;
        const W32 x0 = B::std_to_r30(xs), y0 = B::std_to_r30(ys);
        x = TL::wrap(B::unpack(x0.v));
        y = TL::wrap(B::unpack(y0.v));
        return true;
    }
    G16_HD void store(int row, const F30& x, const F30& y) const {
        const int k = TL::part();
        W32 ox, oy;
        TL::comp(x).pack(ox.v);
        TL::comp(y).pack(oy.v);
        table_pt[(uint64_t)row * row_stride + k] = ox;
        table_pt[(uint64_t)row * row_stride + TL::PARTS + k] = oy;
    }
    G16_HD void store_identity(int row) const {
        const int k = TL::part();
        table_pt[(uint64_t)row * row_stride + k] = W32::zero();
        table_pt[(uint64_t)row * row_stride + TL::PARTS + k] = W32::zero();
    }
    G16_HD void put(int slot, const F30& v) const {
        const B& b = TL::comp(v);
        G16_UNROLL for (int l = 0; l < NL; ++l) park[((uint64_t)slot * NL + l) * stride] = b.l[l];
    }
    G16_HD F30 get(int slot) const {
        B b;
        G16_UNROLL for (int l = 0; l < NL; ++l) b.l[l] = park[((uint64_t)slot * NL + l) * stride];
        return TL::wrap(b);
    }
    G16_HD bool is_zero(const F30& v) const { return TL::all(TL::comp(v).maybe_zero()) && TL::all(TL::comp(v).is_zero_exact()); }
    G16_HD F30 canonical(const F30& v) const { return TL::wrap(TL::comp(v).canonical_lt2p()); }
};

}
```

Before: 67.55 million constraints/s.

## Store precomputed MSM window tables as unpacked 30-bit limb rows

The window-table builder now writes each precomputed point directly in the unpacked 30-bit-limb form the accumulator uses, instead of packing it back to 32-bit standard words. The merged bucket-accumulate kernel gets a LimbRows source that loads these rows without unpacking and adds via add_affine_signed, removing per-point unpack work in the hot MSM loop. In exchange the tables grow (13/12 for BLS12-381), so the memory budget heuristic for bucket mode is scaled up, which could disable the precomputed path on tighter memory. Test forms are added for the new row format.

```diff
diff --git a/groth16_amd/csrc/api.hip b/groth16_amd/csrc/api.hip
--- a/groth16_amd/csrc/api.hip
+++ b/groth16_amd/csrc/api.hip
@@ -235,8 +235,9 @@
             else if (!me || strcmp(me, "auto") == 0) {
                 const double key_bytes = (double)(g1b * 8) * (double)(m * 2 + w + hl) + (double)(g2b * 8) * (double)m;
                 const double rows = m >= ((uint64_t)1 << 20) ? 13.0 : 32.0;
-                const double need = rows * key_bytes * 1.08 + 3.0 * key_bytes + 8.0 * 1073741824.0;
-                bucket = rows * key_bytes <= 80.0 * 1073741824.0 && !(view->flags & G16_PK_DEVICE_PTRS);
+                const double limb_form = ctx->curve == G16_BLS12_381 ? 13.0 / 12.0 : 9.0 / 8.0;
+                const double need = rows * key_bytes * limb_form * 1.08 + 3.0 * key_bytes + 8.0 * 1073741824.0;
+                bucket = rows * key_bytes * limb_form <= 80.0 * 1073741824.0 && !(view->flags & G16_PK_DEVICE_PTRS);
                 const char* pc = getenv("G16_MSM_PRECOMP");
                 if ((pc && atoi(pc) == 0) || m <= 1 || hl == 0) bucket = false;
                 for (g16_ctx* sub : ctx->subs) {
diff --git a/groth16_amd/csrc/batch_affine.hpp b/groth16_amd/csrc/batch_affine.hpp
--- a/groth16_amd/csrc/batch_affine.hpp
+++ b/groth16_amd/csrc/batch_affine.hpp
@@ -176,7 +176,9 @@
             const uint64_t row = a.merged ? (uint64_t)((v >> 26) & 31u) * a.base_count : 0;
             const int64_t idx = (int64_t)pt + a.shift;
             if (idx < 0 || (uint64_t)idx >= a.base_count) return false;
-            if (!F::load_point(a.in, (int64_t)row + idx, x, y)) return false;
+            if (a.merged ? !F::load_row(reinterpret_cast<const typename F::Row*>(a.in), (int64_t)row + idx, x, y)
+                         : !F::load_point(a.in, (int64_t)row + idx, x, y))
+                return false;
             if (v >> 31) y = y.neg_canonical();
             return true;
         } else {
diff --git a/groth16_amd/csrc/devtest.hip b/groth16_amd/csrc/devtest.hip
--- a/groth16_amd/csrc/devtest.hip
+++ b/groth16_amd/csrc/devtest.hip
@@ -1,5 +1,6 @@
 #include "internal.hpp"
 #include "fp30.hpp"
+#include "window_tables.hpp"
 #include <vector>
 
 using namespace g16;
@@ -34,6 +35,8 @@
         case 63: case 64: case 65: i = 8; o = 2; break;
         case 70: i = 11; o = 5; break;
         case 71: case 72: i = 21; o = 9; break;
+        case 80: i = 3; o = 5; break;
+        case 81: i = 5; o = 9; break;
         default: return false;
     }
     *nin = i;
@@ -42,7 +45,7 @@
 }
 constexpr int lab_nin(int form) { int i = 0, o = 0; lab_slots(form, &i, &o); return i; }
 constexpr int lab_nout(int form) { int i = 0, o = 0; lab_slots(form, &i, &o); return o; }
-constexpr bool lab_is_pair(int form) { return (form >= 60 && form < 70) || form == 72; }
+constexpr bool lab_is_pair(int form) { return (form >= 60 && form < 70) || form == 72 || form == 81; }
 template <class P>
 constexpr bool lab_has(int form) {
     constexpr bool base = FipsAsm<P>::has_sub;
@@ -98,6 +101,26 @@
         if (a.inf) a.x = a.y = a.zz = a.zzz = F::zero();
         stf(out, 0, hi, a.x); stf(out, C, hi, a.y); stf(out, 2 * C, hi, a.zz); stf(out, 3 * C, hi, a.zzz);
         if (F::LANES_PER_TASK == 1 || hi == 0) st_flag<P>(out, 4 * C, a.inf);
+    }
+};
+
+template <class P, class F>
+struct RowLab {
+    typedef Fp30<P> B;
+    static constexpr int C = F::LANES_PER_TASK == 2 ? 2 : 1;
+    G16_HD static void run(const uint32_t* in, uint32_t* out, int lane, typename F::Row& row) {
+        const Fp<P> xw = ld_words<P>(in, lane), yw = ld_words<P>(in, C + lane);
+        const bool flip = in[2 * C * B::NL] != 0;
+        TableDeviceIO<B> io{nullptr, row.w[lane], 0, nullptr, 0};
+        if (xw.is_zero() && yw.is_zero()) io.store_identity(0);
+        else io.store(0, B::unpack(xw.v), B::unpack(yw.v));
+        st<P>(out, 2 * C + 1 + lane, B::unpack(xw.v));
+        st<P>(out, 3 * C + 1 + lane, B::unpack_cond_neg(yw, flip));
+    }
+    G16_HD static void gathered(uint32_t* out, int lane, bool ok, const B& px, const B& py, bool flip) {
+        st<P>(out, lane, px);
+        st<P>(out, C + lane, B::cond_neg2(py, flip));
+        if (lane == 0) st_flag<P>(out, 2 * C, ok);
     }
 };
 
@@ -161,8 +184,17 @@
         }
         else if constexpr (FORM == 70) AccLab<P, Fp30<P>>::run(in, out, 0);
         else if constexpr (FORM == 71) AccLab<P, Fp2x30<P>>::run(in, out, 0);
+        else if constexpr (FORM == 80) {
+            typename B::Row row[1];
+            RowLab<P, B>::run(in, out, 0, row[0]);
+            B px, py;
+            const bool ok = B::load_row(row, 0, px, py);
+            RowLab<P, B>::gathered(out, 0, ok, px, py, in[2 * B::NL] != 0);
+        }
     }
 };
+
+constexpr int LAB_WG = 64;
 
 template <class P, int FORM>
 struct LabPair {
@@ -172,6 +204,15 @@
     static __device__ __forceinline__ void run(const uint32_t* in, uint32_t* out) {
         const int hi = F::lane_hi() ? 1 : 0;
         if constexpr (FORM == 72) { AccLab<P, F>::run(in, out, hi); return; }
+        if constexpr (FORM == 81) {
+            __shared__ typename F::Row rows[LAB_WG / 2];
+            typename F::Row* row = &rows[threadIdx.x >> 1];
+            RowLab<P, F>::run(in, out, hi, *row);
+            F px = F::zero(), py = F::zero();
+            const bool ok = F::load_row(row, 0, px, py);
+            RowLab<P, F>::gathered(out, hi, ok, px.c, py.c, in[4 * B::NL] != 0);
+            return;
+        }
         auto L = [&](int k) { return F{ld<P>(in, 2 * k + hi)}; };
         F r = F::zero();
         if constexpr (FORM == 60) r = F::mul_v(F::lhs(L(0)), F::rhs(L(1)));
@@ -184,6 +225,19 @@
     }
 #endif
     static void run_host(const uint32_t* in, uint32_t* out) {
+        if constexpr (FORM == 81) {
+            typename F::Row row;
+            for (int h = 0; h < 2; ++h) RowLab<P, F>::run(in, out, h, row);
+            bool zero = true;
+            for (int h = 0; h < 2; ++h)
+                for (int i = 0; i < 2 * B::NL; ++i) zero = zero && row.w[h][i] == 0;
+            for (int h = 0; h < 2; ++h) {
+                B px, py;
+                for (int i = 0; i < B::NL; ++i) { px.l[i] = row.w[h][i]; py.l[i] = row.w[h][B::NL + i]; }
+                RowLab<P, F>::gathered(out, h, !zero, px, py, in[4 * B::NL] != 0);
+            }
+            return;
+        }
         for (int h = 0; h < 2; ++h) {
             const bool hi = h != 0;
             auto C = [&](int k, int c) { return ld<P>(in, 2 * k + c); };
@@ -199,8 +253,6 @@
         }
     }
 };
-
-constexpr int LAB_WG = 64;
 
 template <class P, int FORM>
 __global__ void __launch_bounds__(LAB_WG) devlab_op(const uint32_t* __restrict__ in, uint32_t* __restrict__ out, uint32_t n) {
@@ -253,7 +305,8 @@
 
 #define LAB_FORMS(X)                                                                                                              \
     X(0) X(1) X(2) X(3) X(4) X(5) X(6) X(7) X(8) X(9) X(10) X(11) X(20) X(21) X(22) X(23) X(24) X(25) X(26) X(27) X(28) X(30) X(31) \
-    X(32) X(33) X(34) X(35) X(36) X(37) X(38) X(39) X(40) X(41) X(42) X(43) X(50) X(51) X(60) X(61) X(62) X(63) X(64) X(65) X(70) X(71) X(72)
+    X(32) X(33) X(34) X(35) X(36) X(37) X(38) X(39) X(40) X(41) X(42) X(43) X(50) X(51) X(60) X(61) X(62) X(63) X(64) X(65) X(70) X(71) X(72) \
+    X(80) X(81)
 
 template <class P>
 int lab_dispatch(bool device, hipStream_t st, int form, const uint32_t* operands, uint64_t n, uint32_t* out) {
diff --git a/groth16_amd/csrc/fp30.hpp b/groth16_amd/csrc/fp30.hpp
--- a/groth16_amd/csrc/fp30.hpp
+++ b/groth16_amd/csrc/fp30.hpp
@@ -7,6 +7,20 @@
 #endif
 
 namespace g16 {
+
+template <class P> struct Fp30;
+
+#ifndef G16_TABLE_ROW_ALIGN
+#define G16_TABLE_ROW_ALIGN 8
+#endif
+template <class P, int PARTS>
+struct alignas(G16_TABLE_ROW_ALIGN) TableRow {
+    uint32_t w[PARTS][2 * P::NL30];
+};
+template <class F> struct TableRowFor;
+template <class P> struct TableRowFor<Fp<P>> { typedef TableRow<P, 1> type; };
+template <class P> struct TableRowFor<Fp2<P>> { typedef TableRow<P, 2> type; };
+template <class F> constexpr size_t table_row_bytes() { return sizeof(typename TableRowFor<F>::type); }
 
 template <class P>
 struct Fp30 {
@@ -410,7 +424,12 @@
         yw = p.y;
         return true;
     }
-
+    typedef TableRow<P, 1> Row;
+    G16_HD static bool load_row(const Row* rows, int64_t idx, Fp30& px, Fp30& py) {
+        const uint32_t* w = rows[idx].w[0];
+        G16_UNROLL for (int i = 0; i < NL; ++i) { px.l[i] = w[i]; py.l[i] = w[NL + i]; }
+        return !(px.raw_zero() && py.raw_zero());
+    }
 
     G16_HD Fp30 canonical_lt2p() const {
         Fp30 d;
@@ -711,6 +730,12 @@
         return true;
     }
     G16_HD static Fp2p30 unpack_cond_neg(const PackedC& y, bool flip) { return {B::unpack_cond_neg(y, flip)}; }
+    typedef TableRow<P, 2> Row;
+    G16_HD static bool load_row(const Row* rows, int64_t idx, Fp2p30& px, Fp2p30& py) {
+        const uint32_t* w = rows[idx].w[lane_hi() ? 1 : 0];
+        G16_UNROLL for (int i = 0; i < B::NL; ++i) { px.c.l[i] = w[i]; py.c.l[i] = w[B::NL + i]; }
+        return !both(px.c.raw_zero() && py.c.raw_zero());
+    }
 };
 
 template <class R>
diff --git a/groth16_amd/csrc/internal.hpp b/groth16_amd/csrc/internal.hpp
--- a/groth16_amd/csrc/internal.hpp
+++ b/groth16_amd/csrc/internal.hpp
@@ -206,7 +206,7 @@
 template <class F> int msm_heavy_reduce_batch(const MsmBuffers<F>* const* bufs, const ScalarSort* const* sorts, int n, hipStream_t st);
 template <class F> int convert_bases(Affine<F>* d_bases, uint64_t n, hipStream_t st);
 template <class F> XYZZ<F> fold_windows(const XYZZ<F>* window_sums, const MsmPlan& plan);
-template <class F> int build_window_tables(const Affine<F>* d_src, uint64_t n, int c, int W, Affine<F>* d_table, hipStream_t st, void* park = nullptr);
+template <class F> int build_window_tables(const Affine<F>* d_src, uint64_t n, int c, int W, void* d_table, hipStream_t st, void* park = nullptr);
 template <class F> size_t window_table_park_bytes(uint64_t n, int W);
 
 template <class C>
diff --git a/groth16_amd/csrc/key_load.hpp b/groth16_amd/csrc/key_load.hpp
--- a/groth16_amd/csrc/key_load.hpp
+++ b/groth16_amd/csrc/key_load.hpp
@@ -63,8 +63,9 @@
         const int W = msm_plan_windows(c, Fr::Params::BITS, modw, Fr::N);
         if (W <= 0) return G16_ERR_INTERNAL;
         const char* cap = getenv("G16_PK_TABLE_BUDGET_MB");
-        if (cap && (double)q.count * sizeof(P) * W > atof(cap) * 1048576.0) return G16_ERR_OOM;
-        if (ls.alloc((void**)out, q.count * sizeof(P) * (size_t)W) != G16_OK) return G16_ERR_OOM;
+        const size_t table_bytes = q.count * g16::table_row_bytes<F>() * (size_t)W;
+        if (cap && (double)table_bytes > atof(cap) * 1048576.0) return G16_ERR_OOM;
+        if (ls.alloc((void**)out, table_bytes) != G16_OK) return G16_ERR_OOM;
         const P* src = reinterpret_cast<const P*>(q.points);
         P* staged = nullptr;
         if (!dev_ptrs) {
@@ -182,8 +183,9 @@
         {
             const uint64_t rows_z = p->c_z ? (uint64_t)msm_plan_windows(p->c_z, Fr::Params::BITS, modw, Fr::N) : 1;
             const uint64_t rows_h = p->c_h ? (uint64_t)msm_plan_windows(p->c_h, Fr::Params::BITS, modw, Fr::N) : 1;
-            p->table_bytes = rows_z * ((v->a.count + v->b_g1.count + v->l.count) * sizeof(G1A) + v->b_g2.count * sizeof(G2A)) +
-                             rows_h * v->h.count * sizeof(G1A);
+            const uint64_t g1z = p->c_z ? g16::table_row_bytes<Fq>() : sizeof(G1A), g2z = p->c_z ? g16::table_row_bytes<Fq2>() : sizeof(G2A);
+            const uint64_t g1h = p->c_h ? g16::table_row_bytes<Fq>() : sizeof(G1A);
+            p->table_bytes = rows_z * ((v->a.count + v->b_g1.count + v->l.count) * g1z + v->b_g2.count * g2z) + rows_h * v->h.count * g1h;
         }
         const bool load_ok = hipStreamSynchronize(ctx->stream) == hipSuccess;
         ls.release();
diff --git a/groth16_amd/csrc/msm.hip b/groth16_amd/csrc/msm.hip
--- a/groth16_amd/csrc/msm.hip
+++ b/groth16_amd/csrc/msm.hip
@@ -5,6 +5,7 @@
 #include "window_tables.hpp"
 #include <algorithm>
 #include <cstdlib>
+#include <type_traits>
 
 namespace g16 {
 
@@ -376,9 +377,40 @@
     AccRaw<typename F30::Raw>* partials[PASS_BATCH];
 };
 
-template <class F30, bool DIRECT>
+struct PackedPoints {
+    template <class F30> using Y = typename F30::PackedC;
+    template <class F30> __device__ __forceinline__ static Y<F30> y_zero() { return Y<F30>::zero(); }
+    __device__ __forceinline__ static bool decode(uint32_t v, int64_t shift, uint64_t base_count, int64_t* at) {
+        const int64_t idx = (int64_t)(v & 0x7fffffffu) + shift;
+        *at = idx;
+        return idx >= 0 && (uint64_t)idx < base_count;
+    }
+    template <class F30>
+    __device__ __forceinline__ static bool load(const Affine<typename F30::Std>* bases, int64_t at, F30& px, Y<F30>& py) {
+        return F30::load_point_py(bases, at, px, py);
+    }
+    template <class Acc, class F30>
+    __device__ __forceinline__ static void add(Acc& acc, const F30& px, const Y<F30>& py, bool minus) { acc.add_affine_packed(px, py, minus); }
+};
+struct LimbRows {
+    template <class F30> using Y = F30;
+    template <class F30> __device__ __forceinline__ static Y<F30> y_zero() { return F30::zero(); }
+    __device__ __forceinline__ static bool decode(uint32_t v, int64_t shift, uint64_t base_count, int64_t* at) {
+        const int64_t idx = (int64_t)(v & 0x3ffffffu) + shift;
+        *at = (int64_t)((uint64_t)((v >> 26) & 31u) * base_count) + idx;
+        return idx >= 0 && (uint64_t)idx < base_count;
+    }
+    template <class F30>
+    __device__ __forceinline__ static bool load(const Affine<typename F30::Std>* bases, int64_t at, F30& px, Y<F30>& py) {
+        return F30::load_row(reinterpret_cast<const typename F30::Row*>(bases), at, px, py);
+    }
+    template <class Acc, class F30>
+    __device__ __forceinline__ static void add(Acc& acc, const F30& px, const Y<F30>& py, bool minus) { acc.add_affine_signed(px, py, minus); }
+};
+
+template <class F30, bool DIRECT, class Src>
 __global__ __launch_bounds__(ACC_THREADS, F30::ACC_MIN_WAVES) void bucket_accumulate30_kernel(
-    PassBatch<F30> batch, uint32_t M, uint32_t off_shift, uint32_t lseg, uint32_t merged) {
+    PassBatch<F30> batch, uint32_t M, uint32_t off_shift, uint32_t lseg) {
     const Affine<typename F30::Std>* __restrict__ bases = batch.bases[blockIdx.y];
     const int64_t shift = batch.shift[blockIdx.y];
     const uint64_t base_count = batch.base_count[blockIdx.y];
@@ -405,22 +437,15 @@
     acc.inf = true;
     auto flush = [&](AccRaw<typename F30::Raw>* dst) { acc.gather().store_raw(dst); acc.inf = true; };
     uint32_t v_next = 0;
-    typedef typename F30::PackedC YNext;
+    typedef typename Src::template Y<F30> YNext;
     F30 px_next = F30::zero();
-    YNext py_next = YNext::zero();
+    YNext py_next = Src::template y_zero<F30>();
     bool ok_next = false;
-    auto decode = [&](uint32_t v, int64_t* at) -> bool {
-        const uint32_t pt = merged ? (v & 0x3ffffffu) : (v & 0x7fffffffu);
-        const uint64_t row = merged ? (uint64_t)((v >> 26) & 31u) * base_count : 0;
-        const int64_t idx = (int64_t)pt + shift;
-        *at = (int64_t)row + idx;
-        return idx >= 0 && (uint64_t)idx < base_count;
-    };
     auto fetch = [&](uint32_t v) {
         v_next = DIRECT ? 0u : v;
         int64_t at = (int64_t)v;
-        ok_next = DIRECT ? true : decode(v, &at);
-        if (ok_next) ok_next = F30::load_point_py(bases, at, px_next, py_next);
+        ok_next = DIRECT ? true : Src::decode(v, shift, base_count, &at);
+        if (ok_next) ok_next = Src::template load<F30>(bases, at, px_next, py_next);
     };
     fetch(DIRECT ? start : sorted[start]);
     uint32_t v_fetch = DIRECT ? start + 1 : (start + 1 < end ? sorted[start + 1] : 0u);
@@ -440,7 +465,7 @@
             else v_fetch = e + 2 < end ? sorted[e + 2] : 0u;
         };
         if constexpr (F30::ACC_PREFETCH) advance();
-        if (ok) acc.add_affine_packed(px, py, (v >> 31) != 0);
+        if (ok) Src::add(acc, px, py, (v >> 31) != 0);
         if constexpr (!F30::ACC_PREFETCH) advance();
     }
     flush(&partials[slot_off[b] + (t - b_first / lseg)]);
@@ -959,7 +984,7 @@
             b.bases[i] = lists[(R - 1) & 1]; b.shift[i] = 0; b.base_count[i] = 0; b.sorted[i] = nullptr;
             b.offsets[i] = ss.offsets; b.slot_off[i] = ss.task_off; b.partials[i] = partials;
         }
-        hipLaunchKernelGGL((bucket_accumulate30_kernel<F30, true>), grid, dim3(ACC_THREADS), 0, st, b, M, (uint32_t)R, plan.Lmax, 0u);
+        hipLaunchKernelGGL((bucket_accumulate30_kernel<F30, true, PackedPoints>), grid, dim3(ACC_THREADS), 0, st, b, M, (uint32_t)R, plan.Lmax);
         G16_LAUNCH_CHECK();
     }
     if (bucket_timer) G16_TRY(bucket_timer->stop(st));
@@ -999,8 +1024,12 @@
     if (max_segments) {
         const uint64_t lanes = (uint64_t)max_segments * F30::LANES_PER_TASK;
         const dim3 grid((unsigned)((lanes + ACC_THREADS - 1) / ACC_THREADS), (unsigned)n);
-        hipLaunchKernelGGL((bucket_accumulate30_kernel<F30, false>), grid, dim3(ACC_THREADS), pass_lds_pad<F30>(), st, b, plan.buckets(), 0u,
-                           plan.Lmax, plan.merged ? 1u : 0u);
+        if (plan.merged)
+            hipLaunchKernelGGL((bucket_accumulate30_kernel<F30, false, LimbRows>), grid, dim3(ACC_THREADS), pass_lds_pad<F30>(), st, b,
+                               plan.buckets(), 0u, plan.Lmax);
+        else
+            hipLaunchKernelGGL((bucket_accumulate30_kernel<F30, false, PackedPoints>), grid, dim3(ACC_THREADS), pass_lds_pad<F30>(), st, b,
+                               plan.buckets(), 0u, plan.Lmax);
         G16_LAUNCH_CHECK();
     }
     if (bucket_timer) G16_TRY(bucket_timer->stop(st));
@@ -1143,14 +1172,15 @@
 template <class F30>
 __global__ __launch_bounds__(TABLE_THREADS, 2) void build_window_tables_kernel(const Affine<typename F30::Std>* __restrict__ src, uint64_t first,
                                                                               uint64_t count, uint64_t n, int c, int W,
-                                                                              Affine<typename F30::Std>* __restrict__ table, uint32_t* __restrict__ park) {
+                                                                              typename F30::Row* __restrict__ table, uint32_t* __restrict__ park) {
     typedef TableDeviceIO<F30> IO;
     typedef typename IO::W32 W32;
     const uint64_t lane = (uint64_t)blockIdx.x * TABLE_THREADS + threadIdx.x;
     const uint64_t t = lane / F30::LANES_PER_TASK;
     if (t >= count) return;
     const uint64_t i = first + t;
-    IO io{reinterpret_cast<const W32*>(src + i), reinterpret_cast<W32*>(table + i), n * 2 * IO::TL::PARTS, park + lane, count * F30::LANES_PER_TASK};
+    IO io{reinterpret_cast<const W32*>(src + i), table[i].w[IO::TL::part()], n * (sizeof(typename F30::Row) / sizeof(uint32_t)), park + lane,
+          count * F30::LANES_PER_TASK};
     window_table_task<F30>(io, c, W);
 }
 
@@ -1162,9 +1192,10 @@
 }
 
 template <class F>
-int build_window_tables(const Affine<F>* d_src, uint64_t n, int c, int W, Affine<F>* d_table, hipStream_t st, void* park_buf) {
+int build_window_tables(const Affine<F>* d_src, uint64_t n, int c, int W, void* d_table, hipStream_t st, void* park_buf) {
     typedef typename Lazy30<F>::type F30;
     static_assert(sizeof(Affine<F>) == 2 * TableLane<F30>::PARTS * sizeof(typename TableLane<F30>::B::Std), "affine point = x parts | y parts");
+    static_assert(std::is_same<typename F30::Row, typename TableRowFor<F>::type>::value, "the builder writes the rows the bucket pass gathers");
     if (n == 0) return G16_OK;
     if (W > TABLE_MAX_W) return G16_ERR_INTERNAL;
     const uint64_t chunk = std::min(n, TABLE_CHUNK);
@@ -1175,7 +1206,7 @@
         const uint64_t count = std::min(chunk, n - first);
         const uint64_t lanes = count * F30::LANES_PER_TASK;
         hipLaunchKernelGGL((build_window_tables_kernel<F30>), dim3((unsigned)((lanes + TABLE_THREADS - 1) / TABLE_THREADS)), dim3(TABLE_THREADS), 0, st,
-                           d_src, first, count, n, c, W, d_table, park);
+                           d_src, first, count, n, c, W, static_cast<typename F30::Row*>(d_table), park);
         if (hipGetLastError() != hipSuccess) rc = G16_ERR_HIP;
     }
     if (!park_buf) {
@@ -1189,8 +1220,8 @@
     template int convert_bases<typename C::Fq>(Affine<typename C::Fq>*, uint64_t, hipStream_t);                             \
     template int convert_bases<typename C::Fq2>(Affine<typename C::Fq2>*, uint64_t, hipStream_t);                           \
     template int sort_scalars<C>(const typename C::Fr*, uint64_t, int, Arena&, hipStream_t, ScalarSort*, int, int);                   \
-    template int build_window_tables<typename C::Fq>(const Affine<typename C::Fq>*, uint64_t, int, int, Affine<typename C::Fq>*, hipStream_t, void*);    \
-    template int build_window_tables<typename C::Fq2>(const Affine<typename C::Fq2>*, uint64_t, int, int, Affine<typename C::Fq2>*, hipStream_t, void*); \
+    template int build_window_tables<typename C::Fq>(const Affine<typename C::Fq>*, uint64_t, int, int, void*, hipStream_t, void*);    \
+    template int build_window_tables<typename C::Fq2>(const Affine<typename C::Fq2>*, uint64_t, int, int, void*, hipStream_t, void*); \
     template size_t window_table_park_bytes<typename C::Fq>(uint64_t, int);                                                 \
     template size_t window_table_park_bytes<typename C::Fq2>(uint64_t, int);                                                \
     template int msm_bucket_pass<typename C::Fq>(const Affine<typename C::Fq>*, int64_t, uint64_t, const ScalarSort&, Arena&, \
diff --git a/groth16_amd/csrc/unit_api.hpp b/groth16_amd/csrc/unit_api.hpp
--- a/groth16_amd/csrc/unit_api.hpp
+++ b/groth16_amd/csrc/unit_api.hpp
@@ -79,10 +79,10 @@
         if (shard_n > 1 && !n) { memset(out_affine, 0, sizeof(A)); drain.dismiss(); return G16_OK; }
         if (merged_c) {
             const int W = msm_plan_windows(merged_c, Fr::Params::BITS, modw, Fr::N);
-            A* d_t = nullptr;
+            typename TableRowFor<F>::type* d_t = nullptr;
             G16_TRY(ctx->arena.alloc_n((size_t)n * W, &d_t));
             G16_TRY((build_window_tables<F>(d_b, n, merged_c, W, d_t, st)));
-            d_b = d_t;
+            d_b = reinterpret_cast<A*>(d_t);
         } else {
             G16_TRY((convert_bases<F>(d_b, n, st)));
         }
diff --git a/groth16_amd/csrc/window_tables.hpp b/groth16_amd/csrc/window_tables.hpp
--- a/groth16_amd/csrc/window_tables.hpp
+++ b/groth16_amd/csrc/window_tables.hpp
@@ -77,7 +77,7 @@
     typedef typename B::Std W32;
     static constexpr int NL = B::NL;
     const W32* src_pt;
-    W32* table_pt;
+    uint32_t* row0;
     uint64_t row_stride;
     uint32_t* park;
     uint64_t stride;
@@ -91,17 +91,12 @@
         return true;
     }
     G16_HD void store(int row, const F30& x, const F30& y) const {
-        const int k = TL::part();
-        W32 ox, oy;
-        TL::comp(x).pack(ox.v);
-        TL::comp(y).pack(oy.v);
-        table_pt[(uint64_t)row * row_stride + k] = ox;
-        table_pt[(uint64_t)row * row_stride + TL::PARTS + k] = oy;
+        uint32_t* w = row0 + (uint64_t)row * row_stride;
+        G16_UNROLL for (int l = 0; l < NL; ++l) { w[l] = TL::comp(x).l[l]; w[NL + l] = TL::comp(y).l[l]; }
     }
     G16_HD void store_identity(int row) const {
-        const int k = TL::part();
-        table_pt[(uint64_t)row * row_stride + k] = W32::zero();
-        table_pt[(uint64_t)row * row_stride + TL::PARTS + k] = W32::zero();
+        uint32_t* w = row0 + (uint64_t)row * row_stride;
+        G16_UNROLL for (int l = 0; l < 2 * NL; ++l) w[l] = 0;
     }
     G16_HD void put(int slot, const F30& v) const {
         const B& b = TL::comp(v);
```

After: 66.96 million constraints/s. No clear change (-0.9%).
